# elodin-sys/elodin

Hardware: AMD Instinct MI355X
Metric: entity-steps/s (6DOF RK4) (higher is better)
Workload: dtype f64

## Files before the change

elodin_amd/codegen.py:

```python
from __future__ import annotations

import hashlib
import os
import subprocess
from dataclasses import dataclass, field
from pathlib import Path
from typing import Callable, Optional, Dict, List, NamedTuple, Sequence, Tuple

from . import dsl

PKG = Path(__file__).resolve().parent
CSRC = PKG / "csrc"
JIT_DIR = PKG / "_jit"
HIPCC = os.environ.get("HIPCC", "/opt/rocm/bin/hipcc")

_LEAF_CPP = {
    "qi": "b.q.i", "qj": "b.q.j", "qk": "b.q.k", "qw": "b.q.w", "px": "b.p.x", "py": "b.p.y", "pz": "b.p.z",
    "wx": "b.v.ang.x", "wy": "b.v.ang.y", "wz": "b.v.ang.z", "vx": "b.v.lin.x", "vy": "b.v.lin.y", "vz": "b.v.lin.z",
    "Ix": "b.I.x", "Iy": "b.I.y", "Iz": "b.I.z", "mass": "b.mass",
}
_BIN = {"add": "+", "sub": "-", "mul": "*", "div": "/"}
_FN1 = {"sqrt": "m_sqrt", "abs": "m_abs", "sin": "m_sin", "cos": "m_cos", "tan": "m_tan", "exp": "m_exp",
        "log": "m_log", "acos": "m_acos", "asin": "m_asin", "log1p": "m_log1p", "expm1": "m_expm1", "cbrt": "m_cbrt",
        "floor": "m_floor", "ceil": "m_ceil", "trunc": "m_trunc", "rint": "m_rint", "sinh": "m_sinh", "cosh": "m_cosh",
# ... 1490 lines not shown
    if constexpr (kOnlySmall != 1) {{      // one pack launch (unless p->packed), then fold + integrate per tick
        const hipError_t e = launch_pair_ticks_t<PairCustom, false, kOnlyIntegrator>(*p, integrator, n_ticks, p->packed != 0, s, launches);
        if (e != hipSuccess) return static_cast<int>(e);
    }}
    return static_cast<int>(hipSuccess);
}}
'''


def build_pair(tf: "dsl.TracedFold", integrator: Optional[int] = None, small: Optional[bool] = None) -> Path:
    return _compile(generate_pair_source(tf, integrator, small), "pair")


def generate_graph_fold_source(tf: "dsl.TracedGraphFold") -> str:
    u = _Unit()
    f = tf.fold
    w = tf.widths[f.out]
    _, loads_a, loads_b, body = _fold_front(u, tf.outputs, w, [(f"P.left[{i}]", tf.widths[n]) for i, n in enumerate(f.left)],
                                            [(f"P.right[{i}]", tf.widths[n]) for i, n in enumerate(f.right)], T="double")
    init = ", ".join(repr(v) for v in f.init)
    nl = "\n"
    return f'''// generated by elodin_amd/codegen.py — do not edit.  stand-alone edge_fold system: {f.__name__}
#include <hip/hip_runtime.h>
#include <cstdint>
#include <cmath>
namespace sixdof {{
__device__ __forceinline__ double fast_sqrt(double x) {{ return sqrt(x); }}
__device__ __forceinline__ float fast_sqrt(float x) {{ return sqrtf(x); }}
{_PRELUDE}
{_emit_tables(u)}
struct GraphFoldParams {{
    const double* left[8];
    const double* right[8];
    double* scratch;             // [n_src, {w}]
    double* out;                 // the output component column, dense over the row set
    const uint32_t* row_start;   // [n_src + 1]
    const uint32_t* dst;         // [n_edges] target rows
    const uint32_t* src_rows;    // [n_src] source rows
    uint32_t n_src;
}};

__global__ __launch_bounds__(256) void graph_fold_kernel(const GraphFoldParams P) {{
    using T = double;
    const uint32_t i = blockIdx.x * blockDim.x + threadIdx.x;
    if (i >= P.n_src) return;
    const uint32_t row = P.src_rows[i];
{nl.join(loads_a)}
    double acc[{w}] = {{{init}}};
    for (uint32_t e = P.row_start[i]; e < P.row_start[i + 1]; e++) {{
{nl.join(loads_b("P.dst[e]"))}
{body}
    }}
    for (int k = 0; k < {w}; k++) P.scratch[(size_t)i * {w} + k] = acc[k];
}}

__global__ __launch_bounds__(256) void graph_fold_commit(const GraphFoldParams P) {{
    const uint32_t i = blockIdx.x * blockDim.x + threadIdx.x;
    if (i >= P.n_src) return;
    for (int k = 0; k < {w}; k++) P.out[(size_t)P.src_rows[i] * {w} + k] = P.scratch[(size_t)i * {w} + k];
}}
}}  // namespace sixdof

extern "C" unsigned graph_fold_abi() {{ return static_cast<unsigned>(sizeof(sixdof::GraphFoldParams)); }}
extern "C" int graph_fold_launch(const sixdof::GraphFoldParams* p, unsigned n_ticks, void* stream) {{
    using namespace sixdof;
    if (p->n_src == 0) return 0;
    hipStream_t s = static_cast<hipStream_t>(stream);
    const dim3 grid((p->n_src + 255) / 256);
    for (unsigned t = 0; t < n_ticks; t++) {{
        hipLaunchKernelGGL(graph_fold_kernel, grid, dim3(256), 0, s, *p);
        hipLaunchKernelGGL(graph_fold_commit, grid, dim3(256), 0, s, *p);
    }}
    return static_cast<int>(hipGetLastError());
}}
'''


def build_graph_fold(tf: "dsl.TracedGraphFold") -> Path:
    return _compile(generate_graph_fold_source(tf), "gfold")


def _headers_digest() -> str:
    h = hashlib.sha1()
    for name in ("step_kernel.hpp", "pair_kernel.hpp", "effectors.hpp", "spatial.hpp", "kernels.hpp"):
        h.update((CSRC / name).read_bytes())
    h.update((PKG.parent / "include" / "sixdof_hip.h").read_bytes())
    return h.hexdigest()


def policy_for(n_rows: int, row_elems: int, elem_bytes: int) -> Optional[int]:
    if os.environ.get("SIXDOF_STREAMING") is not None or os.environ.get("SIXDOF_ALL_POLICIES", "") == "1":
        return None
    return 1 if int(n_rows) * int(row_elems) * int(elem_bytes) <= (768 << 20) else 9


def build(tp: dsl.TracedPipe, dtype: str = "float64", integrator: int = 0, fast_math: bool = False, window_soa: bool = False,
          column_soa: bool = False, guard_selects: Optional[bool] = None, policy: Optional[int] = None) -> Path:
    policy = policy if policy in (0, 1, 9) else None
    if getattr(tp, "prebuilt_so", None) is not None:
        if not Path(tp.prebuilt_so).exists():
            raise FileNotFoundError(tp.prebuilt_so)
        return Path(tp.prebuilt_so)
    if getattr(tp, "frozen_source", None) is not None:
        return _compile(tp.frozen_source, "pipe")
    if dtype == "float32" and getattr(tp, "float32_refused", None):
        raise NotImplementedError("this program cannot be built with dtype float32: " + "; ".join(tp.float32_refused[:4]))
    variants = VARIANTS if isinstance(tp, dsl.TracedProgram) else VARIANTS[:2]
    first_src = None
    if isinstance(tp, dsl.TracedProgram) and not tp.fold_stages:
        u = _unit(tp, variants[0], fast_math, window_soa, column_soa, guard_selects, policy, estimate=True)
        first_src = _source(tp, dtype, integrator, fast_math, u)
        est = u.estimate
        regs_per_value = 2 if dtype == "float64" else 1
        held = sum(int(w_) for _, w_ in tp.columns)
        if est and (est.get("program", 0) + held) * regs_per_value > PRESSURE_BUDGET_REGS:
            lean = sorted([v for v in ("program", "demand", "pressure") if v in est], key=lambda v: (est[v], VARIANTS.index(v)))
            variants = tuple(lean) + tuple(v for v in variants if v not in lean)
            first_src = None
        last_estimate.clear()
        last_estimate.update(est)
    for k, variant in enumerate(variants):
        try:
            src_k = first_src if (k == 0 and first_src is not None) else \
                generate_variant(tp, variant, dtype, integrator, fast_math, window_soa, column_soa, guard_selects, policy)
            so = _compile(src_k, "pipe", expect_scratch=variant == "memory")
            last_variant[0] = variant
            return so
        except SpillError:
            if os.environ.get(ALLOW_SPILLS_ENV, "") == "1" or k == len(variants) - 1:
                raise


VARIANTS = ("program", "demand", "pressure", "memory", "out_of_line")
PRESSURE_BUDGET_REGS = 440
last_estimate: Dict[str, int] = {}
last_variant = ["program"]


def generate_variant(tp, variant: str, dtype: str = "float64", integrator: int = 0, fast_math: bool = False, window_soa: bool = False,
                     column_soa: bool = False, guard_selects: Optional[bool] = None, policy: Optional[int] = None) -> str:
    if variant not in VARIANTS:
        raise ValueError(f"variant must be one of {VARIANTS}")
    return _source(tp, dtype, integrator, fast_math, _unit(tp, variant, fast_math, window_soa, column_soa, guard_selects, policy))


_BASE_FLAGS = ["-mllvm", "-disable-machine-licm"]
_RETRY_FLAGS = ["-mllvm", "-sink-insts-to-avoid-spills"]
_ATTEMPTS = (("-O3", _BASE_FLAGS), ("-O3", _BASE_FLAGS + _RETRY_FLAGS), ("-O1", []))
_CACHE_TAG = "rp3"
SPECULATIVE_MIN_SOURCE = 120_000
build_stats: Dict[str, float] = {"hipcc_invocations": 0, "cache_hits": 0}
ALLOW_SPILLS_ENV = "SIXDOF_ALLOW_SPILLS"
last_resources: Dict[str, int] = {}


class SpillError(RuntimeError):
    """No build of a generated program fits a wave's registers."""


_hipcc_id = None


def _hipcc_version() -> str:
    global _hipcc_id
    if _hipcc_id is None:
        try:
            _hipcc_id = subprocess.run([HIPCC, "--version"], capture_output=True, text=True).stdout.strip()
# ... 381 lines not shown
```

elodin_amd/csrc/aql_chain.cpp:

```cpp
#include <dlfcn.h>
#include <elf.h>
#include <hip/hip_runtime.h>
#include <hsa/hsa_ext_amd.h>

#include <algorithm>
#include <atomic>
#include <chrono>
#include <cstring>
#include <fstream>
#include <iterator>
#include <map>
#include <mutex>
#include <string>
#include <vector>

#include "aql_chain.hpp"

namespace sixdof::aql {

namespace {

constexpr uint32_t kRingSlots = 1024;
constexpr char kBundleMagic[] = "__CLANG_OFFLOAD_BUNDLE__";
constexpr char kTarget[] = "hipv4-amdgcn-amd-amdhsa--gfx950";
// ... 117 lines not shown
                uint64_t off, size, tl;
                std::memcpy(&off, sec + e, 8);
                std::memcpy(&size, sec + e + 8, 8);
                std::memcpy(&tl, sec + e + 16, 8);
                e += 24;
                if (e + tl > s.sh_size) break;
                if (std::string(sec + e, tl) == kTarget && b + off + size <= s.sh_size) out.emplace_back(s.sh_offset + b + off, size);
                e += tl;
            }
        }
    }
    return out;
}

bool contains(const char* p, size_t n, const std::string& needle) {
    return std::search(p, p + n, needle.begin(), needle.end()) != p + n;
}

}

Device* acquire(int hip_device, std::string* why) {
    std::lock_guard<std::mutex> lock(g_devices_mutex);
    auto it = g_devices.find(hip_device);
    if (it != g_devices.end()) {
        it->second->refs++;
        return it->second;
    }
    hsa_status_t s = hsa_init();
    if (s != HSA_STATUS_SUCCESS) return *why = hsa_error("hsa_init", s), nullptr;
    auto* d = new Device();
    d->hip_device = hip_device;
    if (!setup(d, why)) {
        destroy(d);
        return nullptr;
    }
    d->refs = 1;
    g_devices[hip_device] = d;
    return d;
}

void release(Device* d) {
    if (!d) return;
    std::lock_guard<std::mutex> lock(g_devices_mutex);
    if (--d->refs > 0) return;
    g_devices.erase(d->hip_device);
    destroy(d);
}

bool kernel_code(Device* d, const void* stub, uint32_t explicit_kernarg_bytes, KernelCode* out, std::string* why) {
    std::lock_guard<std::mutex> lock(d->m);
    if (auto it = d->kernels.find(stub); it != d->kernels.end()) return *out = it->second, true;
    Dl_info info{};
    if (!dladdr(stub, &info) || !info.dli_sname || info.dli_saddr != stub) return *why = "dladdr: the kernel's host handle has no symbol", false;
    const std::string name = std::string(info.dli_sname) + ".kd";
    for (const auto& [off, size] : gfx950_code_objects(d->library)) {
        if (!contains(d->library.data() + off, size, std::string(1, '\0') + name + '\0')) continue;
        auto ex = d->executables.find(off);
        if (ex == d->executables.end()) {
            hsa_code_object_reader_t reader;
            hsa_executable_t exe;
            hsa_status_t s = hsa_code_object_reader_create_from_memory(d->library.data() + off, size, &reader);
            if (s != HSA_STATUS_SUCCESS) return *why = hsa_error("hsa_code_object_reader_create_from_memory", s), false;
            s = hsa_executable_create_alt(HSA_PROFILE_FULL, HSA_DEFAULT_FLOAT_ROUNDING_MODE_DEFAULT, nullptr, &exe);
            if (s == HSA_STATUS_SUCCESS) {
                s = hsa_executable_load_agent_code_object(exe, d->agent, reader, nullptr, nullptr);
                if (s == HSA_STATUS_SUCCESS) s = hsa_executable_freeze(exe, nullptr);
                if (s != HSA_STATUS_SUCCESS) hsa_executable_destroy(exe);
            }
            hsa_code_object_reader_destroy(reader);
            if (s != HSA_STATUS_SUCCESS) return *why = hsa_error("loading the library's gfx950 code object", s), false;
            ex = d->executables.emplace(off, exe).first;
        }
        hsa_executable_symbol_t sym;
        if (hsa_executable_get_symbol_by_name(ex->second, name.c_str(), &d->agent, &sym) != HSA_STATUS_SUCCESS) continue;
        KernelCode k;
        bool dynamic_stack = true;
        hsa_status_t s = hsa_executable_symbol_get_info(sym, HSA_EXECUTABLE_SYMBOL_INFO_KERNEL_OBJECT, &k.object);
        if (s == HSA_STATUS_SUCCESS) s = hsa_executable_symbol_get_info(sym, HSA_EXECUTABLE_SYMBOL_INFO_KERNEL_KERNARG_SEGMENT_SIZE, &k.kernarg_size);
        if (s == HSA_STATUS_SUCCESS) s = hsa_executable_symbol_get_info(sym, HSA_EXECUTABLE_SYMBOL_INFO_KERNEL_KERNARG_SEGMENT_ALIGNMENT, &k.kernarg_align);
        if (s == HSA_STATUS_SUCCESS) s = hsa_executable_symbol_get_info(sym, HSA_EXECUTABLE_SYMBOL_INFO_KERNEL_GROUP_SEGMENT_SIZE, &k.group_size);
        if (s == HSA_STATUS_SUCCESS) s = hsa_executable_symbol_get_info(sym, HSA_EXECUTABLE_SYMBOL_INFO_KERNEL_PRIVATE_SEGMENT_SIZE, &k.private_size);
        if (s == HSA_STATUS_SUCCESS) s = hsa_executable_symbol_get_info(sym, HSA_EXECUTABLE_SYMBOL_INFO_KERNEL_DYNAMIC_CALLSTACK, &dynamic_stack);
        if (s != HSA_STATUS_SUCCESS) return *why = hsa_error("hsa_executable_symbol_get_info", s), false;
        if (k.kernarg_size != explicit_kernarg_bytes)
            return *why = name + ": kernarg segment of " + std::to_string(k.kernarg_size) + " bytes, " +
                          std::to_string(explicit_kernarg_bytes) + " explicit (hidden arguments)", false;
        if (dynamic_stack) return *why = name + ": dynamic call stack", false;
        d->kernels[stub] = k;
        return *out = k, true;
    }
    return *why = name + ": not found in the library's gfx950 code objects", false;
}

namespace {

uint64_t ring_read_index(void* q) { return hsa_queue_load_read_index_scacquire(static_cast<hsa_queue_t*>(q)); }
uint64_t ring_reserve(void* q, uint64_t n) { return hsa_queue_add_write_index_scacq_screl(static_cast<hsa_queue_t*>(q), n); }
void ring_doorbell(void* q, uint64_t index) {
    hsa_signal_store_screlease(static_cast<hsa_queue_t*>(q)->doorbell_signal, static_cast<hsa_signal_value_t>(index));
}

}

bool run_chain(Device* d, const Run* runs, size_t n_runs, double stall_s, double* device_ms, std::string* why) {
    std::lock_guard<std::mutex> lock(d->m);
    if (d->fault.empty() && d->queue_status.load() != HSA_STATUS_SUCCESS)
        d->fault = hsa_error("AQL queue error", static_cast<hsa_status_t>(d->queue_status.load()));
    if (!d->fault.empty()) return *why = d->fault, false;
    uint64_t n = 0;
    for (size_t i = 0; i < n_runs; i++) n += runs[i].count;
    *device_ms = 0.0;
    if (n == 0) return true;
    hsa_signal_store_relaxed(d->first, 1);
    hsa_signal_store_relaxed(d->last, 1);
    const hsa_signal_t first = n == 1 ? d->last : d->first;
    const Ring ring{static_cast<hsa_kernel_dispatch_packet_t*>(d->queue->base_address), d->queue->size, d->queue,
                    ring_read_index, ring_reserve, ring_doorbell};
    if (!write_chain(ring, runs, n_runs, first, d->last, stall_s))
        return *why = d->fault = "AQL chain: the queue read no packet for " + std::to_string(stall_s) + " s", false;
    uint64_t seen = hsa_queue_load_read_index_relaxed(d->queue);
    auto deadline = std::chrono::steady_clock::now() + std::chrono::duration<double>(stall_s);
    while (hsa_signal_load_scacquire(d->last) != 0) {
        if (d->queue_status.load() != HSA_STATUS_SUCCESS)
            return *why = d->fault = hsa_error("AQL queue error", static_cast<hsa_status_t>(d->queue_status.load())), false;
        const auto now = std::chrono::steady_clock::now();
        if (const uint64_t read = hsa_queue_load_read_index_relaxed(d->queue); read != seen) {
            seen = read;
            deadline = now + std::chrono::duration<double>(stall_s);
        } else if (now > deadline) {
            return *why = d->fault = "AQL chain: no progress for " + std::to_string(stall_s) + " s", false;
        }
    }
    hsa_amd_profiling_dispatch_time_t a{}, b{};
    if (hsa_amd_profiling_get_dispatch_time(d->agent, first, &a) == HSA_STATUS_SUCCESS &&
        hsa_amd_profiling_get_dispatch_time(d->agent, d->last, &b) == HSA_STATUS_SUCCESS && b.end > a.start)
        *device_ms = static_cast<double>(b.end - a.start) * 1e-6;
    return true;
}

}
```

elodin_amd/csrc/aql_chain.hpp:

```cpp
#pragma once

#include <hsa/hsa.h>

#include <cstdint>
#include <string>

namespace sixdof::aql {

constexpr uint16_t kWorkgroup = 64;

struct KernelCode {
    uint64_t object = 0;
    uint32_t kernarg_size = 0, kernarg_align = 0, group_size = 0, private_size = 0;
};

struct Run {
    KernelCode code;
    const void* kernarg = nullptr;
    uint32_t blocks = 0;
    uint64_t count = 0;
};

uint32_t header_setup(uint64_t i, uint64_t n);

void fill_body(hsa_kernel_dispatch_packet_t* p, const KernelCode& k, uint32_t blocks, const void* kernarg, hsa_signal_t signal);

struct Ring {
    hsa_kernel_dispatch_packet_t* base = nullptr;
    uint64_t size = 0;
    void* ctx = nullptr;
    uint64_t (*read_index)(void* ctx) = nullptr;
    uint64_t (*reserve)(void* ctx, uint64_t n) = nullptr;
    void (*doorbell)(void* ctx, uint64_t index) = nullptr;
};

bool write_chain(const Ring& r, const Run* runs, size_t n_runs, hsa_signal_t first, hsa_signal_t last, double timeout_s);


struct Device;

Device* acquire(int hip_device, std::string* why);
void release(Device* d);

bool kernel_code(Device* d, const void* stub, uint32_t explicit_kernarg_bytes, KernelCode* out, std::string* why);

bool run_chain(Device* d, const Run* runs, size_t n_runs, double stall_s, double* device_ms, std::string* why);

}
```

elodin_amd/csrc/aql_packets.cpp:

```cpp
#include <chrono>
#include <cstring>

#include "aql_chain.hpp"

namespace sixdof::aql {

uint32_t header_setup(uint64_t i, uint64_t n) {
    const uint32_t acquire = i == 0 ? HSA_FENCE_SCOPE_SYSTEM : HSA_FENCE_SCOPE_AGENT;
    const uint32_t release = i + 1 == n ? HSA_FENCE_SCOPE_SYSTEM : HSA_FENCE_SCOPE_AGENT;
    const uint32_t header = (HSA_PACKET_TYPE_KERNEL_DISPATCH << HSA_PACKET_HEADER_TYPE) | (1u << HSA_PACKET_HEADER_BARRIER) |
                            (acquire << HSA_PACKET_HEADER_SCACQUIRE_FENCE_SCOPE) |
                            (release << HSA_PACKET_HEADER_SCRELEASE_FENCE_SCOPE);
    const uint32_t setup = 1u << HSA_KERNEL_DISPATCH_PACKET_SETUP_DIMENSIONS;
    return header | setup << 16;
}

void fill_body(hsa_kernel_dispatch_packet_t* p, const KernelCode& k, uint32_t blocks, const void* kernarg, hsa_signal_t signal) {
    std::memset(reinterpret_cast<char*>(p) + 4, 0, sizeof(*p) - 4);
    p->workgroup_size_x = kWorkgroup;
    p->workgroup_size_y = 1;
    p->workgroup_size_z = 1;
    p->grid_size_x = static_cast<uint32_t>(kWorkgroup) * blocks;
    p->grid_size_y = 1;
    p->grid_size_z = 1;
    p->private_segment_size = k.private_size;
    p->group_segment_size = k.group_size;
    p->kernel_object = k.object;
    p->kernarg_address = const_cast<void*>(kernarg);
    p->completion_signal = signal;
}

bool write_chain(const Ring& r, const Run* runs, size_t n_runs, hsa_signal_t first, hsa_signal_t last, double timeout_s) {
    uint64_t n = 0;
    for (size_t i = 0; i < n_runs; i++) n += runs[i].count;
    if (n == 0) return true;
    const hsa_signal_t none{0};
    size_t run = 0;
    uint64_t in_run = 0;
    uint64_t done = 0;
    while (done < n) {
        uint64_t room = r.size - (r.reserve(r.ctx, 0) - r.read_index(r.ctx));
        const auto deadline = std::chrono::steady_clock::now() + std::chrono::duration<double>(timeout_s);
        while (room == 0) {
            if (std::chrono::steady_clock::now() > deadline) return false;
            room = r.size - (r.reserve(r.ctx, 0) - r.read_index(r.ctx));
        }
        const uint64_t m = n - done < room ? n - done : room;
        const uint64_t w = r.reserve(r.ctx, m);
        for (uint64_t j = 0; j < m; j++) {
            while (in_run == runs[run].count) run++, in_run = 0;
            const Run& R = runs[run];
            const uint64_t i = done + j;
            const hsa_signal_t sig = i + 1 == n ? last : i == 0 ? first : none;
            fill_body(&r.base[(w + j) & (r.size - 1)], R.code, R.blocks, R.kernarg, sig);
            in_run++;
        }
        for (uint64_t j = 0; j < m; j++)
            __atomic_store_n(reinterpret_cast<uint32_t*>(&r.base[(w + j) & (r.size - 1)]), header_setup(done + j, n), __ATOMIC_RELEASE);
        done += m;
        r.doorbell(r.ctx, w + m - 1);
    }
    return true;
}

}
```

elodin_amd/csrc/hip_fake.cpp:

```cpp
#include <hip/hip_runtime.h>

#include <algorithm>
#include <cstdio>
#include <cstdlib>
#include <cstring>
#include <deque>
#include <functional>
#include <map>
#include <set>
#include <string>
#include <vector>

#include "../../include/sixdof_hip.h"
#include "aql_chain.hpp"
#include "covariance_plan.hpp"
#include "envelope_plan.hpp"
#include "events_plan.hpp"
#include "extremes_plan.hpp"
#include "history_plan.hpp"
#include "kernels.hpp"
#include "quantile_plan.hpp"

namespace hip_fake {

std::map<const char*, size_t> g_allocs;
std::set<void*> g_streams, g_events;
std::map<const char*, size_t> g_pins;
long g_calls = 0, g_fail_at = -1, g_violations = 0;
bool g_fired = false;

enum { kAtOnce = 0, kMinimal = 1, kComputeFirst = 2, kCopyFirst = 3 };
int g_schedule = kAtOnce;
bool g_running = false;
struct Op {
    std::string what;
    std::function<hipError_t()> run;
    std::vector<const void*> dev;
    const char* host = nullptr;
    size_t host_bytes = 0;
    void* wait_stream = nullptr;
    uint64_t wait_pos = 0;
};
struct Queue {
    uint64_t order = 0;
    bool non_blocking = false;
    std::deque<Op> ops;
    uint64_t done = 0;
    uint64_t enqueued() const { return done + ops.size(); }
};
struct Record { void* stream = nullptr; uint64_t pos = 0; };
std::map<void*, Queue> g_queues;
std::map<void*, Record> g_records;
std::vector<void*> g_quarantine;
uint64_t g_order = 0;

void fail_after(long n) { g_fail_at = n < 0 ? -1 : g_calls + n, g_fired = false; }
bool fired() { return g_fired; }
long calls() { return g_calls; }
long violations() { return g_violations; }
size_t live_allocations() { return g_allocs.size(); }
size_t live_streams() { return g_streams.size(); }
size_t live_events() { return g_events.size(); }
size_t live_page_locks() { return g_pins.size(); }
bool lock_intersects(const void* p, size_t bytes) {
    const char* lo = static_cast<const char*>(p);
    for (auto& kv : g_pins)
        if (kv.first < lo + bytes && lo < kv.first + kv.second) return true;
    return false;
}
size_t queued() {
    size_t n = 0;
    for (auto& kv : g_queues) n += kv.second.ops.size();
    return n;
}
const char* schedule_name(int schedule) {
    return schedule == kAtOnce ? "at-once" : schedule == kMinimal ? "minimal" : schedule == kComputeFirst ? "compute-first" : "copy-first";
}

static hipError_t fallible() {
    if (g_calls++ != g_fail_at) return hipSuccess;
    g_fired = true;
    return hipErrorOutOfMemory;
}
static bool live(const void* p, size_t bytes) {
    auto it = g_allocs.upper_bound(static_cast<const char*>(p));
    if (!p || it == g_allocs.begin()) return false;
    --it;
    return static_cast<const char*>(p) + bytes <= it->first + it->second;
}
static bool need(bool ok, const char* what) {
    if (!ok) std::fprintf(stderr, "hip_fake: a launch was handed a table that is not (wholly) a live allocation: %s\n", what), g_violations++;
    return ok;
}
static hipError_t launch(bool ok) {
    if (!g_running)
        if (hipError_t e = fallible(); e != hipSuccess) return e;
    return ok ? hipSuccess : hipErrorInvalidValue;
}

static void flush_quarantine() {
    if (queued()) return;
    for (void* p : g_quarantine) std::free(p);
    g_quarantine.clear();
}
static hipError_t drain(void* s, uint64_t upto) {
    auto it = g_queues.find(s);
    if (it == g_queues.end()) return hipSuccess;
    Queue& q = it->second;
    hipError_t first = hipSuccess;
    while (q.done < upto && !q.ops.empty()) {
        Op& op = q.ops.front();
        if (op.wait_stream)
            if (hipError_t e = drain(op.wait_stream, op.wait_pos); e != hipSuccess) return e;
        if (op.run) {
            if (hipError_t e = fallible(); e != hipSuccess) return e;
            g_running = true;
            const hipError_t e = op.run();
            g_running = false;
            if (e != hipSuccess && first == hipSuccess) first = e;
        }
        q.ops.pop_front();
        q.done++;
    }
    return first;
}
static hipError_t drain_all(bool youngest_first, bool blocking_only = false) {
    std::vector<std::pair<uint64_t, void*>> order;
    for (auto& kv : g_queues)
        if (!blocking_only || !kv.second.non_blocking) order.emplace_back(kv.second.order, kv.first);
    std::sort(order.begin(), order.end());
    if (youngest_first) std::reverse(order.begin(), order.end());
    hipError_t first = hipSuccess;
    for (auto& o : order) {
        auto it = g_queues.find(o.second);
        if (it == g_queues.end()) continue;
        const hipError_t e = drain(o.second, it->second.enqueued());
        if (e == hipErrorOutOfMemory) return e;
        if (e != hipSuccess && first == hipSuccess) first = e;
    }
    return first;
}
static hipError_t force(void* s, uint64_t upto) {
// ... 172 lines not shown
    std::memcpy(dst, src, bytes);
    return hipSuccess;
}
static const char* copy_name(hipMemcpyKind kind) {
    return kind == hipMemcpyDeviceToHost ? "device-to-host copy" : kind == hipMemcpyHostToDevice ? "host-to-device copy" : "device-to-device copy";
}
static void copy_host_side(void* dst, const void* src, size_t bytes, hipMemcpyKind kind) {
    if (kind == hipMemcpyDeviceToHost) host_extent(dst, bytes, copy_name(kind));
    if (kind == hipMemcpyHostToDevice) host_extent(src, bytes, copy_name(kind));
}
hipError_t hipMemcpy(void* dst, const void* src, size_t bytes, hipMemcpyKind kind) {
    copy_host_side(dst, src, bytes, kind);
    if (deferring()) {
        const hipError_t e = g_schedule == kMinimal ? drain_all(false, true) : force(nullptr, 0);
        flush_quarantine();
        if (e != hipSuccess) return e;
    }
    return copy(dst, src, bytes, kind);
}
hipError_t hipMemcpyAsync(void* dst, const void* src, size_t bytes, hipMemcpyKind kind, hipStream_t s) {
    if (!need(g_streams.count(s), "copy on a null or destroyed stream")) return hipErrorInvalidHandle;
    copy_host_side(dst, src, bytes, kind);
    if (!deferring()) return copy(dst, src, bytes, kind);
    std::vector<const void*> dev;
    if (kind != hipMemcpyHostToDevice) dev.push_back(src);
    if (kind != hipMemcpyDeviceToHost) dev.push_back(dst);
    const void* host = kind == hipMemcpyDeviceToHost ? dst : kind == hipMemcpyHostToDevice ? src : nullptr;
    if (kind == hipMemcpyDeviceToHost) std::memset(dst, 0xFF, bytes);
    return defer(s, copy_name(kind), std::move(dev), [=] { return copy(dst, src, bytes, kind); }, host, host ? bytes : 0);
}
hipError_t hipMemsetAsync(void* dst, int v, size_t bytes, hipStream_t s) {
    if (deferring()) return defer(s, "memset", {dst}, [=] { return hipMemsetAsync(dst, v, bytes, s); });
    if (!g_running)
        if (hipError_t e = fallible(); e != hipSuccess) return e;
    if (!need(live(dst, bytes), "memset destination")) return hipErrorInvalidValue;
    std::memset(dst, v, bytes);
    return hipSuccess;
}

namespace sixdof {

static bool body_ok(const void* pos, const void* vel, const void* accel, const void* force, const void* inertia, size_t n, size_t es) {
    return need(live(pos, n * 7 * es), "world_pos") & need(live(vel, n * 6 * es), "world_vel") & need(live(accel, n * 6 * es), "world_accel") &
           need(live(force, n * 6 * es), "force") & need(live(inertia, n * 7 * es), "inertia");
}
static bool ops_ok(const DevOp* ops, uint32_t n_ops, size_t n, size_t es) {
    bool ok = true;
    for (uint32_t k = 0; k < n_ops; k++)
        if (ops[k].aux) ok &= need(live(ops[k].aux, n * (ops[k].aux_width ? ops[k].aux_width : 3) * es), "effector aux column");
    return ok;
}
static bool step_ok(const StepParams& p, int dtype) {
    const size_t n = p.n, es = dtype == 1 ? 4 : 8;
    bool ok = body_ok(p.pos, p.vel, p.accel, p.force, p.inertia, n, es) & ops_ok(p.ops, p.n_ops, n, es);
    if (p.hist_ring) {
        const size_t r = p.hist_ring;
        ok &= need(live(p.hist_pos, r * n * 7 * es), "hist_pos") & need(live(p.hist_vel, r * n * 6 * es), "hist_vel") &
              need(live(p.hist_accel, r * n * 6 * es), "hist_accel") & need(live(p.hist_force, r * n * 6 * es), "hist_force");
    }
    for (int k = 0; k < kMaxModelCols; k++) {
        if (p.model_cols[k]) ok &= need(live(p.model_cols[k], n * es), "program column");
        if (p.model_hist[k]) ok &= need(live(p.model_hist[k], p.hist_ring * n * es), "program column ring");
    }
    return ok;
}
static bool pair_ok(const PairParams& p) {
    const size_t n = p.n, u = sizeof(uint32_t), d = sizeof(double);
    bool ok = body_ok(p.pos, p.vel, p.accel, p.force, p.inertia, n, 8) & ops_ok(p.ops, p.n_ops, n, 8);
    if (n) ok &= need(live(p.pack, n * kPackWidth * d), "pack") & need(live(p.partial, n * p.partial_width * p.splits * d), "partial");
    if (n && p.pack_next) ok &= need(live(p.pack_next, n * kPackWidth * d), "pack_next");
    if (p.pair_kind != SIXDOF_EFF_ALLPAIRS_GRAVITY_SOFTENED) {
        ok &= need(live(p.row_start, (n + 1) * u), "row_start");
        if (ok) ok &= need(p.row_start[n] == p.n_edges, "row_start[n] != n_edges");
    }
    if (p.n_edges) ok &= need(live(p.dst, p.n_edges * u), "dst");
    if (p.n_hubs)
        ok &= need(live(p.hub_rows, p.n_hubs * u), "hub_rows") & need(live(p.hub_chunk_start, (p.n_hubs + 1) * u), "hub_chunk_start") &
              need(live(p.chunk_e0, p.n_hub_chunks * u), "chunk_e0") & need(live(p.chunk_row, p.n_hub_chunks * u), "chunk_row") &
              need(live(p.chunk_partial, size_t(p.n_hub_chunks) * kPartialWidth * d), "chunk_partial");
    return ok;
}

StepKernel select_step(const StepParams&, int, int) { return {}; }
hipError_t launch_step(const StepParams& p, int integrator, int dtype, hipStream_t s) {
    if (deferring()) return defer(s, "launch_step", {p.pos, p.vel, p.accel, p.force, p.hist_pos, p.hist_vel, p.hist_accel, p.hist_force}, [=] { return launch_step(p, integrator, dtype, s); });
    const bool ok = step_ok(p, dtype);
    if (ok && p.hist_ring && p.hist_pos) {
        const size_t es = dtype == 1 ? 4 : 8;
        const void* live_col[4] = {p.pos, p.vel, p.accel, p.force};
        void* rings[4] = {p.hist_pos, p.hist_vel, p.hist_accel, p.hist_force};
        for (uint32_t t = 0; t < p.n_ticks; t++)
            for (int k = 0; k < 4; k++) {
                const size_t block = size_t(p.n) * (k == 0 ? 7 : 6) * es;
                std::memcpy(static_cast<char*>(rings[k]) + (p.hist_slot0 + t) % p.hist_ring * block, live_col[k], block);
            }
    }
    return launch(ok);
}
uint32_t pair_splits_for(uint32_t) { return 1; }
static hipError_t launch_pair(const PairParams& p, hipStream_t s) {
    if (deferring()) return defer(s, "pair launch", {p.pos, p.vel, p.accel, p.force, p.pack, p.partial}, [=] { return launch(pair_ok(p)); });
    return launch(pair_ok(p));
}
hipError_t launch_pair_ticks(const PairParams& p, int, uint32_t n_ticks, hipStream_t s, uint64_t* launches) { return *launches += 1 + 2 * n_ticks, launch_pair(p, s); }
hipError_t launch_pair_small(const PairParams& p, int, uint32_t, hipStream_t s, uint64_t* launches) { return *launches += 1, launch_pair(p, s); }
hipError_t launch_apollo(const ApolloParams&, hipStream_t s) {
    if (deferring()) return defer(s, "launch_apollo", {}, [] { return launch(true); });
    return launch(true);
}

static hipError_t move_rows(char* dst, const char* src, const uint32_t* rows, uint32_t m, size_t row, bool gather) {
    if (!need(live(rows, m * sizeof(uint32_t)), "join rows")) return launch(false);
    for (uint32_t j = 0; j < m; j++) {
        char* to = gather ? dst + j * row : dst + rows[j] * row;
        const char* from = gather ? src + rows[j] * row : src + j * row;
        if (!need(live(to, row) && live(from, row), "joined column")) return launch(false);
        std::memcpy(to, from, row);
    }
    return launch(true);
}
hipError_t launch_gather_rows(void* dst, const void* src, const uint32_t* rows, uint32_t m, uint32_t w, size_t elem, hipStream_t s) {
    if (deferring()) return defer(s, "gather_rows", {dst, src, rows}, [=] { return launch_gather_rows(dst, src, rows, m, w, elem, s); });
    return move_rows(static_cast<char*>(dst), static_cast<const char*>(src), rows, m, w * elem, true);
}
hipError_t launch_scatter_rows(void* dst, const void* src, const uint32_t* rows, uint32_t m, uint32_t w, size_t elem, hipStream_t s) {
    if (deferring()) return defer(s, "scatter_rows", {dst, src, rows}, [=] { return launch_scatter_rows(dst, src, rows, m, w, elem, s); });
    return move_rows(static_cast<char*>(dst), static_cast<const char*>(src), rows, m, w * elem, false);
}
hipError_t launch_history_gather(const HistoryGatherArgs& a, uint32_t n_components, void* out, const uint32_t* rows, uint64_t m, uint64_t n,
                                 uint64_t first_tick, uint64_t n_samples, uint64_t every, uint64_t ring, size_t elem, hipStream_t s) {
    if (deferring()) {
        std::vector<const void*> dev{out, rows};
        for (uint32_t c = 0; c < n_components; c++) dev.push_back(a.c[c].ring);
        return defer(s, "history_gather", std::move(dev), [=] { return launch_history_gather(a, n_components, out, rows, m, n, first_tick, n_samples, every, ring, elem, s); });
    }
    if (!need(live(rows, m * sizeof(uint32_t)), "watch rows")) return launch(false);
    for (uint32_t c = 0; c < n_components; c++) {
        const size_t row = a.c[c].w * elem;
        for (uint64_t e = 0; e < m; e++)
            for (uint64_t j = 0; j < n_samples; j++) {
                const char* from = static_cast<const char*>(a.c[c].ring) + (((first_tick + j * every - 1) % ring) * n + rows[e]) * row;
                char* to = static_cast<char*>(out) + a.c[c].out_offset * elem + (e * n_samples + j) * row;
                if (!need(live(from, row) && live(to, row), "ring or watch staging")) return launch(false);
                std::memcpy(to, from, row);
            }
    }
    return launch(true);
}
template <class Units, class Tick>
static bool ring_bin_walk(const char* who, const RingBinArgs& a, uint32_t n_components, double* out, uint64_t planes, uint64_t stride, uint64_t n,
                          uint32_t period, uint64_t first_tick, uint64_t sample0, uint64_t n_samples, uint64_t every, uint64_t ring, size_t elem,
                          Units units, Tick tick) {
    const std::string scratch = std::string(who) + " scratch of one sample", blocks = std::string("ring or ") + who + " staging";
    for (uint32_t k = 0; k < n_components; k++) {
        const RingBinDesc& d = a.c[k];
        if (!envelope_supported(d.w, period)) return false;
        if (!need(d.scratch_offset + units(d) <= stride, scratch.c_str())) return false;
        const uint64_t total = n * d.w;
        for (uint64_t j = 0; j < n_samples; j++) {
            const char* src = static_cast<const char*>(d.ring) + sample_slot(first_tick, sample0 + j, every, ring) * total * elem;
            double* to = out + d.out_offset + (sample0 + j) * period * planes * d.w;
            if (!need(live(src, total * elem) && live(to, size_t(period) * planes * d.w * sizeof(double)), blocks.c_str())) return false;
            tick(d, j, src, to);
        }
    }
    return true;
}
hipError_t launch_history_envelope(const RingBinArgs& a, uint32_t n_components, double* out, void* partial, uint64_t partial_stride, uint64_t n,
                                   uint32_t period, uint64_t first_tick, uint64_t sample0, uint64_t n_samples, uint64_t every, uint64_t ring,
// ... 322 lines not shown
```

elodin_amd/csrc/kernels.hpp:

```cpp
#pragma once
#include <hip/hip_runtime.h>
#include <stdint.h>

#pragma clang fp contract(on)

namespace sixdof {

constexpr int kMaxOps = 4;
constexpr int kMaxModelCols = 128;
constexpr int kBlock = 256;

struct DevOp {
    int32_t kind;
    int32_t aux_width;
    const void* aux;
    double p[6];
};

struct StepParams {
    void* pos;
    void* vel;
    void* accel;
    void* force;
    const void* inertia;
    uint32_t n;
    uint32_t n_ticks;
    double dt_g;
    double dt;
    uint32_t n_ops;
    uint32_t vel_independent;
    uint32_t streaming;
    uint32_t hist_ring;
    uint64_t hist_slot0;
    void* hist_pos;
    void* hist_vel;
    void* hist_accel;
    void* hist_force;
    uint64_t tick0;
    uint32_t accel_in_check;
    uint32_t state_only;
    DevOp ops[kMaxOps];
    void* model_cols[kMaxModelCols];
    void* model_hist[kMaxModelCols];
};

enum : int { kRk4 = 0, kSemiImplicit = 1, kNone = 2 };

struct StepKernel {
    const void* fn = nullptr;
    dim3 grid;
};

StepKernel select_step(const StepParams& p, int integrator, int dtype);

hipError_t launch_step(const StepParams& p, int integrator, int dtype, hipStream_t stream);

using CustomAbiFn = unsigned (*)();
using CustomLayoutFn = unsigned (*)();
using CustomLaunchFn = int (*)(const StepParams*, int integrator, int dtype, void* stream);

constexpr int kPackWidth = 10;
constexpr int kPartialForce = 9;
constexpr int kPartialWidth = 18;

struct PairParams {
    void* pos;
    void* vel;
    void* accel;
    void* force;
    const void* inertia;
    uint32_t n;
    double dt_g, dt;
    double* pack;
    double* pack_next;
    double* partial;
    uint32_t splits;
    uint32_t partial_width;
    const uint32_t* row_start;
    const uint32_t* dst;
    uint32_t n_edges;
    uint32_t n_hubs, n_hub_chunks;
    const uint32_t* hub_rows;
    const uint32_t* hub_chunk_start;
    const uint32_t* chunk_e0;
    const uint32_t* chunk_row;
    double* chunk_partial;
    int32_t pair_kind;
    double p0, p1;
    uint32_t n_ops;
    DevOp ops[kMaxOps];
    uint32_t packed;
};
uint32_t pair_splits_for(uint32_t n);
hipError_t launch_pair_ticks(const PairParams& p, int integrator, uint32_t n_ticks, hipStream_t stream, uint64_t* launches);
constexpr uint32_t kPairSmallMax = 256;
constexpr uint32_t kHubDegree = 32;
constexpr uint32_t kHubChunk = 256;
hipError_t launch_pair_small(const PairParams& p, int integrator, uint32_t n_ticks, hipStream_t stream,
                             uint64_t* launches);
using CustomPairAbiFn = unsigned (*)();
using CustomPairLaunchFn = int (*)(const PairParams* p, int integrator, uint32_t n_ticks, int small, void* stream,
                                   uint64_t* launches);

hipError_t launch_gather_rows(void* dst, const void* src, const uint32_t* rows, uint32_t m, uint32_t w, size_t elem,
                              hipStream_t s);
hipError_t launch_scatter_rows(void* dst, const void* src, const uint32_t* rows, uint32_t m, uint32_t w, size_t elem,
                               hipStream_t s);

constexpr uint32_t kHistoryGatherMax = 32;
struct HistoryGatherDesc {
    const void* ring;
    uint64_t out_offset;
    uint32_t w;
    uint32_t reserved;
};
struct HistoryGatherArgs { HistoryGatherDesc c[kHistoryGatherMax]; };
hipError_t launch_history_gather(const HistoryGatherArgs& a, uint32_t n_components, void* out, const uint32_t* rows,
                                 uint64_t m, uint64_t n, uint64_t first_tick, uint64_t n_samples, uint64_t every,
                                 uint64_t ring, size_t elem, hipStream_t s);

constexpr uint32_t kRingBinMaxComponents = 32;
struct RingBinDesc {
    const void* ring;
    uint64_t out_offset;
    uint64_t scratch_offset;
    uint32_t w;
    uint32_t reserved;
};
struct RingBinArgs { RingBinDesc c[kRingBinMaxComponents]; };

hipError_t launch_history_envelope(const RingBinArgs& a, uint32_t n_components, double* out, void* partial, uint64_t partial_stride,
                                   uint64_t n, uint32_t period, uint64_t first_tick, uint64_t sample0, uint64_t n_samples,
                                   uint64_t every, uint64_t ring, size_t elem, hipStream_t s);

struct QuantileRanks;
hipError_t launch_history_quantiles(const RingBinArgs& a, uint32_t n_components, const QuantileRanks& ranks, double* out, void* hist,
                                    void* state, uint64_t slot_stride, uint64_t n, uint32_t period, uint64_t first_tick,
                                    uint64_t sample0, uint64_t n_samples, uint64_t every, uint64_t ring, size_t elem, hipStream_t s);
// ... 46 lines not shown
```

elodin_amd/csrc/sixdof_capi.cpp:

```cpp
#include <dlfcn.h>
#include <hip/hip_runtime.h>

#include <algorithm>
#include <chrono>
#include <cmath>
#include <cstdio>
#include <cstdlib>
#include <cstring>
#include <iterator>
#include <map>
#include <string>
#include <unordered_map>
#include <vector>

#include "../../include/sixdof_hip.h"
#include "../../include/sixdof_apollo.h"
#include "kernels.hpp"
#include "abi_guard.hpp"
#include "device_mem.hpp"
#include "aql_chain.hpp"
#include "covariance_plan.hpp"
#include "envelope_plan.hpp"
#include "events_plan.hpp"
#include "extremes_plan.hpp"
#include "quantile_plan.hpp"
#include "history_plan.hpp"
#include "step_plan.hpp"

using namespace sixdof;

namespace {

struct Column {
    uint64_t id = 0;
    int prim = SIXDOF_PRIM_F64;
    uint64_t width = 1;
    uint64_t n_rows = 0;
    size_t elem = 8;
    size_t bytes = 0;
    std::vector<uint64_t> ids;
    void* host = nullptr;
    DeviceBuffer dev;
    std::vector<uint32_t> rows;
    DeviceBuffer d_rows, compact;
    void* live = nullptr;
    bool joined = false;
    DeviceBuffer snap;
    PinnedRange host_pinned;

    void drop_join() {
        d_rows.reset(), compact.reset();
        rows.clear();
        live = nullptr;
        joined = false;
    }
};

thread_local std::string g_create_error;

struct FoldTable {
    const uint32_t* src_rows;
    const uint32_t* row_start;
    const uint32_t* dst;
    uint32_t n_src;
    uint32_t n_lane;
};
constexpr uint32_t kFoldWaveDegree = 64;

struct FoldSlot {
    bool needs_table = false;
    bool wave_ok = false;
    uint32_t count = 1, stride = 0;
    bool set = false;
    DeviceBuffer d_blob;
    FoldTable table{};
};
using SetFoldTableFn = int (*)(unsigned, const FoldTable*);

double now_ms() {
    using namespace std::chrono;
    return duration<double, std::milli>(steady_clock::now().time_since_epoch()).count();
}

uint64_t cid(const char* s) { return sixdof_component_id(s); }

constexpr uint32_t kAqlSlots = 8;
constexpr uint32_t kAqlSpare0 = 3;

struct Replay {
    StepParams key{};
    std::map<uint32_t, hipGraphExec_t> graphs;
    bool state_only_off = false;
    bool aql_off = false;
    aql::Device* aql_dev = nullptr;
    std::string aql_why;
    std::string aql_fault;
    DeviceBuffer aql_args;
    std::map<uint64_t, aql::Run> aql_runs;
    uint64_t aql_slot_key[kAqlSlots] = {};
    uint32_t aql_next_spare = kAqlSpare0;

    void drop() {
        for (auto& kv : graphs) hipGraphExecDestroy(kv.second);
        graphs.clear();
        aql_runs.clear();
        std::fill(std::begin(aql_slot_key), std::end(aql_slot_key), 0);
        aql_next_spare = kAqlSpare0;
    }
    void rekey(StepParams P) {
        P.tick0 = P.hist_slot0 = 0;
        if (std::memcmp(&P, &key, sizeof(P)) != 0) drop(), key = P;
    }
    void release() {
        drop();
        if (!aql_fault.empty()) (void)aql_args.release();
        aql_args.reset();
        aql::release(aql_dev);
    }
};

struct Edges {
    std::vector<uint32_t> src, dst;
    DeviceBuffer d_csr_start, d_csr_dst;
    DeviceBuffer d_hub, d_chunk_partial;
    uint32_t n_hubs = 0, n_hub_chunks = 0;
};

struct History {
    uint32_t ring = 0;
    uint64_t first_tick = 0;
    DeviceBuffer body[4];
    std::vector<DeviceBuffer> model;
    DeviceBuffer env_stage, env_partial;
    DeviceBuffer quant_stage, quant_scratch;
    DeviceBuffer cov_stage, cov_partial;
    struct ScanState {
        bool valid = false;
        std::vector<uint64_t> signature;
        std::vector<const void*> rings;
        std::vector<size_t> widths;
        uint64_t n = 0;
        uint64_t last_tick = 0;
    };
    struct TimeScan {
        DeviceBuffer stage, scratch, rec;
        ScanState acc;
    } extremes, events;
    void reset() { *this = History{}; }
};

struct CopyLane {
    Stream stream;
    Event ev_snap, ev_copied;
    bool pending = false;
    uint64_t stream_lo = 1, stream_hi = 0;
    std::vector<PinnedRange> pinned_user;
    hipError_t hold(hipStream_t compute) { return pending ? hipStreamWaitEvent(compute, ev_copied.get(), 0) : hipSuccess; }
    hipError_t begin(hipStream_t compute) {
        hipError_t e = ensure();
        if (e == hipSuccess) e = hipEventRecord(ev_snap.get(), compute);
        if (e == hipSuccess) e = hipStreamWaitEvent(stream.get(), ev_snap.get(), 0);
        return e;
    }
    hipError_t copy(void* dst, const void* src, size_t bytes, size_t pin_bytes) {
        if (pin_bytes)
            if (hipError_t e = pin(dst, pin_bytes); e != hipSuccess) return e;
        return hipMemcpyAsync(dst, src, bytes, hipMemcpyDeviceToHost, stream.get());
    }
    hipError_t end() {
        hipError_t e = hipEventRecord(ev_copied.get(), stream.get());
        if (e == hipSuccess) pending = true;
        return e;
    }
    hipError_t ensure() {
        if (stream) return hipSuccess;
        Stream s;
// ... 90 lines not shown
    std::vector<uint64_t> watch_ids;
    DeviceBuffer d_watch_rows;
    size_t watch_m = 0;
    DeviceBuffer d_watch_stage;
    int model = 0;
    std::vector<double> ap_time, ap_alt, ap_rate, ap_pitch, ap_hspeed, ap_downrange;
    bool accel_is_host_data = false;
    uint32_t ap_ticks_per_telemetry = 3;
    uint32_t ap_guidance_period = 5;
    uint64_t ap_max_ticks = 0;
    DeviceBuffer d_tick_refs;
    Replay replay;
    std::string path;
    mutable std::string err;

    BodyCol body[5] = {{"world_pos", 7, SIXDOF_COL_WORLD_POS, 0, 0},     {"world_vel", 6, SIXDOF_COL_WORLD_VEL, 1, 0},
                       {"world_accel", 6, SIXDOF_COL_WORLD_ACCEL, 2, 0}, {"force", 6, SIXDOF_COL_FORCE, 3, 0},
                       {"inertia", 7, SIXDOF_COL_INERTIA, -1, 0}};
    uint64_t id_pos, id_vel, id_accel, id_force, id_inertia, id_tick, id_dt;

    int fail(int code, const std::string& msg) const {
        err = msg;
        return code;
    }
    int hip_fail(hipError_t e, const char* what) const {
        err = std::string(what) + ": " + hipGetErrorString(e);
        return SIXDOF_ERR_BACKEND;
    }
    Column* col(uint64_t id) {
        auto it = cols.find(id);
        return it == cols.end() ? nullptr : &it->second;
    }
    const Column* col(uint64_t id) const {
        auto it = cols.find(id);
        return it == cols.end() ? nullptr : &it->second;
    }
    size_t elem_size() const { return desc.dtype == SIXDOF_F32 ? 4 : 8; }
    int state_prim() const { return desc.dtype == SIXDOF_F32 ? SIXDOF_PRIM_F32 : SIXDOF_PRIM_F64; }
    void drop_watch() {
        d_watch_rows.reset();
        watch_ids.clear();
        watch_m = 0;
    }
    bool has_pair_op() const {
        for (auto& o : ops)
            if (SIXDOF_EFF_IS_PAIR(o.kind)) return true;
        return false;
    }
};

std::string* err_of(const sixdof_handle* h) { return h ? &const_cast<sixdof_handle*>(h)->err : &g_create_error; }

#define HIP_TRY(h, call)                                      \
    do {                                                      \
        hipError_t e_ = (call);                               \
        if (e_ != hipSuccess) return (h)->hip_fail(e_, #call); \
    } while (0)

static int resolve_join(sixdof_handle* h, Column* c) {
    if (c->joined) return SIXDOF_OK;
    const size_t m = h->joined_ids.size();
    if (c->ids == h->joined_ids) {
        c->live = c->dev.get();
        c->joined = true;
        return SIXDOF_OK;
    }
    std::vector<uint32_t> rows;
    if (resolve_rows(row_map(c->ids), h->joined_ids.data(), m, &rows) != m)
        return h->fail(SIXDOF_ERR_ENTITY_MISMATCH, "join: a column does not cover the joined Body entity set");
    DeviceBuffer d_rows, compact;
    if (m) {
        HIP_TRY(h, d_rows.alloc(m * sizeof(uint32_t)));
        HIP_TRY(h, hipMemcpy(d_rows.get(), rows.data(), m * sizeof(uint32_t), hipMemcpyHostToDevice));
        HIP_TRY(h, compact.alloc(m * c->width * c->elem));
    }
    c->rows.swap(rows);
    c->d_rows = std::move(d_rows), c->compact = std::move(compact);
    c->live = c->compact.get();
    c->joined = true;
    return SIXDOF_OK;
}

static int gather_joined(sixdof_handle* h, Column* c) {
    if (!c->joined || !c->compact) return SIXDOF_OK;
    hipError_t e = launch_gather_rows(c->compact.get(), c->dev.get(), c->d_rows.get<uint32_t>(), static_cast<uint32_t>(h->joined_ids.size()),
                                      static_cast<uint32_t>(c->width), c->elem, h->stream.get());
    return e == hipSuccess ? SIXDOF_OK : h->hip_fail(e, "gather_rows");
}

static int ensure_joined(sixdof_handle* h, Column* c) {
    if (c->joined) return SIXDOF_OK;
    int rc = resolve_join(h, c);
    return rc != SIXDOF_OK ? rc : gather_joined(h, c);
}

static int upload_one(sixdof_handle* h, Column* c) {
    if (c->bytes) HIP_TRY(h, hipMemcpyAsync(c->dev.get(), c->host, c->bytes, hipMemcpyHostToDevice, h->stream.get()));
    return gather_joined(h, c);
}

extern "C" {

uint32_t sixdof_abi_version(void) { return SIXDOF_ABI_VERSION; }


int sixdof_device_count(void) try {
    int n = 0;
    if (hipGetDeviceCount(&n) != hipSuccess) return 0;
    return n;
} SIXDOF_ABI_CATCH(&g_create_error)

const char* sixdof_last_error(const sixdof_handle* h) { return h ? h->err.c_str() : g_create_error.c_str(); }

void sixdof_destroy(sixdof_handle* h);

int sixdof_create(const sixdof_desc* d, sixdof_handle** out) try {
    if (!d || !out) {
        g_create_error = "sixdof_create: null argument";
        return SIXDOF_ERR_INVALID_ARGUMENT;
    }
    *out = nullptr;
    if (d->struct_size != sizeof(sixdof_desc)) {
        g_create_error = "sixdof_create: struct_size mismatch (ABI version skew)";
        return SIXDOF_ERR_INVALID_ARGUMENT;
    }
    if (d->integrator != SIXDOF_INTEGRATOR_RK4 && d->integrator != SIXDOF_INTEGRATOR_SEMI_IMPLICIT &&
        d->integrator != SIXDOF_INTEGRATOR_NONE) {
        g_create_error = "sixdof_create: unknown integrator";
        return SIXDOF_ERR_INVALID_ARGUMENT;
    }
    if (d->dtype != SIXDOF_F64 && d->dtype != SIXDOF_F32) {
        g_create_error = "sixdof_create: unknown dtype";
        return SIXDOF_ERR_INVALID_ARGUMENT;
    }
    if (d->n_entities > 0xFFFFFFF0ull) {
        g_create_error = "sixdof_create: n_entities exceeds u32 row index range";
        return SIXDOF_ERR_INVALID_ARGUMENT;
    }
    int n_dev = 0;
    hipError_t e = hipGetDeviceCount(&n_dev);
    if (e != hipSuccess || n_dev == 0) {
        g_create_error = std::string("sixdof_create: no HIP device (") + hipGetErrorString(e) +
                         "); this backend has no CPU fallback";
        return SIXDOF_ERR_NO_DEVICE;
    }
    if (d->device_ordinal < 0 || d->device_ordinal >= n_dev) {
        g_create_error = "sixdof_create: device_ordinal out of range";
        return SIXDOF_ERR_INVALID_ARGUMENT;
    }
    auto* h = new sixdof_handle();
    h->desc = *d;
    if (h->desc.ticks_per_launch == 0) h->desc.ticks_per_launch = 1;
    const char* aql_env = std::getenv("SIXDOF_AQL");
    h->replay.aql_off = aql_env && aql_env[0] == '0';
    const char* so_env = std::getenv("SIXDOF_STATE_ONLY");
    h->replay.state_only_off = so_env && so_env[0] == '0';
    h->device = d->device_ordinal;
    for (BodyCol& b : h->body) b.id = cid(b.name);
    h->id_pos = h->body[0].id, h->id_vel = h->body[1].id, h->id_accel = h->body[2].id, h->id_force = h->body[3].id;
    h->id_inertia = h->body[4].id;
    h->id_tick = cid("tick");
    h->id_dt = cid("simulation_time_step");
    if ((e = hipSetDevice(h->device)) != hipSuccess || (e = hipStreamCreate(h->stream.out())) != hipSuccess ||
        (e = hipEventCreate(h->ev0.out())) != hipSuccess || (e = hipEventCreate(h->ev1.out())) != hipSuccess ||
        (e = hipEventCreate(h->evp0.out())) != hipSuccess || (e = hipEventCreate(h->evp1.out())) != hipSuccess) {
        g_create_error = std::string("sixdof_create: ") + hipGetErrorString(e);
        sixdof_destroy(h);
        return SIXDOF_ERR_BACKEND;
    }
    *out = h;
    return SIXDOF_OK;
} SIXDOF_ABI_CATCH(&g_create_error)

void sixdof_destroy(sixdof_handle* h) try {
    if (!h) return;
    hipSetDevice(h->device);
    if (h->stream) hipStreamSynchronize(h->stream.get());
    if (h->copy.stream) hipStreamSynchronize(h->copy.stream.get());
    h->replay.release();
    delete h;
} SIXDOF_ABI_CATCH_VALUE(err_of(h), )

int sixdof_bind_columns(sixdof_handle* h, const sixdof_column* cols, size_t n_cols) try {
    if (!h || (!cols && n_cols)) return SIXDOF_ERR_INVALID_ARGUMENT;
    h->bound = h->resident = false;
    h->hist.extremes.acc.valid = h->hist.events.acc.valid = false;
    HIP_TRY(h, hipSetDevice(h->device));
    h->replay.drop();
    if (h->d_watch_rows) {
        HIP_TRY(h, hipStreamSynchronize(h->stream.get()));
        h->drop_watch();
    }
    for (size_t i = 0; i < n_cols; i++) {
        const sixdof_column& c = cols[i];
        if (c.ndim > 1) return h->fail(SIXDOF_ERR_UNSUPPORTED, "bind_columns: only scalar / 1-D components");
        if (!c.host_ptr && c.n_rows) return h->fail(SIXDOF_ERR_INVALID_ARGUMENT, "bind_columns: null host_ptr");
        Column col;
        col.id = c.component_id;
        col.prim = c.prim_type;
        col.width = c.ndim == 0 ? 1 : c.dims[0];
        col.n_rows = c.n_rows;
        col.elem = c.prim_type == SIXDOF_PRIM_F32 ? 4 : 8;
        col.bytes = static_cast<size_t>(col.width * col.n_rows) * col.elem;
        col.host = c.host_ptr;
        if (c.entity_ids) col.ids.assign(c.entity_ids, c.entity_ids + c.n_rows);
        if (Column* old = h->col(c.component_id)) {
            if (old->bytes == col.bytes) col.dev = std::move(old->dev);
            if (h->copy.stream) HIP_TRY(h, hipStreamSynchronize(h->copy.stream.get()));
        }
        if (!col.dev && col.bytes) HIP_TRY(h, col.dev.alloc(col.bytes));
        h->cols[c.component_id] = std::move(col);
    }
    const Column* first = nullptr;
    bool identical = true;
    for (auto& b : h->body) {
        const Column* c = h->col(b.id);
        if (!c) return h->fail(SIXDOF_ERR_COMPONENT_NOT_FOUND, std::string("bind_columns: missing Body column ") + b.name);
        if (c->prim != h->state_prim())
            return h->fail(SIXDOF_ERR_VALUE_SIZE_MISMATCH, std::string("bind_columns: dtype mismatch on ") + b.name);
        if (c->width != b.width)
            return h->fail(SIXDOF_ERR_VALUE_SIZE_MISMATCH, std::string("bind_columns: shape mismatch on ") + b.name);
        if (c->ids.size() != c->n_rows)
            return h->fail(SIXDOF_ERR_INVALID_ARGUMENT, std::string("bind_columns: entity_ids missing on ") + b.name);
        if (!first) first = c;
        else if (c->ids != first->ids) identical = false;
    }
    if (identical) {
        h->joined_ids = first->ids;
    } else {
        std::vector<uint64_t> acc(first->ids);
        std::sort(acc.begin(), acc.end());
        for (auto& b : h->body) {
            std::vector<uint64_t> ids(h->col(b.id)->ids), out;
            std::sort(ids.begin(), ids.end());
            std::set_intersection(acc.begin(), acc.end(), ids.begin(), ids.end(), std::back_inserter(out));
            acc.swap(out);
        }
        h->joined_ids.swap(acc);
    }
    h->identity_join = identical;
    if (h->desc.n_entities == 0) h->desc.n_entities = h->joined_ids.size();
    if (h->custom_rows_multiple > 1 && h->desc.n_entities % h->custom_rows_multiple != 0)
        return h->fail(SIXDOF_ERR_INVALID_ARGUMENT, "bind_columns: the installed program lays a world out as " + std::to_string(h->custom_rows_multiple) +
                       " consecutive rows; the joined " + std::to_string(h->desc.n_entities) + " rows are not a whole number of worlds");
    if (h->joined_ids.size() != h->desc.n_entities)
        return h->fail(SIXDOF_ERR_VALUE_SIZE_MISMATCH, "bind_columns: n_entities does not match the joined Body entity set");
    for (auto& kv : h->cols) kv.second.drop_join();
    for (auto& b : h->body) {
        int rc = resolve_join(h, h->col(b.id));
        if (rc != SIXDOF_OK) return rc;
    }
    h->bound = true;
    return SIXDOF_OK;
} SIXDOF_ABI_CATCH(err_of(h))

int sixdof_bind_world(sixdof_handle* h, sixdof_world* w) try {
    if (!h || !w) return SIXDOF_ERR_INVALID_ARGUMENT;
    std::vector<uint64_t> ids(sixdof_world_components(w, nullptr, 0));
    sixdof_world_components(w, ids.data(), ids.size());
    std::vector<sixdof_column> cols;
    for (uint64_t id : ids) {
        sixdof_column c{};
        if (sixdof_world_column(w, id, &c) != SIXDOF_OK) continue;
        if (id == h->id_tick || id == h->id_dt) continue;
        if (c.prim_type != h->state_prim() || c.ndim > 1) continue;
        cols.push_back(c);
    }
    h->desc.simulation_time_step = sixdof_world_time_step(w);
    h->tick = sixdof_world_tick(w);
    return sixdof_bind_columns(h, cols.data(), cols.size());
} SIXDOF_ABI_CATCH(err_of(h))

int sixdof_set_effectors(sixdof_handle* h, const sixdof_effector_op* ops, size_t n_ops) try {
    if (!h || (!ops && n_ops)) return SIXDOF_ERR_INVALID_ARGUMENT;
    size_t n_entity_ops = 0, n_pair = 0;
    for (size_t i = 0; i < n_ops; i++) {
        const int k = ops[i].kind;
        if (k < SIXDOF_EFF_CONST_WRENCH || k > SIXDOF_EFF_WORLD_FORCE || k == SIXDOF_EFF_EDGE_CUSTOM)
            return h->fail(SIXDOF_ERR_INVALID_ARGUMENT, "set_effectors: unknown effector kind");
        if (SIXDOF_EFF_IS_PAIR(k)) {
            n_pair++;
            if (i + 1 != n_ops)
                return h->fail(SIXDOF_ERR_UNSUPPORTED, "set_effectors: a pair (edge_fold) op must be last in the pipe");
        } else {
            n_entity_ops++;
        }
    }
    if (n_entity_ops > static_cast<size_t>(kMaxOps))
        return h->fail(SIXDOF_ERR_UNSUPPORTED, "set_effectors: at most 4 per-entity ops");
    if (n_pair > 1) return h->fail(SIXDOF_ERR_UNSUPPORTED, "set_effectors: at most one pair op");
    h->ops.assign(ops, ops + n_ops);
    h->replay.drop();
    return SIXDOF_OK;
} SIXDOF_ABI_CATCH(err_of(h))

int sixdof_set_edges(sixdof_handle* h, const uint64_t* from_ids, const uint64_t* to_ids, size_t n_edges) try {
    if (!h || ((!from_ids || !to_ids) && n_edges)) return SIXDOF_ERR_INVALID_ARGUMENT;
    if (!h->bound) return h->fail(SIXDOF_ERR_COMPONENT_NOT_FOUND, "set_edges: bind Body columns first");
    HIP_TRY(h, hipSetDevice(h->device));
    Edges ne;
    std::vector<uint32_t>&src = ne.src, &dst = ne.dst;
    const RowMap row_of = row_map(h->joined_ids);
    if (resolve_rows(row_of, from_ids, n_edges, &src) != n_edges || resolve_rows(row_of, to_ids, n_edges, &dst) != n_edges)
        return h->fail(SIXDOF_ERR_COMPONENT_NOT_FOUND, "set_edges: edge endpoint is not a Body entity");
    const uint32_t n = static_cast<uint32_t>(h->desc.n_entities);
    std::vector<uint32_t> start(n + 1, 0), cdst(n_edges);
    for (size_t e = 0; e < n_edges; e++) start[src[e] + 1]++;
    for (uint32_t i = 0; i < n; i++) start[i + 1] += start[i];
    std::vector<uint32_t> cursor(start.begin(), start.end() - 1);
    for (size_t e = 0; e < n_edges; e++) cdst[cursor[src[e]]++] = dst[e];
    HIP_TRY(h, ne.d_csr_start.alloc((n + 1) * sizeof(uint32_t)));
    HIP_TRY(h, hipMemcpy(ne.d_csr_start.get(), start.data(), (n + 1) * sizeof(uint32_t), hipMemcpyHostToDevice));
    if (n_edges) {
        HIP_TRY(h, ne.d_csr_dst.alloc(n_edges * sizeof(uint32_t)));
        HIP_TRY(h, hipMemcpy(ne.d_csr_dst.get(), cdst.data(), n_edges * sizeof(uint32_t), hipMemcpyHostToDevice));
    }
    std::vector<uint32_t> hub_rows, hub_chunk_start{0}, chunk_e0, chunk_row;
    const char* no_hubs = std::getenv("SIXDOF_NO_HUBS");
    for (uint32_t i = 0; i < n && !(no_hubs && no_hubs[0] == '1'); i++) {
        const uint32_t deg = start[i + 1] - start[i];
        if (deg < kHubDegree) continue;
        hub_rows.push_back(i);
        for (uint32_t e = start[i]; e < start[i + 1]; e += kHubChunk) {
            chunk_e0.push_back(e);
            chunk_row.push_back(i);
        }
        hub_chunk_start.push_back(static_cast<uint32_t>(chunk_e0.size()));
    }
    ne.n_hubs = static_cast<uint32_t>(hub_rows.size());
    ne.n_hub_chunks = static_cast<uint32_t>(chunk_e0.size());
    if (ne.n_hubs) {
        std::vector<uint32_t> blob;
        blob.insert(blob.end(), hub_rows.begin(), hub_rows.end());
        blob.insert(blob.end(), hub_chunk_start.begin(), hub_chunk_start.end());
        blob.insert(blob.end(), chunk_e0.begin(), chunk_e0.end());
// ... 69 lines not shown
    }
    HIP_TRY(h, hipStreamSynchronize(h->stream.get()));
    h->last.d2h_download_ms = now_ms() - t_dn;
    return SIXDOF_OK;
} SIXDOF_ABI_CATCH(err_of(h))

int sixdof_download_async(sixdof_handle* h, uint32_t mask) try {
    if (!h) return SIXDOF_ERR_INVALID_ARGUMENT;
    if (!h->bound) return h->fail(SIXDOF_ERR_COMPONENT_NOT_FOUND, "download_async: no columns bound");
    HIP_TRY(h, hipSetDevice(h->device));
    CopyLane& lane = h->copy;
    HIP_TRY(h, lane.hold(h->stream.get()));
    Column* picked[5];
    int n_picked = 0;
    for (auto& b : h->body) {
        if (!(mask & b.bit)) continue;
        Column* c = h->col(b.id);
        if (!c || !c->bytes) continue;
        int rc = scatter_back(h, c);
        if (rc != SIXDOF_OK) return rc;
        if (!c->snap) HIP_TRY(h, c->snap.alloc(c->bytes));
        HIP_TRY(h, hipMemcpyAsync(c->snap.get(), c->dev.get(), c->bytes, hipMemcpyDeviceToDevice, h->stream.get()));
        if (!c->host_pinned) c->host_pinned.lock(c->host, c->bytes);
        picked[n_picked++] = c;
    }
    HIP_TRY(h, lane.begin(h->stream.get()));
    for (int k = 0; k < n_picked; k++) HIP_TRY(h, lane.copy(picked[k]->host, picked[k]->snap.get(), picked[k]->bytes, 0));
    HIP_TRY(h, lane.end());
    return SIXDOF_OK;
} SIXDOF_ABI_CATCH(err_of(h))

int sixdof_download_wait(sixdof_handle* h) try {
    if (!h) return SIXDOF_ERR_INVALID_ARGUMENT;
    if (!h->copy.pending) return SIXDOF_OK;
    HIP_TRY(h, hipSetDevice(h->device));
    const double t0 = now_ms();
    HIP_TRY(h, hipEventSynchronize(h->copy.ev_copied.get()));
    h->copy.stream_lo = 1, h->copy.stream_hi = 0;
    h->last.d2h_download_ms = now_ms() - t0;
    return SIXDOF_OK;
} SIXDOF_ABI_CATCH(err_of(h))

int sixdof_sync(sixdof_handle* h) try {
    if (!h) return SIXDOF_ERR_INVALID_ARGUMENT;
    HIP_TRY(h, hipSetDevice(h->device));
    HIP_TRY(h, hipStreamSynchronize(h->stream.get()));
    if (h->copy.stream) HIP_TRY(h, hipStreamSynchronize(h->copy.stream.get()));
    float ms0 = 0.f;
    if (h->step_pending && hipEventElapsedTime(&ms0, h->ev0.get(), h->ev1.get()) == hipSuccess) h->last.kernel_device_ms = ms0;
    h->step_pending = h->prev_pending = false;
    h->copy.pending = false;
    h->copy.stream_lo = 1, h->copy.stream_hi = 0;
    h->copy.pinned_user.clear();
    return SIXDOF_OK;
} SIXDOF_ABI_CATCH(err_of(h))

int sixdof_get_tick(const sixdof_handle* h, uint64_t* tick) try {
    if (!h || !tick) return SIXDOF_ERR_INVALID_ARGUMENT;
    *tick = h->tick;
    return SIXDOF_OK;
} SIXDOF_ABI_CATCH(err_of(h))
int sixdof_set_tick(sixdof_handle* h, uint64_t tick) try {
    if (!h) return SIXDOF_ERR_INVALID_ARGUMENT;
    h->tick = tick;
    h->hist.first_tick = tick + 1;
    return SIXDOF_OK;
} SIXDOF_ABI_CATCH(err_of(h))
int sixdof_set_ticks_per_launch(sixdof_handle* h, uint32_t k) try {
    if (!h || k == 0) return SIXDOF_ERR_INVALID_ARGUMENT;
    h->desc.ticks_per_launch = k;
    h->replay.drop();
    return h->resident ? prepare_graph(h) : SIXDOF_OK;
} SIXDOF_ABI_CATCH(err_of(h))

int sixdof_set_flags(sixdof_handle* h, uint32_t flags) try {
    if (!h) return SIXDOF_ERR_INVALID_ARGUMENT;
    h->desc.flags = flags;
    return SIXDOF_OK;
} SIXDOF_ABI_CATCH(err_of(h))

void* sixdof_device_column(sixdof_handle* h, uint64_t component_id) try {
    if (!h) return nullptr;
    Column* c = h->col(component_id);
    return c ? (c->live ? c->live : c->dev.get()) : nullptr;
} SIXDOF_ABI_CATCH_VALUE(err_of(h), nullptr)
void* sixdof_stream(sixdof_handle* h) { return h ? static_cast<void*>(h->stream.get()) : nullptr; }

}


namespace {

int build_dev_ops(sixdof_handle* h, DevOp* out, uint32_t* n_out, uint32_t* vel_independent) {
    uint32_t n = 0;
    *vel_independent = 1;
    if (h->custom_launch) {
        for (size_t k = 0; k < h->custom_folds.size(); k++)
            if (h->custom_folds[k].needs_table && !h->custom_folds[k].set)
                return h->fail(SIXDOF_ERR_UNSUPPORTED, "step: fold stage " + std::to_string(k) + " of the installed program reads its edges from "
                               "device memory and has no table yet (sixdof_set_fold_edges)");
        for (uint64_t id : h->custom_aux) {
            Column* c = h->col(id);
            if (!c) return h->fail(SIXDOF_ERR_COMPONENT_NOT_FOUND, "step: column read by the generated pipe is not bound");
            if (c->width < 1 || c->width > 3 || c->prim != h->state_prim())
                return h->fail(SIXDOF_ERR_VALUE_SIZE_MISMATCH, "step: generated-pipe columns must be [n,1..3] of the state dtype");
            if (int rc = ensure_joined(h, c); rc != SIXDOF_OK) return rc;
            DevOp d{};
            d.aux = c->live;
            d.aux_width = static_cast<int32_t>(c->width);
            out[n++] = d;
        }
        *n_out = n;
        return SIXDOF_OK;
    }
    for (auto& o : h->ops) {
        if (SIXDOF_EFF_IS_PAIR(o.kind)) continue;
        DevOp d{};
        d.kind = o.kind;
        std::memcpy(d.p, o.p, sizeof(d.p));
        if (o.kind == SIXDOF_EFF_BODY_TORQUE || o.kind == SIXDOF_EFF_BODY_FORCE || o.kind == SIXDOF_EFF_BALL_DRAG ||
            o.kind == SIXDOF_EFF_WORLD_TORQUE || o.kind == SIXDOF_EFF_WORLD_FORCE) {
            Column* c = h->col(o.aux_component_id);
            if (!c) return h->fail(SIXDOF_ERR_COMPONENT_NOT_FOUND, "step: effector aux column not bound");
            if (c->width != 3 || c->prim != h->state_prim())
                return h->fail(SIXDOF_ERR_VALUE_SIZE_MISMATCH, "step: effector aux column must be [n,3] of the state dtype");
            if (int rc = ensure_joined(h, c); rc != SIXDOF_OK) return rc;
            d.aux = c->live;
        }
        if (o.kind == SIXDOF_EFF_BALL_DRAG) *vel_independent = 0;
        out[n++] = d;
    }
    *n_out = n;
    return SIXDOF_OK;
}

int fill_step_params(sixdof_handle* h, StepParams* P) {
    std::memset(P, 0, sizeof(*P));
    P->pos = h->col(h->id_pos)->live;
    P->vel = h->col(h->id_vel)->live;
    P->accel = h->col(h->id_accel)->live;
    P->force = h->col(h->id_force)->live;
    P->inertia = h->col(h->id_inertia)->live;
    P->n = static_cast<uint32_t>(h->desc.n_entities);
    P->dt_g = h->desc.simulation_time_step;
    P->dt = h->desc.has_time_step ? h->desc.time_step : h->desc.simulation_time_step;
    const char* force_nt = std::getenv("SIXDOF_STREAMING");
    size_t row_elems = 32;
    for (size_t k = 0; k < h->custom_model.size(); k++)
        if (const Column* c = h->col(h->custom_model[k])) row_elems += c->width;
    const size_t state_bytes = static_cast<size_t>(h->desc.n_entities) * row_elems * h->elem_size();
    uint32_t policy = 9u;
    if (state_bytes <= (768ull << 20)) policy = 1u;
    if (force_nt) {
        const uint32_t code = static_cast<uint32_t>(std::atoi(force_nt));
#ifdef SIXDOF_AB_BUILD
        policy = code;
#else
        const uint32_t pol = code & 255u;
        if ((code & ~0x1ffu) == 0 && (pol == 0u || pol == 1u || pol == 9u)) policy = code;
#endif
    }
    P->streaming = policy;
    P->hist_ring = h->hist.ring;
    if (h->hist.ring) {
        P->hist_pos = h->hist.body[0].get();
        P->hist_vel = h->hist.body[1].get();
        P->hist_accel = h->hist.body[2].get();
        P->hist_force = h->hist.body[3].get();
    }
    for (size_t k = 0; k < h->custom_model.size(); k++) {
        Column* c = h->col(h->custom_model[k]);
        if (!c) return h->fail(SIXDOF_ERR_COMPONENT_NOT_FOUND, "step: component column of the generated program is not bound");
        const unsigned expect = k < h->custom_model_width.size() ? h->custom_model_width[k] : 0u;
        const bool window = (expect >> 31) != 0;
        const size_t want = expect & 0x1fffffffu;
        if (c->prim != h->state_prim() || c->width < 1 || (!window && c->width > 64) || (want && c->width != want))
            return h->fail(SIXDOF_ERR_VALUE_SIZE_MISMATCH,
                           "step: program columns must be of the state dtype and as wide as the generated code expects "
                           "([n,1..64]; a window column [n, rows*width])");
        if (!c->joined) {
            int rc = resolve_join(h, c);
            if (rc != SIXDOF_OK) return rc;
            if (c->compact && ((expect >> 29) & 1u))
                return h->fail(SIXDOF_ERR_UNSUPPORTED, "step: a program built for element-major columns needs every column on "
                                                       "the executor's own entity set (no entity-set join)");
            if (rc = gather_joined(h, c); rc != SIXDOF_OK) return rc;
        }
        P->model_cols[k] = c->live;
        P->model_hist[k] = (h->hist.ring && k < h->hist.model.size()) ? h->hist.model[k].get() : nullptr;
    }
    P->tick0 = h->tick;
    return build_dev_ops(h, P->ops, &P->n_ops, &P->vel_independent);
}

size_t align_up(size_t x, size_t a) { return (x + a - 1) / a * a; }

hipError_t launch_any(sixdof_handle* h, const StepParams& P) {
    if (h->desc.integrator == SIXDOF_INTEGRATOR_NONE && !h->custom_launch) return hipErrorInvalidValue;
    if (h->custom_launch) {
        for (size_t k = 0; k < h->custom_folds.size(); k++)
            if (h->custom_folds[k].needs_table) h->custom_set_fold_table(static_cast<unsigned>(k), h->custom_folds[k].set ? &h->custom_folds[k].table : nullptr);
        return static_cast<hipError_t>(h->custom_launch(&P, h->desc.integrator, h->desc.dtype, h->stream.get()));
    }
    return launch_step(P, h->desc.integrator, h->desc.dtype, h->stream.get());
}

int fill_pair_params(sixdof_handle* h, PairParams* P) {
    std::memset(P, 0, sizeof(*P));
    const size_t n = h->desc.n_entities;
    const size_t es = h->elem_size();
    const sixdof_effector_op& pop = h->ops.back();
    const uint32_t splits = pop.kind == SIXDOF_EFF_ALLPAIRS_GRAVITY_SOFTENED ? pair_splits_for(static_cast<uint32_t>(n)) : 1;
    (void)es;
    const bool allpairs = pop.kind == SIXDOF_EFF_ALLPAIRS_GRAVITY_SOFTENED;
    const size_t pwidth = allpairs ? kPartialForce : kPartialWidth;
    const size_t pack_bytes = align_up(sizeof(double) * kPackWidth * n, 256);
    const size_t partial_bytes = align_up(sizeof(double) * pwidth * n * splits, 256);
    const size_t total = pack_bytes + partial_bytes + (allpairs ? 0 : pack_bytes);
    if (total > h->d_scratch.bytes()) HIP_TRY(h, h->d_scratch.alloc(total));
    char* base = h->d_scratch.get<char>();
    P->pos = h->col(h->id_pos)->live;
    P->vel = h->col(h->id_vel)->live;
    P->accel = h->col(h->id_accel)->live;
    P->force = h->col(h->id_force)->live;
    P->inertia = h->col(h->id_inertia)->live;
    P->n = static_cast<uint32_t>(n);
    P->dt_g = h->desc.simulation_time_step;
    P->dt = h->desc.has_time_step ? h->desc.time_step : h->desc.simulation_time_step;
    P->pack = reinterpret_cast<double*>(base);
    P->partial = reinterpret_cast<double*>(base + pack_bytes);
    P->pack_next = allpairs ? nullptr : reinterpret_cast<double*>(base + pack_bytes + partial_bytes);
    P->splits = splits;
    P->partial_width = static_cast<uint32_t>(pwidth);
    P->pair_kind = pop.kind;
    P->p0 = pop.p[0];
    P->p1 = pop.p[1];
    if (pop.kind != SIXDOF_EFF_ALLPAIRS_GRAVITY_SOFTENED) {
        const Edges& ed = h->edges;
        if (!ed.d_csr_start) return h->fail(SIXDOF_ERR_COMPONENT_NOT_FOUND, "step: edge effector without sixdof_set_edges");
        P->row_start = ed.d_csr_start.get<uint32_t>();
        P->dst = ed.d_csr_dst.get<uint32_t>();
        P->n_edges = static_cast<uint32_t>(ed.src.size());
        P->n_hubs = ed.n_hubs;
        P->n_hub_chunks = ed.n_hub_chunks;
        if (ed.n_hubs) {
            P->hub_rows = ed.d_hub.get<uint32_t>();
            P->hub_chunk_start = P->hub_rows + ed.n_hubs;
            P->chunk_e0 = P->hub_chunk_start + (ed.n_hubs + 1);
            P->chunk_row = P->chunk_e0 + ed.n_hub_chunks;
            P->chunk_partial = ed.d_chunk_partial.get<double>();
        }
    }
    uint32_t vi = 0;
    return build_dev_ops(h, P->ops, &P->n_ops, &vi);
}

double ref_interp(double t, const std::vector<double>& xs, const std::vector<double>& ys) {
    const size_t n = xs.size();
    if (t <= xs[0]) return ys[0];
    if (t >= xs[n - 1]) return ys[n - 1];
    size_t lo = 0, hi = n;
    while (lo < hi) {
        const size_t mid = (lo + hi) / 2;
        if (t < xs[mid]) hi = mid; else lo = mid + 1;
    }
    const size_t a = lo - 1, b = lo;
    const double span = xs[b] - xs[a];
    if (span <= 0.0) return ys[a];
    const double frac = (t - xs[a]) / span;
    return ys[a] + (ys[b] - ys[a]) * frac;
}

int snapshot_tick_to_ring(sixdof_handle* h, uint64_t ticks_done) {
    if (!h->hist.ring) return SIXDOF_OK;
    const size_t n = h->desc.n_entities, es = h->elem_size();
    const size_t slot = static_cast<size_t>(history_slot(ticks_done, h->hist.ring));
    for (int k = 0; k < 4; k++) {
        const size_t block = n * h->body[k].width * es;
        if (!block) continue;
        HIP_TRY(h, hipMemcpyAsync(h->hist.body[k].get<char>() + slot * block, h->col(h->body[k].id)->live, block,
                                  hipMemcpyDeviceToDevice, h->stream.get()));
    }
    return SIXDOF_OK;
}

int step_apollo(sixdof_handle* h, uint64_t n_ticks, uint64_t* launches) {
    const char* names[5] = {"apollo_state", "apollo_params", "apollo_guidance", "apollo_score", "apollo_result"};
    const uint64_t widths[5] = {APOLLO_N_STATE, APOLLO_N_PARAMS, APOLLO_N_GUIDANCE, APOLLO_N_SCORE, APOLLO_N_RESULT};
    Column* c[5];
    for (int k = 0; k < 5; k++) {
        c[k] = h->col(cid(names[k]));
        if (!c[k]) return h->fail(SIXDOF_ERR_COMPONENT_NOT_FOUND, std::string("step: Apollo model column not bound: ") + names[k]);
        if (c[k]->width != widths[k] || c[k]->prim != SIXDOF_PRIM_F64)
            return h->fail(SIXDOF_ERR_VALUE_SIZE_MISMATCH, std::string("step: bad shape for ") + names[k]);
        if (int rc = ensure_joined(h, c[k]); rc != SIXDOF_OK) return rc;
    }
    ApolloParams P{};
    P.pos = static_cast<double*>(h->col(h->id_pos)->live);
    P.vel = static_cast<double*>(h->col(h->id_vel)->live);
    P.accel = static_cast<double*>(h->col(h->id_accel)->live);
    P.force = static_cast<double*>(h->col(h->id_force)->live);
    P.inertia = static_cast<double*>(h->col(h->id_inertia)->live);
    P.state = static_cast<double*>(c[0]->live);
    P.params = static_cast<const double*>(c[1]->live);
    P.guidance = static_cast<double*>(c[2]->live);
    P.score = static_cast<double*>(c[3]->live);
    P.result = static_cast<double*>(c[4]->live);
    P.n = static_cast<uint32_t>(h->desc.n_entities);
    P.max_ticks = h->ap_max_ticks;
    P.guidance_period = h->ap_guidance_period;
    P.ticks_per_telemetry = h->ap_ticks_per_telemetry;
    P.dt = h->desc.simulation_time_step;
    const uint32_t K = h->hist.ring ? 1u : h->desc.ticks_per_launch;
    if (const size_t need = static_cast<size_t>(K) * 8 * sizeof(double); need > h->d_tick_refs.bytes())
        HIP_TRY(h, h->d_tick_refs.alloc(need));
    std::vector<double> refs(static_cast<size_t>(K) * 8);
    uint64_t done = 0;
    while (done < n_ticks) {
        const uint32_t k = static_cast<uint32_t>(std::min<uint64_t>(K, n_ticks - done));
        for (uint32_t j = 0; j < k; j++) {
            const double t_s = static_cast<double>(h->tick + done + j) * (1.0 / 120.0);
            double* r = &refs[static_cast<size_t>(j) * 8];
            r[0] = ref_interp(t_s, h->ap_time, h->ap_alt);
            r[1] = ref_interp(t_s, h->ap_time, h->ap_rate);
            r[2] = std::fabs(ref_interp(t_s, h->ap_time, h->ap_pitch));
            r[3] = ref_interp(t_s, h->ap_time, h->ap_hspeed);
            r[4] = ref_interp(t_s, h->ap_time, h->ap_downrange);
            r[5] = r[3] - ref_interp(t_s + 1.0, h->ap_time, h->ap_hspeed);
            r[6] = r[7] = 0.0;
        }
        HIP_TRY(h, hipMemcpyAsync(h->d_tick_refs.get(), refs.data(), static_cast<size_t>(k) * 8 * sizeof(double),
                                  hipMemcpyHostToDevice, h->stream.get()));
        HIP_TRY(h, hipStreamSynchronize(h->stream.get()));
        P.tick_refs = h->d_tick_refs.get<double>();
        P.n_ticks = k;
        P.tick0 = h->tick + done;
        hipError_t e = launch_apollo(P, h->stream.get());
        if (e != hipSuccess) return h->hip_fail(e, "launch_apollo");
        (*launches)++;
        done += k;
        if (h->hist.ring) {
            int rc = snapshot_tick_to_ring(h, h->tick + done);
            if (rc != SIXDOF_OK) return rc;
        }
    }
    return SIXDOF_OK;
}

}

extern "C" {

int sixdof_set_model_apollo(sixdof_handle* h, const sixdof_apollo_tables* t) try {
    if (!h || !t || t->n < 2 || !t->time_s || !t->altitude_m || !t->descent_rate_mps || !t->pitch_deg ||
        !t->horizontal_speed_mps || !t->downrange_m)
        return SIXDOF_ERR_INVALID_ARGUMENT;
    if (h->desc.integrator != SIXDOF_INTEGRATOR_SEMI_IMPLICIT || h->desc.dtype != SIXDOF_F64)
        return h->fail(SIXDOF_ERR_UNSUPPORTED, "set_model_apollo: the example uses el.Integrator.SemiImplicit in f64 (sim.py:523)");
    h->ap_time.assign(t->time_s, t->time_s + t->n);
    h->ap_alt.assign(t->altitude_m, t->altitude_m + t->n);
    h->ap_rate.assign(t->descent_rate_mps, t->descent_rate_mps + t->n);
    h->ap_pitch.assign(t->pitch_deg, t->pitch_deg + t->n);
    h->ap_hspeed.assign(t->horizontal_speed_mps, t->horizontal_speed_mps + t->n);
    h->ap_downrange.assign(t->downrange_m, t->downrange_m + t->n);
    h->ap_guidance_period = t->guidance_period_ticks ? t->guidance_period_ticks : 5;
    h->ap_ticks_per_telemetry = t->ticks_per_telemetry ? t->ticks_per_telemetry : 3;
    h->ap_max_ticks = t->max_ticks;
    h->model = 1;
    return SIXDOF_OK;
} SIXDOF_ABI_CATCH(err_of(h))

int sixdof_last_timings(const sixdof_handle* h, sixdof_timings* out) try {
    if (!h || !out) return SIXDOF_ERR_INVALID_ARGUMENT;
    *out = h->last;
    return SIXDOF_OK;
} SIXDOF_ABI_CATCH(err_of(h))

int sixdof_count_nonfinite(sixdof_handle* h, uint64_t* count, uint8_t* row_flags) try {
    if (!h || !count) return SIXDOF_ERR_INVALID_ARGUMENT;
    if (!h->bound) return h->fail(SIXDOF_ERR_COMPONENT_NOT_FOUND, "count_nonfinite: no columns bound");
    HIP_TRY(h, hipSetDevice(h->device));
    const uint32_t n = static_cast<uint32_t>(h->desc.n_entities);
    DeviceBuffer d_count, d_flags;
    HIP_TRY(h, d_count.alloc(sizeof(unsigned long long)));
    hipError_t e = hipMemsetAsync(d_count.get(), 0, sizeof(unsigned long long), h->stream.get());
    if (e == hipSuccess && row_flags && n) e = d_flags.alloc(n);
    if (e == hipSuccess)
        e = launch_nonfinite(h->col(h->id_pos)->live, h->col(h->id_vel)->live, n, h->elem_size(), d_flags.get<uint8_t>(),
                             d_count.get<unsigned long long>(), h->stream.get());
    unsigned long long host_count = 0;
    if (e == hipSuccess) e = hipMemcpyAsync(&host_count, d_count.get(), sizeof(host_count), hipMemcpyDeviceToHost, h->stream.get());
    if (e == hipSuccess && d_flags) e = hipMemcpyAsync(row_flags, d_flags.get(), n, hipMemcpyDeviceToHost, h->stream.get());
    if (e == hipSuccess) e = hipStreamSynchronize(h->stream.get());
    if (e != hipSuccess) {
        (void)hipStreamSynchronize(h->stream.get());
        return h->hip_fail(e, "count_nonfinite");
    }
    *count = host_count;
    return SIXDOF_OK;
} SIXDOF_ABI_CATCH(err_of(h))

int sixdof_set_custom_pipe(sixdof_handle* h, const char* so_path, const uint64_t* aux_ids, size_t n_aux) try {
    if (!h || !so_path || (!aux_ids && n_aux)) return SIXDOF_ERR_INVALID_ARGUMENT;
    DlHandle owned;
    void* dl = *owned.out() = dlopen(so_path, RTLD_NOW | RTLD_LOCAL);
    if (!dl) return h->fail(SIXDOF_ERR_BACKEND, std::string("set_custom_pipe: dlopen failed: ") + dlerror());
    auto abi = reinterpret_cast<CustomAbiFn>(dlsym(dl, "sixdof_custom_abi"));
    auto layout = reinterpret_cast<CustomLayoutFn>(dlsym(dl, "sixdof_custom_layout"));
    auto launch = reinterpret_cast<CustomLaunchFn>(dlsym(dl, "sixdof_custom_launch"));
    if (!abi || !layout || !launch || abi() != sizeof(StepParams))
        return h->fail(SIXDOF_ERR_BACKEND, "set_custom_pipe: not a generated pipe for this library build (StepParams layout differs)");
    auto col_widths = reinterpret_cast<void (*)(unsigned*)>(dlsym(dl, "sixdof_custom_column_widths"));
    auto rows_multiple = reinterpret_cast<unsigned (*)()>(dlsym(dl, "sixdof_custom_rows_multiple"));
    if (rows_multiple && rows_multiple() > 1 && h->desc.n_entities % rows_multiple() != 0)
        return h->fail(SIXDOF_ERR_INVALID_ARGUMENT, "set_custom_pipe: the program lays a world out as " + std::to_string(rows_multiple()) +
                       " consecutive rows; " + std::to_string(h->desc.n_entities) + " rows are not a whole number of worlds");
    const unsigned lay = layout();
    const size_t k_aux = lay & 0xff, k_model = (lay >> 8) & 0xff;
    if (k_aux > static_cast<size_t>(kMaxOps) || k_model > static_cast<size_t>(kMaxModelCols) || k_aux + k_model != n_aux)
        return h->fail(SIXDOF_ERR_VALUE_SIZE_MISMATCH, "set_custom_pipe: column list does not match the generated code's layout");
    auto fold_count = reinterpret_cast<unsigned (*)()>(dlsym(dl, "sixdof_custom_fold_count"));
    auto fold_info = reinterpret_cast<int (*)(unsigned, unsigned*)>(dlsym(dl, "sixdof_custom_fold_info"));
    auto set_fold_table = reinterpret_cast<SetFoldTableFn>(dlsym(dl, "sixdof_custom_set_fold_table"));
    std::vector<FoldSlot> folds;
    if (fold_count && fold_info && set_fold_table) {
        folds.resize(fold_count());
        for (size_t k = 0; k < folds.size(); k++) {
            unsigned info[4] = {0, 0, 0, 0};
            if (fold_info(static_cast<unsigned>(k), info) != 0 || info[3] != sizeof(FoldTable))
                return h->fail(SIXDOF_ERR_BACKEND, "set_custom_pipe: the object's fold tables are not this library build's (FoldTable layout differs)");
            folds[k].needs_table = (info[0] & 1u) != 0;
            folds[k].wave_ok = (info[0] & 2u) != 0;
            folds[k].count = info[1];
            folds[k].stride = info[2];
        }
    }
    HIP_TRY(h, hipStreamSynchronize(h->stream.get()));
    h->custom_set_fold_table = folds.empty() ? nullptr : set_fold_table;
    h->custom_folds = std::move(folds);
    h->custom_dl = std::move(owned);
    h->custom_launch = launch;
    h->custom_rows_multiple = rows_multiple ? rows_multiple() : 1;
    h->custom_aux.assign(aux_ids, aux_ids + k_aux);
    h->custom_model.assign(aux_ids + k_aux, aux_ids + k_aux + k_model);
    h->custom_tick_free = ((lay >> 17) & 1u) != 0;
    h->custom_model_width.assign(k_model, 0u);
    if (col_widths && k_model) col_widths(h->custom_model_width.data());
    h->ops.clear();
    h->replay.drop();
    return SIXDOF_OK;
} SIXDOF_ABI_CATCH(err_of(h))

int sixdof_set_fold_edges(sixdof_handle* h, uint32_t fold_index, const uint64_t* from_ids, const uint64_t* to_ids, size_t n_edges) try {
    if (!h || ((!from_ids || !to_ids) && n_edges)) return SIXDOF_ERR_INVALID_ARGUMENT;
    if (!h->custom_launch) return h->fail(SIXDOF_ERR_UNSUPPORTED, "set_fold_edges: no generated program is installed (sixdof_set_custom_pipe)");
    if (!h->custom_set_fold_table)
        return h->fail(SIXDOF_ERR_UNSUPPORTED, "set_fold_edges: the installed program bakes its folds' edges into its code; build it with device fold tables");
    if (fold_index >= h->custom_folds.size())
        return h->fail(SIXDOF_ERR_INVALID_ARGUMENT, "set_fold_edges: fold_index " + std::to_string(fold_index) + " out of range (the program has " +
                       std::to_string(h->custom_folds.size()) + " fold stages)");
    FoldSlot& f = h->custom_folds[fold_index];
    if (!f.needs_table) return h->fail(SIXDOF_ERR_INVALID_ARGUMENT, "set_fold_edges: this fold stage folds the complete graph of a world: it has no edge table");
    if (!h->bound) return h->fail(SIXDOF_ERR_COMPONENT_NOT_FOUND, "set_fold_edges: bind Body columns first");
    if (n_edges > 0xFFFFFFFFull) return h->fail(SIXDOF_ERR_INVALID_ARGUMENT, "set_fold_edges: more than 2^32 - 1 edges");
    const uint64_t n = h->desc.n_entities;
    const bool replicated = f.count > 1 || f.stride > 0;
    if (replicated && static_cast<uint64_t>(f.count) * f.stride != n)
        return h->fail(SIXDOF_ERR_INVALID_ARGUMENT, "set_fold_edges: the program was generated for " + std::to_string(f.count) + " replicas of " +
                       std::to_string(f.stride) + " rows; the handle has " + std::to_string(n) + " rows");
    const uint32_t row_limit = replicated ? f.stride : static_cast<uint32_t>(std::min<uint64_t>(n, 0xFFFFFFFFull));
    std::vector<uint32_t> src, dst;
    const RowMap row_of = row_map(h->joined_ids);
    if (resolve_rows(row_of, from_ids, n_edges, &src) != n_edges || resolve_rows(row_of, to_ids, n_edges, &dst) != n_edges)
        return h->fail(SIXDOF_ERR_COMPONENT_NOT_FOUND, "set_fold_edges: edge endpoint is not an entity of this handle");
    std::vector<uint32_t> o_src(n_edges), o_start(n_edges + 1), o_dst(n_edges);
    uint32_t n_src = 0, n_lane = 0;
    const int brc = sixdof_build_fold_table(src.data(), dst.data(), n_edges, row_limit, f.wave_ok ? kFoldWaveDegree : 0u, o_src.data(),
                                            o_start.data(), o_dst.data(), &n_src, &n_lane);
    if (brc == SIXDOF_ERR_INVALID_ARGUMENT)
        return h->fail(brc, replicated ? "set_fold_edges: with replicas the edges name entities of replica 0 only" : "set_fold_edges: an edge row lies outside the handle's rows");
    if (brc != SIXDOF_OK) return h->fail(brc, "set_fold_edges: the table could not be built (out of memory)");
    std::vector<uint32_t> blob;
    blob.reserve(static_cast<size_t>(n_src) * 2 + 1 + n_edges);
    blob.insert(blob.end(), o_src.begin(), o_src.begin() + n_src);
    blob.insert(blob.end(), o_start.begin(), o_start.begin() + n_src + 1);
    blob.insert(blob.end(), o_dst.begin(), o_dst.end());
    HIP_TRY(h, hipSetDevice(h->device));
    DeviceBuffer fresh;
    HIP_TRY(h, fresh.alloc(blob.size() * sizeof(uint32_t)));
    hipError_t e = hipMemcpyAsync(fresh.get(), blob.data(), blob.size() * sizeof(uint32_t), hipMemcpyHostToDevice, h->stream.get());
    if (e == hipSuccess) e = hipStreamSynchronize(h->stream.get());
    if (e != hipSuccess) {
        (void)hipStreamSynchronize(h->stream.get());
        return h->hip_fail(e, "set_fold_edges: upload");
    }
    f.d_blob = std::move(fresh);
    const uint32_t* d_new = f.d_blob.get<uint32_t>();
    f.table.src_rows = d_new;
    f.table.row_start = d_new + n_src;
    f.table.dst = d_new + static_cast<size_t>(n_src) * 2 + 1;
    f.table.n_src = n_src;
    f.table.n_lane = n_lane;
    f.set = true;
    h->replay.drop();
    return SIXDOF_OK;
} SIXDOF_ABI_CATCH(err_of(h))

int sixdof_set_custom_pair(sixdof_handle* h, const char* so_path) try {
    if (!h || !so_path) return SIXDOF_ERR_INVALID_ARGUMENT;
    if (h->custom_launch) return h->fail(SIXDOF_ERR_UNSUPPORTED, "set_custom_pair: a generated per-entity pipe is installed; pair folds combine with built-in ops only");
    DlHandle owned;
    void* dl = *owned.out() = dlopen(so_path, RTLD_NOW | RTLD_LOCAL);
    if (!dl) return h->fail(SIXDOF_ERR_BACKEND, std::string("set_custom_pair: dlopen failed: ") + dlerror());
    auto abi = reinterpret_cast<CustomPairAbiFn>(dlsym(dl, "sixdof_custom_pair_abi"));
    auto launch = reinterpret_cast<CustomPairLaunchFn>(dlsym(dl, "sixdof_custom_pair_launch"));
    if (!abi || !launch || abi() != sizeof(PairParams))
        return h->fail(SIXDOF_ERR_BACKEND, "set_custom_pair: not a generated pair fold for this library build (PairParams layout differs)");
    h->pair_dl = std::move(owned);
    h->pair_launch = launch;
    auto only_small = reinterpret_cast<int (*)()>(dlsym(dl, "sixdof_custom_pair_only_small"));
    h->pair_only_small = only_small ? only_small() : -1;
    while (!h->ops.empty() && SIXDOF_EFF_IS_PAIR(h->ops.back().kind)) h->ops.pop_back();
    sixdof_effector_op op{};
    op.kind = SIXDOF_EFF_EDGE_CUSTOM;
// ... 583 lines not shown
            return SIXDOF_OK;
        },
        [&](const StagedRead& rd, size_t, uint64_t units, uint32_t segments, bool merge_into) -> int {
            if (events_record_bytes(units) > sc.rec.bytes()) {
                HIP_TRY(h, hipStreamSynchronize(h->stream.get()));
                HIP_TRY(h, sc.rec.alloc(static_cast<size_t>(events_record_bytes(units))));
            }
            hipError_t e = launch_history_events(a, nt, sc.rec.get(), sc.stage.get<double>(), sc.scratch.get(), segments, merge_into, n, period, first_tick, n_samples,
                                                 every, hs.ring, h->elem_size(), h->stream.get());
            if (e != hipSuccess) return h->hip_fail(e, "history_events");
            for (size_t k0 = 0; k0 < n_captures; k0 += kRingBinMaxComponents) {
                const uint32_t cnt = static_cast<uint32_t>(std::min<size_t>(kRingBinMaxComponents, n_captures - k0));
                RingBinArgs c{};
                for (uint32_t k = 0; k < cnt; k++) {
                    const StagedRead::Part& p = rd.parts[1 + k0 + k];
                    c.c[k].ring = p.ring, c.c[k].out_offset = p.offset / sizeof(double), c.c[k].w = static_cast<uint32_t>(p.w);
                }
                e = launch_events_capture(a, nt, c, cnt, sc.rec.get(), sc.stage.get<double>(), merge_into, n, period, first_tick, n_samples, every, hs.ring,
                                          h->elem_size(), h->stream.get());
                if (e != hipSuccess) return h->hip_fail(e, "history_events capture");
            }
            return SIXDOF_OK;
        });
} SIXDOF_ABI_CATCH(err_of(h))

int sixdof_download_column(sixdof_handle* h, uint64_t component_id) try {
    if (!h) return SIXDOF_ERR_INVALID_ARGUMENT;
    Column* c = h->col(component_id);
    if (!c) return h->fail(SIXDOF_ERR_COMPONENT_NOT_FOUND, "download_column: unknown component");
    HIP_TRY(h, hipSetDevice(h->device));
    int rc = scatter_back(h, c);
    if (rc != SIXDOF_OK) return rc;
    if (c->bytes) HIP_TRY(h, hipMemcpyAsync(c->host, c->dev.get(), c->bytes, hipMemcpyDeviceToHost, h->stream.get()));
    HIP_TRY(h, hipStreamSynchronize(h->stream.get()));
    return SIXDOF_OK;
} SIXDOF_ABI_CATCH(err_of(h))

int sixdof_upload_column(sixdof_handle* h, uint64_t component_id) try {
    if (!h) return SIXDOF_ERR_INVALID_ARGUMENT;
    Column* c = h->col(component_id);
    if (!c) return h->fail(SIXDOF_ERR_COMPONENT_NOT_FOUND, "upload_column: unknown component");
    if (!h->resident) return h->fail(SIXDOF_ERR_INVALID_ARGUMENT, "upload_column: nothing is resident yet (sixdof_upload first)");
    HIP_TRY(h, hipSetDevice(h->device));
    if (int rc = upload_one(h, c); rc != SIXDOF_OK) return rc;
    HIP_TRY(h, hipStreamSynchronize(h->stream.get()));
    if (component_id == h->id_accel) h->accel_is_host_data = true;
    return SIXDOF_OK;
} SIXDOF_ABI_CATCH(err_of(h))

bool graph_eligible(const sixdof_handle* h) {
    return (h->desc.flags & SIXDOF_FLAG_USE_GRAPH) && !(h->desc.flags & SIXDOF_FLAG_TIME_EACH_LAUNCH) && !h->hist.ring &&
           (h->custom_model.empty() || h->custom_tick_free) && h->model == 0 && !h->has_pair_op();
}

static bool opens_with_check(const sixdof_handle* h, uint64_t n_ticks) {
    return h->accel_is_host_data && h->desc.integrator == SIXDOF_INTEGRATOR_RK4 && n_ticks > 0;
}

static bool state_only_eligible(const sixdof_handle* h) {
    return !h->replay.state_only_off && !h->custom_launch && !h->hist.ring && h->model == 0 && !h->has_pair_op();
}

constexpr size_t kGraphCacheMax = 8;

enum class Chain : uint32_t { kAll = 0, kStateOnly = 1, kClosing = 2 };
static uint32_t graph_key(uint32_t len, Chain v) { return len << 2 | static_cast<uint32_t>(v); }

int ensure_graph(sixdof_handle* h, const StepParams& P, uint32_t len, Chain variant, hipGraphExec_t* out) {
    std::map<uint32_t, hipGraphExec_t>& graphs = h->replay.graphs;
    if (auto it = graphs.find(graph_key(len, variant)); it != graphs.end()) {
        *out = it->second;
        return SIXDOF_OK;
    }
    if (graphs.size() >= kGraphCacheMax) {
        for (auto g = graphs.begin(); g != graphs.end();) {
            if (g->first >> 2 == kGraphLen || g->first >> 2 == kGraphLong) { ++g; continue; }
            hipGraphExecDestroy(g->second);
            g = graphs.erase(g);
        }
    }
    StepParams Q = P;
    Q.state_only = variant == Chain::kAll ? 0u : 1u;
    hipGraph_t g = nullptr;
    HIP_TRY(h, hipStreamBeginCapture(h->stream.get(), hipStreamCaptureModeThreadLocal));
    hipError_t le = hipSuccess;
    for (uint32_t i = 0; i < len && le == hipSuccess; i++) {
        if (i + 1 == len && variant == Chain::kClosing) Q.state_only = 0;
        le = launch_any(h, Q);
    }
    hipError_t ce = hipStreamEndCapture(h->stream.get(), &g);
    if (le != hipSuccess) return h->hip_fail(le, "launch_step (capture)");
    if (ce != hipSuccess) return h->hip_fail(ce, "hipStreamEndCapture");
    hipGraphExec_t exec = nullptr;
    hipError_t ie = hipGraphInstantiate(&exec, g, nullptr, nullptr, 0);
    hipGraphDestroy(g);
    if (ie != hipSuccess) return h->hip_fail(ie, "hipGraphInstantiate");
    (void)hipGraphUpload(exec, h->stream.get());
    graphs[graph_key(len, variant)] = exec;
    *out = exec;
    return SIXDOF_OK;
}

struct ChainReplay {
    uint32_t len = 0;
    Chain variant = Chain::kAll;
    uint64_t times = 0;
    hipGraphExec_t graph = nullptr;
};

static int ensure_plan_graphs(sixdof_handle* h, const StepParams& P, const BatchPlan& b, ChainReplay r[5]) {
    const ChainPlan& c = b.chains;
    const Chain v = state_only_eligible(h) ? Chain::kStateOnly : Chain::kAll;
    r[0] = {kGraphLen, v, c.open ? 1u : 0u};
    r[1] = {kGraphLong, v, c.n_long};
    r[2] = {kGraphLen, v, c.n_short};
    r[3] = {c.tail, v, c.tail ? 1u : 0u};
    r[4] = {};
    if (v == Chain::kStateOnly && c.launches() && c.launches() == b.full && !b.rem) {
        int last = 3;
        while (!r[last].times) last--;
        r[last].times--;
        r[4] = {r[last].len, Chain::kClosing, 1};
    }
    for (bool tail : {false, true})
        for (int i = 0; i < 5; i++) {
            if (!r[i].times || (r[i].len != kGraphLen && r[i].len != kGraphLong) != tail) continue;
            if (int rc = ensure_graph(h, P, r[i].len, r[i].variant, &r[i].graph); rc != SIXDOF_OK) return rc;
        }
    return SIXDOF_OK;
}


constexpr size_t kAqlSlotBytes = (sizeof(StepParams) + 255) / 256 * 256;
constexpr double kAqlStallS = 60.0;

static bool aql_run(sixdof_handle* h, const StepParams& P, uint32_t check, uint32_t state_only, uint32_t ticks, aql::Run* out) {
    Replay& rp = h->replay;
    const uint64_t key = uint64_t(state_only) << 33 | uint64_t(check) << 32 | ticks;
    if (auto it = rp.aql_runs.find(key); it != rp.aql_runs.end()) return *out = it->second, true;
    uint32_t slot_index = state_only ? 2 : check;
    if (ticks != h->desc.ticks_per_launch) {
        slot_index = rp.aql_next_spare;
        rp.aql_next_spare = slot_index + 1 == kAqlSlots ? kAqlSpare0 : slot_index + 1;
        rp.aql_runs.erase(rp.aql_slot_key[slot_index]);
        rp.aql_slot_key[slot_index] = 0;
    }
    StepParams Q = P;
    Q.accel_in_check = check;
    Q.state_only = state_only;
    Q.n_ticks = ticks;
    Q.tick0 = Q.hist_slot0 = 0;
    const StepKernel k = select_step(Q, h->desc.integrator, h->desc.dtype);
    if (!k.fn) return rp.aql_why = "no built-in kernel for this launch", false;
    aql::Run r;
    if (!aql::kernel_code(rp.aql_dev, k.fn, sizeof(StepParams), &r.code, &rp.aql_why)) return false;
    if (r.code.kernarg_align > 256) return rp.aql_why = "kernarg alignment above 256 bytes", false;
    char* slot = rp.aql_args.get<char>() + slot_index * kAqlSlotBytes;
    hipError_t e = hipMemcpy(slot, &Q, sizeof(Q), hipMemcpyHostToDevice);
    if (e != hipSuccess) return rp.aql_why = std::string("hipMemcpy (argument block): ") + hipGetErrorString(e), false;
    r.kernarg = slot;
    r.blocks = k.grid.x;
    rp.aql_runs[key] = r;
    if (slot_index >= kAqlSpare0) rp.aql_slot_key[slot_index] = key;
    return *out = r, true;
}

constexpr size_t kAqlRuns = 4;

static bool aql_batch(sixdof_handle* h, const StepParams& P, const BatchPlan& b, aql::Run runs[kAqlRuns]) {
    const uint32_t K = h->desc.ticks_per_launch;
    const uint64_t closing = state_only_eligible(h) ? (b.full && !b.rem ? 1 : 0) : b.full;
    const uint64_t state_only = b.full - closing;
    if ((b.check_ticks && !aql_run(h, P, 1, 0, b.check_ticks, &runs[0])) || (state_only && !aql_run(h, P, 0, 1, K, &runs[1])) ||
        (closing && !aql_run(h, P, 0, 0, K, &runs[2])) || (b.rem && !aql_run(h, P, 0, 0, b.rem, &runs[3])))
        return false;
    runs[0].count = b.check_ticks ? 1 : 0;
    runs[1].count = state_only;
    runs[2].count = closing;
    runs[3].count = b.rem ? 1 : 0;
    return true;
}

enum class Path { kApollo, kPair, kAql, kRigid };

struct Route {
    Path path;
    const char* why = nullptr;
    int rc = SIXDOF_OK;
    BatchPlan plan{};
};

static Route choose_path(sixdof_handle* h, uint64_t n_ticks, StepParams* P, aql::Run runs[kAqlRuns]) {
    if (h->model == 1) return {Path::kApollo};
    if (h->has_pair_op()) return {Path::kPair};
    Replay& rp = h->replay;
    const bool replay = graph_eligible(h);
    const char* why = nullptr;
    if (rp.aql_off) why = "SIXDOF_AQL=0";
    else if (!replay) why = "not graph-eligible";
    else if (h->custom_launch) why = "generated pipe";
    else if (h->desc.flags & SIXDOF_FLAG_ASYNC_STEP) why = "ASYNC_STEP";
    else if (h->desc.n_entities == 0) why = "no rows";
    else if (!rp.aql_why.empty()) why = rp.aql_why.c_str();
    else if (!rp.aql_fault.empty()) return {Path::kAql};
    else if (!h->resident) why = "columns not uploaded yet";
    if (!h->bound) return {Path::kRigid, why, SIXDOF_ERR_COMPONENT_NOT_FOUND};
    if (int rc = fill_step_params(h, P); rc != SIXDOF_OK) return {Path::kRigid, why ? why : h->err.c_str(), rc};
    const uint32_t K = h->desc.ticks_per_launch;
    P->n_ticks = K;
    if (replay) rp.rekey(*P);
    const BatchPlan plan = plan_batch(n_ticks, K, opens_with_check(h, n_ticks), replay);
    if (!why && !rp.aql_dev && (rp.aql_dev = aql::acquire(h->device, &rp.aql_why))) {
        if (hipError_t e = rp.aql_args.alloc(kAqlSlots * kAqlSlotBytes); e != hipSuccess)
            rp.aql_why = std::string("hipMalloc: ") + hipGetErrorString(e);
    }
    if (!why && (!rp.aql_why.empty() || !aql_batch(h, *P, plan, runs))) why = rp.aql_why.c_str();
    return {why ? Path::kRigid : Path::kAql, why, SIXDOF_OK, plan};
}

static int prepare_batch(sixdof_handle* h, const Route& r, const StepParams& P, uint64_t n_ticks) {
    if (r.path == Path::kAql && !h->replay.aql_fault.empty()) return SIXDOF_OK;
    aql::Run runs[kAqlRuns];
    ChainReplay unused[5];
    for (bool check : {false, opens_with_check(h, n_ticks)}) {
        const BatchPlan b = plan_batch(n_ticks, h->desc.ticks_per_launch, check, true);
        if (r.path == Path::kAql) (void)aql_batch(h, P, b, runs);
        else if (int rc = ensure_plan_graphs(h, P, b, unused); rc != SIXDOF_OK) return rc;
    }
    if (r.path != Path::kAql) HIP_TRY(h, hipStreamSynchronize(h->stream.get()));
    return SIXDOF_OK;
}

int prepare_graph(sixdof_handle* h) {
    if (!h->bound || !graph_eligible(h)) return SIXDOF_OK;
    StepParams P;
    aql::Run runs[kAqlRuns];
    const Route r = choose_path(h, h->desc.ticks_per_launch, &P, runs);
    if (r.rc != SIXDOF_OK) return SIXDOF_OK;
    if (r.path == Path::kAql) return prepare_batch(h, r, P, 2 * uint64_t(h->desc.ticks_per_launch));
    hipGraphExec_t unused = nullptr;
    int rc = ensure_graph(h, P, kGraphLen, state_only_eligible(h) ? Chain::kStateOnly : Chain::kAll, &unused);
    if (rc == SIXDOF_OK) (void)hipStreamSynchronize(h->stream.get());
    return rc;
}

int sixdof_prepare_step(sixdof_handle* h, uint64_t n_ticks) try {
    if (!h) return SIXDOF_ERR_INVALID_ARGUMENT;
    if (!h->bound || !h->resident) return h->fail(SIXDOF_ERR_COMPONENT_NOT_FOUND, "prepare_step: upload the columns first");
    if (!graph_eligible(h)) return SIXDOF_OK;
    HIP_TRY(h, hipSetDevice(h->device));
    StepParams P;
    aql::Run runs[kAqlRuns];
    const Route r = choose_path(h, n_ticks, &P, runs);
    return r.rc != SIXDOF_OK ? r.rc : prepare_batch(h, r, P, n_ticks);
} SIXDOF_ABI_CATCH(err_of(h))

const char* sixdof_step_path(sixdof_handle* h) try {
    if (!h) return "invalid handle";
    (void)hipSetDevice(h->device);
    StepParams P;
    aql::Run runs[kAqlRuns];
    const Route r = choose_path(h, h->desc.ticks_per_launch, &P, runs);
    if (r.path == Path::kApollo) h->path = "apollo";
    else if (r.path == Path::kPair) h->path = "pair";
    else if (r.path == Path::kAql) h->path = h->replay.aql_fault.empty() ? "aql" : "aql (failed: " + h->replay.aql_fault + ")";
    else h->path = std::string(graph_eligible(h) ? "hipgraph: " : "eager: ") + r.why;
    return h->path.c_str();
} SIXDOF_ABI_CATCH_VALUE(err_of(h), nullptr)

static int step_pair(sixdof_handle* h, uint64_t n_ticks, uint64_t* launches) {
    if (h->desc.dtype != SIXDOF_F64) return h->fail(SIXDOF_ERR_UNSUPPORTED, "step: pair effectors are f64 only");
    PairParams P;
    int rc = fill_pair_params(h, &P);
    if (rc != SIXDOF_OK) return rc;
    const char* no_small = std::getenv("SIXDOF_PAIR_SMALL");
    const bool custom = P.pair_kind == SIXDOF_EFF_EDGE_CUSTOM;
    bool small = P.n <= kPairSmallMax && !(no_small && no_small[0] == '0');
    if (custom) {
        if (!h->pair_launch) return h->fail(SIXDOF_ERR_BACKEND, "step: custom pair op without sixdof_set_custom_pair");
        if (h->pair_only_small >= 0) small = h->pair_only_small == 1;
        if (small && P.n > kPairSmallMax)
            return h->fail(SIXDOF_ERR_INVALID_ARGUMENT, "step: the pair object was generated for the one-launch small-graph kernel (<= " +
                           std::to_string(kPairSmallMax) + " rows) but the joined graph has " + std::to_string(P.n) + " rows");
    }
    const uint32_t K = h->hist.ring ? 1u : (small ? h->desc.ticks_per_launch : 1u << 20);
    const bool sets_packed = custom || !small;
    for (uint64_t done = 0; done < n_ticks;) {
        const uint32_t k = static_cast<uint32_t>(std::min<uint64_t>(K, n_ticks - done));
        if (custom) {
            hipError_t e = static_cast<hipError_t>(h->pair_launch(&P, h->desc.integrator, k, small ? 1 : 0, h->stream.get(), launches));
            if (e != hipSuccess) return h->hip_fail(e, "custom pair launch");
        } else if (small) {
            hipError_t e = launch_pair_small(P, h->desc.integrator, k, h->stream.get(), launches);
            if (e != hipSuccess) return h->hip_fail(e, "launch_pair_small");
        } else {
            hipError_t e = launch_pair_ticks(P, h->desc.integrator, k, h->stream.get(), launches);
            if (e != hipSuccess) return h->hip_fail(e, "launch_pair_ticks");
        }
        done += k;
        if (sets_packed) P.packed = 1;
        if (int src = snapshot_tick_to_ring(h, h->tick + done); src != SIXDOF_OK) return src;
    }
    return SIXDOF_OK;
}

static int step_rigid(sixdof_handle* h, const StepParams& P, const BatchPlan& b, uint64_t n_ticks, uint64_t* launches) {
    const uint32_t K = h->desc.ticks_per_launch;
    const bool time_each = (h->desc.flags & SIXDOF_FLAG_TIME_EACH_LAUNCH) != 0;
    if (time_each) {
        const uint64_t need = 2 * b.launches();
        if (need > 8192) return h->fail(SIXDOF_ERR_INVALID_ARGUMENT, "step: TIME_EACH_LAUNCH supports <= 4096 launches per call");
        while (h->launch_events.size() < need) {
            Event e;
            HIP_TRY(h, hipEventCreate(e.out()));
            h->launch_events.push_back(std::move(e));
        }
    }
    const bool may_skip = state_only_eligible(h);
    auto eager = [&](StepParams Q, uint32_t ticks) -> int {
        Q.n_ticks = ticks;
        Q.state_only = may_skip && !Q.accel_in_check && *launches + 1 < b.launches();
        Q.tick0 = Q.hist_slot0 = h->tick + *launches * K;
        if (time_each) HIP_TRY(h, hipEventRecord(h->launch_events[2 * *launches].get(), h->stream.get()));
        hipError_t e = launch_any(h, Q);
        if (e != hipSuccess) return h->hip_fail(e, "launch_step");
        if (time_each) HIP_TRY(h, hipEventRecord(h->launch_events[2 * *launches + 1].get(), h->stream.get()));
        ++*launches;
        return SIXDOF_OK;
    };
    if (n_ticks > 0) h->accel_is_host_data = false;
    if (b.check_ticks) {
        StepParams P1 = P;
        P1.accel_in_check = 1;
        if (int rc = eager(P1, b.check_ticks); rc != SIXDOF_OK) return rc;
    }
    if (const ChainPlan& c = b.chains; c.launches()) {
        ChainReplay replays[5];
        if (int rc = ensure_plan_graphs(h, P, b, replays); rc != SIXDOF_OK) return rc;
        HIP_TRY(h, hipEventRecord(h->ev0.get(), h->stream.get()));
        for (const ChainReplay& r : replays)
            for (uint64_t i = 0; i < r.times; i++) HIP_TRY(h, hipGraphLaunch(r.graph, h->stream.get()));
        *launches += c.launches();
    }
    h->last.graph_launches = b.chains.launches();
    for (uint64_t i = b.chains.launches(); i < b.full; i++)
        if (int rc = eager(P, K); rc != SIXDOF_OK) return rc;
    return b.rem ? eager(P, b.rem) : SIXDOF_OK;
}

static int step_aql(sixdof_handle* h, const BatchPlan& b, const aql::Run runs[kAqlRuns], uint64_t n_ticks, uint64_t* launches) {
    Replay& rp = h->replay;
    if (!rp.aql_fault.empty()) return h->fail(SIXDOF_ERR_BACKEND, rp.aql_fault);
    for (hipStream_t s : {h->stream.get(), static_cast<hipStream_t>(nullptr)}) {
        const hipError_t q = hipStreamQuery(s);
        if (q == hipErrorNotReady) HIP_TRY(h, hipStreamSynchronize(s));
        else if (q != hipSuccess) return h->hip_fail(q, "hipStreamQuery");
    }
    double device_ms = 0.0;
    if (!aql::run_chain(rp.aql_dev, runs, kAqlRuns, kAqlStallS, &device_ms, &rp.aql_fault))
        return h->fail(SIXDOF_ERR_BACKEND, rp.aql_fault);
    if (n_ticks > 0) h->accel_is_host_data = false;
    *launches = b.launches();
    h->last.graph_launches = b.chains.launches();
    h->last.kernel_device_ms = device_ms;
    return SIXDOF_OK;
}

int sixdof_step(sixdof_handle* h, uint64_t n_ticks, sixdof_timings* tm) try {
    if (!h) return SIXDOF_ERR_INVALID_ARGUMENT;
    if (!h->bound) return h->fail(SIXDOF_ERR_COMPONENT_NOT_FOUND, "step: no columns bound");
    HIP_TRY(h, hipSetDevice(h->device));
    const double t0 = now_ms();
    const bool async_step = (h->desc.flags & SIXDOF_FLAG_ASYNC_STEP) != 0;
    if (h->step_pending || h->prev_pending) {
        std::swap(h->ev0, h->evp0);
        std::swap(h->ev1, h->evp1);
        std::swap(h->step_pending, h->prev_pending);
        if (h->step_pending) {
            float ms_prev = 0.f;
            HIP_TRY(h, hipEventSynchronize(h->ev1.get()));
            if (hipEventElapsedTime(&ms_prev, h->ev0.get(), h->ev1.get()) == hipSuccess) h->last.kernel_device_ms = ms_prev;
            h->step_pending = false;
        }
    }
    if (h->hist.ring && h->copy.pending && h->copy.stream_hi >= h->copy.stream_lo && n_ticks) {
        const uint64_t ring = h->hist.ring, in_flight = h->copy.stream_hi - h->copy.stream_lo + 1;
        const uint64_t a = history_slot(h->tick + 1, ring), b = history_slot(h->copy.stream_lo, ring);
        const uint64_t gap_ab = (b + ring - a) % ring, gap_ba = (a + ring - b) % ring;
        const bool overlap = n_ticks + in_flight > ring || gap_ab < std::min<uint64_t>(n_ticks, ring) || gap_ba < in_flight;
        if (overlap) HIP_TRY(h, hipStreamWaitEvent(h->stream.get(), h->copy.ev_copied.get(), 0));
    }
    if (h->desc.integrator == SIXDOF_INTEGRATOR_NONE && (!h->custom_launch || h->model != 0 || h->has_pair_op()))
        return h->fail(SIXDOF_ERR_UNSUPPORTED, "step: SIXDOF_INTEGRATOR_NONE runs generated system programs only (sixdof_set_custom_pipe)");
    uint64_t launches = 0;
    StepParams P;
    aql::Run runs[kAqlRuns];
    const Route r = choose_path(h, n_ticks, &P, runs);
    if (r.rc != SIXDOF_OK) return r.rc;
    const bool aql = r.path == Path::kAql;
    if (!aql) HIP_TRY(h, hipEventRecord(h->ev0.get(), h->stream.get()));
    const int rc = aql                       ? step_aql(h, r.plan, runs, n_ticks, &launches)
                   : r.path == Path::kApollo ? step_apollo(h, n_ticks, &launches)
                   : r.path == Path::kPair   ? step_pair(h, n_ticks, &launches)
                                             : step_rigid(h, P, r.plan, n_ticks, &launches);
    if (rc != SIXDOF_OK) return rc;
    if (!aql) HIP_TRY(h, hipEventRecord(h->ev1.get(), h->stream.get()));
    if (!async_step && !aql) {
        const double spin_until = now_ms() + 0.25;
        hipError_t q = hipEventQuery(h->ev1.get());
        while (q == hipErrorNotReady && now_ms() < spin_until) q = hipEventQuery(h->ev1.get());
        if (q != hipSuccess) {
            (void)hipGetLastError();
            HIP_TRY(h, hipStreamSynchronize(h->stream.get()));
        }
        float ms0 = 0.f;
        hipEventElapsedTime(&ms0, h->ev0.get(), h->ev1.get());
        h->last.kernel_device_ms = ms0;
    }
    h->tick += n_ticks;
    h->step_pending = async_step;
    h->last.kernel_invoke_ms = now_ms() - t0;
    h->last.launches = launches;
    h->last.ticks = n_ticks;
    h->last.kernel_sum_ms = 0.0;
    if ((h->desc.flags & SIXDOF_FLAG_TIME_EACH_LAUNCH) && !h->has_pair_op()) {
        for (uint64_t i = 0; i < launches && 2 * i + 1 < h->launch_events.size(); i++) {
            float one = 0.f;
            if (hipEventElapsedTime(&one, h->launch_events[2 * i].get(), h->launch_events[2 * i + 1].get()) == hipSuccess) h->last.kernel_sum_ms += one;
        }
    }
    if (tm) *tm = h->last;
    return SIXDOF_OK;
} SIXDOF_ABI_CATCH(err_of(h))


static thread_local sixdof_handle* g_tick_handle = nullptr;

int sixdof_tick_bind(sixdof_handle* h) try {
    g_tick_handle = h;
    return SIXDOF_OK;
} SIXDOF_ABI_CATCH(err_of(h))

static void tick_slot_ids(const sixdof_handle* h, std::vector<uint64_t>* in, std::vector<uint64_t>* out) {
    *in = {h->id_tick, h->id_force, h->id_inertia, h->id_pos, h->id_dt, h->id_vel, h->id_accel};
    for (auto& o : h->ops)
        if (o.aux_component_id) in->push_back(o.aux_component_id);
    std::map<uint64_t, int> ordered;
    for (uint64_t id : *in) ordered[id] = 1;
    out->clear();
    for (auto& kv : ordered) out->push_back(kv.first);
}

static uint64_t slot_bytes(const sixdof_handle* h, uint64_t id) {
    if (id == h->id_tick || id == h->id_dt) return 8;
    const Column* c = h->col(id);
    return c ? c->bytes : 0;
}

int sixdof_tick_slots(const sixdof_handle* h, sixdof_slot* inputs, size_t in_cap, size_t* n_in, sixdof_slot* outputs,
                      size_t out_cap, size_t* n_out) try {
    if (!h || !n_in || !n_out) return SIXDOF_ERR_INVALID_ARGUMENT;
    std::vector<uint64_t> in, out;
    tick_slot_ids(h, &in, &out);
    *n_in = in.size();
    *n_out = out.size();
    if (in_cap < in.size() || out_cap < out.size())
        return h->fail(SIXDOF_ERR_VALUE_SIZE_MISMATCH, "tick_slots: buffer too small");
    for (size_t i = 0; inputs && i < in.size(); i++) inputs[i] = {in[i], slot_bytes(h, in[i])};
    for (size_t i = 0; outputs && i < out.size(); i++) outputs[i] = {out[i], slot_bytes(h, out[i])};
    return SIXDOF_OK;
} SIXDOF_ABI_CATCH(err_of(h))

void sixdof_tick(const uint8_t* const* inputs, uint8_t* const* outputs) try {
    sixdof_handle* h = g_tick_handle;
    if (!h || !h->bound || !inputs || !outputs) return;
    if (hipSetDevice(h->device) != hipSuccess) return;
    std::vector<uint64_t> in, out;
    tick_slot_ids(h, &in, &out);
    uint64_t tick = 0;
    for (size_t i = 0; i < in.size(); i++) {
        if (in[i] == h->id_tick) std::memcpy(&tick, inputs[i], 8);
        else if (in[i] == h->id_dt) std::memcpy(&h->desc.simulation_time_step, inputs[i], 8);
// ... 24 lines not shown
```

elodin_amd/csrc/sixdof_kernels.hip:

```cpp
#include "step_kernel.hpp"

namespace sixdof {


namespace {

using PipeNone = PipeStatic<>;
using PipeGravity = PipeStatic<SIXDOF_EFF_UNIFORM_GRAVITY>;
using PipeGravityTorque = PipeStatic<SIXDOF_EFF_UNIFORM_GRAVITY, SIXDOF_EFF_BODY_TORQUE>;
using PipeGravityDrag = PipeStatic<SIXDOF_EFF_UNIFORM_GRAVITY, SIXDOF_EFF_BALL_DRAG>;
using PipeGravityThrustTorque = PipeStatic<SIXDOF_EFF_UNIFORM_GRAVITY, SIXDOF_EFF_BODY_FORCE, SIXDOF_EFF_BODY_TORQUE>;

bool kinds_are(const StepParams& p, std::initializer_list<int> kinds) {
    if (p.n_ops != kinds.size()) return false;
    uint32_t k = 0;
    for (int kind : kinds)
        if (p.ops[k++].kind != kind) return false;
    return true;
}

}

StepKernel select_step(const StepParams& p, int integrator, int dtype) {
    const dim3 grid((p.n + kWave - 1) / kWave);
    if (kinds_are(p, {})) return select_p<PipeNone>(p, integrator, dtype, grid);
    if (kinds_are(p, {SIXDOF_EFF_UNIFORM_GRAVITY})) return select_p<PipeGravity>(p, integrator, dtype, grid);
    if (kinds_are(p, {SIXDOF_EFF_UNIFORM_GRAVITY, SIXDOF_EFF_BODY_TORQUE}))
        return select_p<PipeGravityTorque, true>(p, integrator, dtype, grid);
    if (kinds_are(p, {SIXDOF_EFF_UNIFORM_GRAVITY, SIXDOF_EFF_BALL_DRAG}))
        return select_p<PipeGravityDrag>(p, integrator, dtype, grid);
    if (kinds_are(p, {SIXDOF_EFF_UNIFORM_GRAVITY, SIXDOF_EFF_BODY_FORCE, SIXDOF_EFF_BODY_TORQUE}))
        return select_p<PipeGravityThrustTorque>(p, integrator, dtype, grid);
    return select_p<PipeGeneric>(p, integrator, dtype, grid);
}

hipError_t launch_step(const StepParams& p, int integrator, int dtype, hipStream_t stream) {
    if (p.n == 0) return hipSuccess;
    const StepKernel k = select_step(p, integrator, dtype);
    if (!k.fn) return hipSuccess;
    void* args[] = {const_cast<StepParams*>(&p)};
    return hipLaunchKernel(k.fn, k.grid, dim3(kWave), args, 0, stream);
}

}
```

elodin_amd/csrc/step_kernel.hpp:

```cpp
#pragma once
#include <type_traits>

#include "effectors.hpp"
#include "kernels.hpp"
#include "spatial.hpp"

namespace sixdof {

constexpr int kWave = 64;

typedef __attribute__((address_space(1))) const void* global_cptr;
typedef __attribute__((address_space(3))) void* lds_ptr;


constexpr int kPolPlain = 0, kPolNtStores = 1, kPolSc1Stores = 2, kPolNt = 9;
constexpr int pol_ld(int pol) { return pol / 8; }
constexpr int pol_st(int pol) { return pol % 8; }

template <int BYTES, int POL>
__device__ __forceinline__ void slab_dma_in(const char* __restrict__ g, char* l, uint32_t lane) {
    constexpr int kFull = BYTES / 1024, kRem = (BYTES % 1024) / 16;
    constexpr int kAux = pol_ld(POL) == 1 ? 2 : 0;
#pragma unroll
    for (int i = 0; i < kFull; i++)
        __builtin_amdgcn_global_load_lds((global_cptr)(g + i * 1024 + lane * 16), (lds_ptr)(l + i * 1024), 16, 0,
                                         kAux);
    if (kRem && lane < (uint32_t)kRem)
        __builtin_amdgcn_global_load_lds((global_cptr)(g + kFull * 1024 + lane * 16), (lds_ptr)(l + kFull * 1024), 16,
                                         0, kAux);
}

typedef float vfloat4 __attribute__((ext_vector_type(4)));
template <int POL>
__device__ __forceinline__ void store16(char* g, vfloat4 v) {
    constexpr int ST = pol_st(POL);
    if constexpr (ST == 1) __builtin_nontemporal_store(v, reinterpret_cast<vfloat4*>(g));
    else if constexpr (ST == 2) asm volatile("global_store_dwordx4 %0, %1, off sc1" ::"v"(g), "v"(v) : "memory");
    else if constexpr (ST == 3) asm volatile("global_store_dwordx4 %0, %1, off sc0 sc1" ::"v"(g), "v"(v) : "memory");
    else if constexpr (ST == 4) asm volatile("global_store_dwordx4 %0, %1, off sc1 nt" ::"v"(g), "v"(v) : "memory");
    else *reinterpret_cast<vfloat4*>(g) = v;
}
template <int BYTES, int NT>
__device__ __forceinline__ void slab_out(const char* l, char* __restrict__ g, uint32_t lane) {
    constexpr int kFull = BYTES / 1024, kRem = (BYTES % 1024) / 16;
    vfloat4 tmp[kFull + 1];
#pragma unroll
    for (int i = 0; i < kFull; i++) tmp[i] = *reinterpret_cast<const vfloat4*>(l + i * 1024 + lane * 16);
    if (kRem && lane < (uint32_t)kRem) tmp[kFull] = *reinterpret_cast<const vfloat4*>(l + kFull * 1024 + lane * 16);
#pragma unroll
    for (int i = 0; i < kFull; i++) store16<NT>(g + i * 1024 + lane * 16, tmp[i]);
    if (kRem && lane < (uint32_t)kRem) store16<NT>(g + kFull * 1024 + lane * 16, tmp[kFull]);
}

template <class T>
__device__ __forceinline__ void slab_in_tail(const T* __restrict__ g, T* l, uint32_t count, uint32_t lane) {
    for (uint32_t e = lane; e < count; e += kWave) l[e] = g[e];
}
template <class T>
__device__ __forceinline__ void slab_out_tail(const T* l, T* __restrict__ g, uint32_t count, uint32_t lane) {
    for (uint32_t e = lane; e < count; e += kWave) g[e] = l[e];
}

template <int POL, class T>
__device__ __forceinline__ T col_ld(const T* p) {
    if constexpr (pol_ld(POL) == 1) return __builtin_nontemporal_load(p);
    else return *p;
}
template <int POL, class T>
__device__ __forceinline__ void col_st(T* p, T v) {
    if constexpr (pol_st(POL) == 1) __builtin_nontemporal_store(v, p);
    else *p = v;
}



template <class PIPE, int K, bool WIDTH>
struct OpArgs {
    int32_t kind, aux_width;
    const void* aux;
    double p[6];
};
template <class PIPE, int K, bool WIDTH>
__device__ __forceinline__ OpArgs<PIPE, K, WIDTH> op_args(const StepParams& P) {
    OpArgs<PIPE, K, WIDTH> o{};
    if constexpr (!PIPE::kStatic) o.kind = P.ops[K].kind;
    if constexpr (WIDTH) o.aux_width = P.ops[K].aux_width;
    if constexpr (PIPE::template uses_aux<K>()) o.aux = P.ops[K].aux;
#pragma unroll
    for (int j = 0; j < PIPE::template n_params<K>(); j++) o.p[j] = P.ops[K].p[j];
    return o;
}
struct NotRead {};
template <bool READ, class V>
__device__ __forceinline__ auto arg_if(const V& v) {
    if constexpr (READ) return v;
    else return NotRead{};
}
template <class V>
__device__ __forceinline__ void hold_in_sgpr(V v) {
    asm volatile("" ::"s"(v));
}
__device__ __forceinline__ void hold_in_sgpr(NotRead) {}
template <class PIPE, int K, bool WIDTH>
__device__ __forceinline__ void hold_in_sgpr(OpArgs<PIPE, K, WIDTH> o) {
    if constexpr (!PIPE::kStatic) hold_in_sgpr(o.kind);
    if constexpr (WIDTH) hold_in_sgpr(o.aux_width);
    if constexpr (PIPE::template uses_aux<K>()) hold_in_sgpr(o.aux);
#pragma unroll
    for (int j = 0; j < PIPE::template n_params<K>(); j++) hold_in_sgpr(o.p[j]);
}
template <class... V>
__device__ __forceinline__ void hold_in_sgprs(V... v) {
    (hold_in_sgpr(v), ...);
}
template <class PIPE, bool CHECK, bool WIDTH>
__device__ __forceinline__ void read_entry_args(const StepParams& P) {
    hold_in_sgprs(P.n_ticks, P.n_ops, P.streaming, P.state_only, P.dt_g, P.dt, arg_if<!PIPE::kStatic>(P.vel_independent),
                  arg_if<CHECK>(P.accel_in_check),
                  P.hist_pos, P.hist_ring, P.hist_slot0, P.hist_vel, P.hist_accel, P.hist_force,
                  op_args<PIPE, 0, WIDTH>(P), op_args<PIPE, 1, WIDTH>(P), op_args<PIPE, 2, WIDTH>(P), op_args<PIPE, 3, WIDTH>(P));
}


template <class T, int INTEGRATOR, class PIPE, int POL, bool CHECK = false, int ROWS = kWave>
__global__ __launch_bounds__(kWave) void sixdof_step_kernel(const StepParams P) {
    __shared__ __attribute__((aligned(16))) T lds[ROWS * 25];
    T* const l_pos = lds;
    T* const l_vel = lds + ROWS * 7;
    T* const l_c = lds + ROWS * 13;
    T* const l_force = lds + ROWS * 19;

    const uint32_t row0 = blockIdx.x * ROWS;
    const uint32_t rows = min((uint32_t)ROWS, P.n - row0);
    const uint32_t t = threadIdx.x;
    const bool full = rows == ROWS;

    T* const g_pos = static_cast<T*>(P.pos) + (size_t)row0 * 7;
    T* const g_vel = static_cast<T*>(P.vel) + (size_t)row0 * 6;
    T* const g_accel = static_cast<T*>(P.accel) + (size_t)row0 * 6;
    T* const g_force = static_cast<T*>(P.force) + (size_t)row0 * 6;
    const T* const g_inertia = static_cast<const T*>(P.inertia) + (size_t)row0 * 7;

    constexpr bool kEntryArgs = PIPE::kBuiltIn && (PIPE::kStatic || INTEGRATOR == kRk4);
    constexpr bool kAuxRows3 = kEntryArgs && (PIPE::kStatic || sizeof(T) == 8);
    if constexpr (kEntryArgs) read_entry_args<PIPE, CHECK, !kAuxRows3>(P);

    constexpr bool kDead = INTEGRATOR == kNone && PIPE::kBodyDead;
    if constexpr (!kDead) {
        if (full) {
            slab_dma_in<ROWS * 7 * sizeof(T), POL>(reinterpret_cast<const char*>(g_pos), reinterpret_cast<char*>(l_pos), t);
            slab_dma_in<ROWS * 6 * sizeof(T), POL>(reinterpret_cast<const char*>(g_vel), reinterpret_cast<char*>(l_vel), t);
            slab_dma_in<ROWS * 7 * sizeof(T), POL>(reinterpret_cast<const char*>(g_inertia), reinterpret_cast<char*>(l_c), t);
        } else {
            slab_in_tail(g_pos, l_pos, rows * 7, t);
            slab_in_tail(g_vel, l_vel, rows * 6, t);
            slab_in_tail(g_inertia, l_c, rows * 7, t);
        }
    }

    const bool active = t < rows;
    Vec3<T> aux[kMaxOps];
#pragma unroll
    for (int k = 0; k < kMaxOps; k++) aux[k] = Vec3<T>{T(0), T(0), T(0)};
    auto load_aux = [&](auto kc) {
        constexpr int k = decltype(kc)::value;
        if constexpr (PIPE::template uses_aux<k>()) {
            if (k < (int)P.n_ops && P.ops[k].aux != nullptr && active) {
                if constexpr (!kAuxRows3) {
                    const int w = P.ops[k].aux_width ? P.ops[k].aux_width : 3;
                    const T* a = static_cast<const T*>(P.ops[k].aux) + (size_t)(row0 + t) * w;
                    aux[k] = Vec3<T>{a[0], w > 1 ? a[1] : T(0), w > 2 ? a[2] : T(0)};
                } else {
                    const T* a = static_cast<const T*>(P.ops[k].aux) + (size_t)(row0 + t) * 3;
                    aux[k] = Vec3<T>{a[0], a[1], a[2]};
                }
            }
        }
    };
    load_aux(std::integral_constant<int, 0>{});
    load_aux(std::integral_constant<int, 1>{});
    load_aux(std::integral_constant<int, 2>{});
    load_aux(std::integral_constant<int, 3>{});

    typename PIPE::template Regs<T> regs;
    if constexpr (PIPE::kHasModel) PIPE::template load<T, POL>(P, row0 + t, active, regs);

    asm volatile("s_waitcnt vmcnt(0)" ::: "memory");
    __syncthreads();

    const Spatial<T> zero6 = {{T(0), T(0), T(0)}, {T(0), T(0), T(0)}};
    Quat<T> q0 = {T(0), T(0), T(0), T(1)};
    Vec3<T> p0 = {T(0), T(0), T(0)}, inv_I = {T(1), T(1), T(1)}, I_diag = {T(1), T(1), T(1)};
    Spatial<T> v0 = zero6, A_out = zero6, F_out = zero6;
    T mass = T(1), inv_m = T(1);
    if (active && !kDead) {
        const T* r = l_pos + t * 7;
        q0 = Quat<T>{r[0], r[1], r[2], r[3]};
        p0 = Vec3<T>{r[4], r[5], r[6]};
        const T* s = l_vel + t * 6;
        v0.ang = Vec3<T>{s[0], s[1], s[2]};
        v0.lin = Vec3<T>{s[3], s[4], s[5]};
        const T* m = l_c + t * 7;
        I_diag = Vec3<T>{m[0], m[1], m[2]};
        inv_I = Vec3<T>{recip(m[0]), recip(m[1]), recip(m[2])};
        mass = m[6];
        inv_m = recip(mass);
        if constexpr (INTEGRATOR == kNone || PIPE::kPreReadsAccel) {
            const T* a = g_accel + (size_t)t * 6;
            A_out = Spatial<T>{{a[0], a[1], a[2]}, {a[3], a[4], a[5]}};
        }
        if constexpr (INTEGRATOR == kNone) {
            const T* f = g_force + (size_t)t * 6;
            F_out = Spatial<T>{{f[0], f[1], f[2]}, {f[3], f[4], f[5]}};
        }
    }
    if (P.n_ticks == 0) return;
    __syncthreads();

    auto stage_pos = [&](const Quat<T>& q, const Vec3<T>& p) {
        if (active) {
            T* r = l_pos + t * 7;
            r[0] = q.i; r[1] = q.j; r[2] = q.k; r[3] = q.w; r[4] = p.x; r[5] = p.y; r[6] = p.z;
        }
    };
    auto stage6 = [&](T* l, const Spatial<T>& m) {
        if (active) {
            T* s = l + t * 6;
            s[0] = m.ang.x; s[1] = m.ang.y; s[2] = m.ang.z; s[3] = m.lin.x; s[4] = m.lin.y; s[5] = m.lin.z;
        }
    };
    auto flush7 = [&](const T* l, T* o, auto pol) {
        if (full) slab_out<ROWS * 7 * sizeof(T), decltype(pol)::value>(reinterpret_cast<const char*>(l), reinterpret_cast<char*>(o), t);
        else slab_out_tail(l, o, rows * 7, t);
    };
    auto flush6 = [&](const T* l, T* o, auto pol) {
        if (full) slab_out<ROWS * 6 * sizeof(T), decltype(pol)::value>(reinterpret_cast<const char*>(l), reinterpret_cast<char*>(o), t);
        else slab_out_tail(l, o, rows * 6, t);
    };
    constexpr std::integral_constant<int, POL> kLive{};
    constexpr std::integral_constant<int, 1> kRing{};

    const bool record = P.hist_pos != nullptr && P.hist_ring != 0;
    const bool early_ok = !PIPE::kHasModel && !record && !(P.streaming & 256u);
    const bool state_only = !PIPE::kHasModel && P.state_only != 0;
    const T dt_g = T(P.dt_g), dt = T(P.dt);
    Body<T> b;
    b.mass = mass;
    b.I = I_diag;
    Wrench<T> F = zero_wrench<T>();
    bool flushed = false;
#ifdef SIXDOF_TICK_OUT_OF_LINE
    auto one_tick = [&](auto early_tag, auto check_tag, uint32_t tick) __attribute__((noinline)) {
#else
    auto one_tick = [&](auto early_tag, auto check_tag, uint32_t tick) {
#endif
        constexpr bool early = decltype(early_tag)::value;
        const bool check = decltype(check_tag)::value || (PIPE::kHasModel && P.accel_in_check && tick == 0);
        if constexpr (PIPE::kHasModel) {
            PIPE::pre(P, P.tick0 + tick + 1, regs, q0, p0, v0, I_diag, mass, A_out);
            if constexpr (PIPE::kWritesInertia) {
                inv_I = Vec3<T>{recip(I_diag.x), recip(I_diag.y), recip(I_diag.z)};
                inv_m = recip(mass);
                b.mass = mass;
                b.I = I_diag;
            }
        }
        if constexpr (INTEGRATOR == kRk4) {
            const T h1 = dt_g * T(0.5), h3 = dt_g;
            Spatial<T> A, sv, sa;
            b.q = normalized(q0);
            b.p = p0;
            b.v = v0;
            if (check && active) {
                const T* a = g_accel + (size_t)t * 6;
                b.v.ang = b.v.ang + T(0) * Vec3<T>{a[0], a[1], a[2]};
                b.v.lin = b.v.lin + T(0) * Vec3<T>{a[3], a[4], a[5]};
            }
            F = zero_wrench<T>();
            PIPE::apply(P, aux, regs, b, F);
            A = calc_accel<PIPE>(b.q, F, inv_I, inv_m, T(0));
            sv = b.v;
            sa = A;
            b.q = integrate_world(q0, h1 * v0.ang);
            b.p = axpy(h1, v0.lin, p0);
            b.v = axpy(h1, A, v0);
            sv = axpy(T(2), b.v, sv);
            F = zero_wrench<T>();
            PIPE::apply(P, aux, regs, b, F);
            A = calc_accel<PIPE>(b.q, F, inv_I, inv_m, T(0));
            sa = axpy(T(2), A, sa);
            b.v = axpy(h1, A, v0);
            sv = axpy(T(2), b.v, sv);
            if (!PIPE::vel_independent(P)) {
                F = zero_wrench<T>();
                PIPE::apply(P, aux, regs, b, F);
                A = calc_accel<PIPE>(b.q, F, inv_I, inv_m, T(0));
            }
            sa = axpy(T(2), A, sa);
            T n3;
            b.q = integrate_world(q0, h3 * v0.ang, &n3);
            const T taint = accel_taint(n3);
            b.p = axpy(h3, v0.lin, p0);
            b.v = axpy(PIPE::vel_independent(P) ? h3 : h3 + taint, A, v0);
            sv = sv + b.v;
            const T g = dt * T(1.0 / 6.0);
            const Quat<T> q_new = integrate_world(q0, g * sv.ang);
            const Vec3<T> p_new = axpy(g + taint, sv.lin, p0);
            if constexpr (early) {
                stage_pos(q_new, p_new);
                __syncthreads();
                flush7(l_pos, g_pos, kLive);
            }
            F = zero_wrench<T>();
            PIPE::apply(P, aux, regs, b, F);
            if constexpr (early) {
                if (!state_only) {
                    stage6(l_force, world_wrench<PIPE>(b.q, F));
                    __syncthreads();
                    flush6(l_force, g_force, kLive);
                }
            }
            A = calc_accel<PIPE>(b.q, F, inv_I, inv_m + taint, taint);
            if constexpr (early) {
                if (!state_only) {
                    stage6(l_c, A);
                    __syncthreads();
                    flush6(l_c, g_accel, kLive);
                }
            }
            sa = sa + A;
            v0 = axpy(g, sa, v0);
            q0 = q_new;
            p0 = p_new;
            A_out = A;
            if constexpr (early) {
                stage6(l_vel, v0);
                __syncthreads();
                flush6(l_vel, g_vel, kLive);
                flushed = true;
            }
        } else if constexpr (INTEGRATOR == kNone) {
        } else {
            T n0;
            b.q = normalized(q0, &n0);
            const T taint = accel_taint(n0);
            b.p = p0;
            b.v = v0;
            F = zero_wrench<T>();
            PIPE::apply(P, aux, regs, b, F);
            if constexpr (early) {
                if (!state_only) {
                    stage6(l_force, world_wrench<PIPE>(b.q, F));
                    __syncthreads();
                    flush6(l_force, g_force, kLive);
                }
            }
            const Spatial<T> A = calc_accel<PIPE>(b.q, F, inv_I, inv_m + taint, taint);
            if constexpr (early) {
                if (!state_only) {
                    stage6(l_c, A);
                    __syncthreads();
                    flush6(l_c, g_accel, kLive);
                }
            }
            v0 = axpy(dt, A, v0);
            if constexpr (early) {
                stage6(l_vel, v0);
                __syncthreads();
                flush6(l_vel, g_vel, kLive);
            }
            q0 = integrate_world(q0, dt * v0.ang);
            p0 = axpy(dt, v0.lin, p0);
            A_out = A;
            if constexpr (early) {
                stage_pos(q0, p0);
                __syncthreads();
                flush7(l_pos, g_pos, kLive);
                flushed = true;
            }
        }
        if constexpr (PIPE::kHasModel) PIPE::post(P, P.tick0 + tick + 1, regs, q0, p0, v0, I_diag, mass, A_out);
        if (record) {
            if constexpr (INTEGRATOR != kNone) F_out = world_wrench<PIPE>(b.q, F);
            const size_t slot = (size_t)((P.hist_slot0 + tick) % P.hist_ring);
            if constexpr (!kDead) {
                stage_pos(q0, p0);
                stage6(l_vel, v0);
                stage6(l_c, A_out);
                stage6(l_force, F_out);
                __syncthreads();
                const size_t r7 = (slot * P.n + row0) * 7, r6 = (slot * P.n + row0) * 6;
                flush7(l_pos, static_cast<T*>(P.hist_pos) + r7, kRing);
                flush6(l_vel, static_cast<T*>(P.hist_vel) + r6, kRing);
                flush6(l_c, static_cast<T*>(P.hist_accel) + r6, kRing);
                flush6(l_force, static_cast<T*>(P.hist_force) + r6, kRing);
            }
            if constexpr (PIPE::kHasModel)
                if (active) PIPE::record(P, slot, row0 + t, regs);
            __syncthreads();
        }
    };
    {
        constexpr std::false_type no{};
        constexpr std::true_type yes{};
        uint32_t tick = 0;
        if constexpr (PIPE::kHasModel) {
            for (; tick < P.n_ticks; tick++) one_tick(no, no, tick);
        } else {
            if constexpr (INTEGRATOR == kRk4 && CHECK)
                if (P.accel_in_check && P.n_ticks) one_tick(no, yes, tick++);
            for (; tick + 1 < P.n_ticks; tick++) one_tick(no, no, tick);
            if (tick < P.n_ticks) {
                if (early_ok) one_tick(yes, no, tick);
                else one_tick(no, no, tick);
            }
        }
    }
    if constexpr (PIPE::kHasModel) {
        if (active) {
            PIPE::template store<T, POL>(P, row0 + t, regs);
            if constexpr (PIPE::kWritesInertia) {
                T* gi = static_cast<T*>(const_cast<void*>(P.inertia)) + (size_t)(row0 + t) * 7;
                gi[0] = I_diag.x; gi[1] = I_diag.y; gi[2] = I_diag.z; gi[6] = mass;
            }
        }
    }
    if (flushed || kDead) return;
    stage_pos(q0, p0);
    stage6(l_vel, v0);
    if (!state_only) {
        if constexpr (INTEGRATOR != kNone) F_out = world_wrench<PIPE>(b.q, F);
        stage6(l_c, A_out);
        stage6(l_force, F_out);
    }
    __syncthreads();
    flush7(l_pos, g_pos, kLive);
    flush6(l_vel, g_vel, kLive);
    if (state_only) return;
    flush6(l_c, g_accel, kLive);
    flush6(l_force, g_force, kLive);
}


template <class T, class PIPE, int POL>
inline StepKernel select_i(const StepParams& p, int integrator, dim3 grid) {
#ifdef SIXDOF_AB_BUILD
    if constexpr (!PIPE::kHasModel) {
        if ((p.streaming & 512u) && integrator == kRk4 && !p.accel_in_check)
            return {reinterpret_cast<const void*>(&sixdof_step_kernel<T, kRk4, PIPE, POL, false, 32>), dim3((p.n + 31) / 32)};
    }
#endif
    if (integrator == kRk4) {
        if constexpr (!PIPE::kHasModel) {
            if (p.accel_in_check)
                return {reinterpret_cast<const void*>(&sixdof_step_kernel<T, kRk4, PIPE, kPolPlain, true>), grid};
        }
        return {reinterpret_cast<const void*>(&sixdof_step_kernel<T, kRk4, PIPE, POL>), grid};
    }
    if (integrator == kNone) {
        if constexpr (PIPE::kHasModel) return {reinterpret_cast<const void*>(&sixdof_step_kernel<T, kNone, PIPE, POL>), grid};
        return {};
    }
    return {reinterpret_cast<const void*>(&sixdof_step_kernel<T, kSemiImplicit, PIPE, POL>), grid};
}

template <class T, class PIPE, bool SWEEP>
inline StepKernel select_t(const StepParams& p, int integrator, dim3 grid) {
    const uint32_t pol = p.streaming & 255u;
    switch (pol) {
    case kPolNt: return select_i<T, PIPE, kPolNt>(p, integrator, grid);
    case kPolNtStores: return select_i<T, PIPE, kPolNtStores>(p, integrator, grid);
    default: break;
    }
#ifdef SIXDOF_AB_BUILD
    if (pol == kPolSc1Stores) return select_i<T, PIPE, kPolSc1Stores>(p, integrator, grid);
    if constexpr (SWEEP) {
        switch (pol) {
        case 3: return select_i<T, PIPE, 3>(p, integrator, grid);
        case 4: return select_i<T, PIPE, 4>(p, integrator, grid);
        case 8: return select_i<T, PIPE, 8>(p, integrator, grid);
        case 10: return select_i<T, PIPE, 10>(p, integrator, grid);
        case 11: return select_i<T, PIPE, 11>(p, integrator, grid);
        case 12: return select_i<T, PIPE, 12>(p, integrator, grid);
        default: break;
        }
    }
#endif
    return select_i<T, PIPE, kPolPlain>(p, integrator, grid);
}

template <class PIPE, bool SWEEP = false>
inline StepKernel select_p(const StepParams& p, int integrator, int dtype, dim3 grid) {
    if (dtype == SIXDOF_F64) return select_t<double, PIPE, SWEEP>(p, integrator, grid);
    return select_t<float, PIPE, false>(p, integrator, grid);
}

}
```

profiles/summarize.py:

```python
#!/usr/bin/env python3
import csv
import glob
import json
import sys
from collections import defaultdict

out, tag = sys.argv[1], sys.argv[2]


def rows(pattern):
    for f in glob.glob(pattern, recursive=True):
        with open(f, newline="") as fh:
            yield from csv.DictReader(fh)


stats = defaultdict(list)
for r in rows(f"{out}/trace/**/*kernel_trace.csv"):
    grid = int(r.get("Grid_Size_X") or r.get("Grid_Size") or 0)
    dur = int(r["End_Timestamp"]) - int(r["Start_Timestamp"])
    stats[(r["Kernel_Name"], grid)].append(dur)

lines = [f"# rocprofv3 --kernel-trace --stats summary ({tag})", "",
         "Command: `python bench.py --steps 2048 --warmup 128 --no-cpu-baseline --extras --skip-legs telemetry_commit,history_stream,monte_carlo_example,world_module,build` (profiles/collect.sh).",
         "Durations in microseconds; `grid` = total work-items (= entities for the step kernel). The 65536-entity",
         "step kernel appears with ticks_per_launch = 1 (timed region + warmup), = 64 (`fused`) and = 64 with the",
         "telemetry ring (`recording`): rows are split by duration.  PipeStatic<2, 3> = gravity | body_torque;",
         "the trailing int is the cache-policy code of the instantiation (load * 8 + store: 1 = plain loads + nt stores,",
         "2 = plain loads + sc1 stores, 9 = nt both ways; csrc/step_kernel.hpp); PipeCustom = a generated pipe / program",
         "(`<float, 1, PipeCustom, 1>` at grid 32768 = the Falcon 9 ascent campaign, 1000 ticks per launch).", "",
         "| kernel | grid | launches | avg us | min us | max us | total ms |", "|---|---|---|---|---|---|---|"]
for (name, grid), d in sorted(stats.items(), key=lambda kv: -sum(kv[1])):
    groups = [("", d)]
    if "sixdof_step_kernel" in name and grid == 65536:
        groups = [(" [1 tick/launch]", [x for x in d if x < 15000]),
                  (" [8 ticks/launch, `telemetry_commit` leg]", [x for x in d if 15000 <= x < 30000]),
                  (" [64 ticks/launch]", [x for x in d if 30000 <= x < 80000]),
                  (" [64 ticks/launch + telemetry ring]", [x for x in d if x >= 80000])]
    for label, g in groups:
        if g:
            lines.append(f"| `{name}`{label} | {grid} | {len(g)} | {sum(g)/len(g)/1e3:.3f} | {min(g)/1e3:.3f} | "
                         f"{max(g)/1e3:.3f} | {sum(g)/1e6:.3f} |")

pmc = defaultdict(lambda: defaultdict(list))
for which in ("fetch", "write"):
    for r in rows(f"{out}/pmc_{which}_*/**/*counter_collection.csv"):
        if "sixdof_step_kernel" not in r["Kernel_Name"]:
            continue
        grid = int(r.get("Grid_Size") or 0)
        pmc[grid][r["Counter_Name"]].append(float(r["Counter_Value"]))
traffic = {}
lines += ["", "## HBM traffic per launch (separate --pmc passes)", "",
          "| entities | FETCH_SIZE KiB (raw) | read bytes (x2, gfx950) | WRITE_SIZE KiB | write bytes | total bytes | algorithmic (384 B/entity) |",
          "|---|---|---|---|---|---|---|"]
for grid, c in sorted(pmc.items()):
    if "FETCH_SIZE" in c and "WRITE_SIZE" in c:
        f = sum(c["FETCH_SIZE"]) / len(c["FETCH_SIZE"])
        w = sum(c["WRITE_SIZE"]) / len(c["WRITE_SIZE"])
        rd, wr = 2 * f * 1024, w * 1024
        traffic[str(grid)] = {"fetch_size_kib_raw": f, "write_size_kib": w, "read_bytes": rd, "write_bytes": wr,
                              "hbm_bytes_per_launch": rd + wr, "correction": "FETCH_SIZE x2 (gfx950), KiB units"}
        lines.append(f"| {grid} | {f:.1f} | {rd:.0f} | {w:.1f} | {wr:.0f} | {rd+wr:.0f} | {384*grid} |")
import hashlib
import os
from pathlib import Path
root = Path(__file__).resolve().parent.parent
h = hashlib.sha256()
for name in ("step_kernel.hpp", "effectors.hpp", "spatial.hpp", "kernels.hpp", "sixdof_kernels.hip"):
    h.update((root / "elodin_amd" / "csrc" / name).read_bytes())
traffic["_stamp"] = {"step_kernel_hash": h.hexdigest()[:16], "tag": tag, "commit": os.environ.get("SIXDOF_COMMIT", "unknown (no .git on the GPU box)")}
open(f"{out}/summary_{tag}.md", "w").write("\n".join(lines) + "\n")
json.dump(traffic, open(f"{out}/pmc_traffic.json", "w"), indent=1)
print("\n".join(lines))
```

Before: 16.02 billion.

## Add specialized one-tick kernel with preloaded kernarg block and cached inverse inertia

Adds a dedicated sixdof_tick_kernel for single-tick RK4 launches with static pipes. It takes a compact TickBlock argument layout so the leading fields can be preloaded, instead of the full StepParams struct. It also adds an optional cached buffer of inverse inertia rows, filled by a small kernel whenever inertia is marked dirty. The aim is to cut kernarg load cost and per-entity divisions in one-tick dispatches, at the price of more kernel instantiations, dirty-flag bookkeeping and a fallback path. The inverse cache is off unless SIXDOF_TICK_INVERSE=1.

```diff
diff --git a/elodin_amd/codegen.py b/elodin_amd/codegen.py
--- a/elodin_amd/codegen.py
+++ b/elodin_amd/codegen.py
@@ -1596,7 +1596,7 @@
 
 def _headers_digest() -> str:
     h = hashlib.sha1()
-    for name in ("step_kernel.hpp", "pair_kernel.hpp", "effectors.hpp", "spatial.hpp", "kernels.hpp"):
+    for name in ("step_kernel.hpp", "step_body.hpp", "pair_kernel.hpp", "effectors.hpp", "spatial.hpp", "kernels.hpp"):
         h.update((CSRC / name).read_bytes())
     h.update((PKG.parent / "include" / "sixdof_hip.h").read_bytes())
     return h.hexdigest()
diff --git a/elodin_amd/csrc/aql_chain.cpp b/elodin_amd/csrc/aql_chain.cpp
--- a/elodin_amd/csrc/aql_chain.cpp
+++ b/elodin_amd/csrc/aql_chain.cpp
@@ -223,9 +223,7 @@
         if (s == HSA_STATUS_SUCCESS) s = hsa_executable_symbol_get_info(sym, HSA_EXECUTABLE_SYMBOL_INFO_KERNEL_PRIVATE_SEGMENT_SIZE, &k.private_size);
         if (s == HSA_STATUS_SUCCESS) s = hsa_executable_symbol_get_info(sym, HSA_EXECUTABLE_SYMBOL_INFO_KERNEL_DYNAMIC_CALLSTACK, &dynamic_stack);
         if (s != HSA_STATUS_SUCCESS) return *why = hsa_error("hsa_executable_symbol_get_info", s), false;
-        if (k.kernarg_size != explicit_kernarg_bytes)
-            return *why = name + ": kernarg segment of " + std::to_string(k.kernarg_size) + " bytes, " +
-                          std::to_string(explicit_kernarg_bytes) + " explicit (hidden arguments)", false;
+        if (!explicit_arguments_only(name, k.kernarg_size, explicit_kernarg_bytes, why)) return false;
         if (dynamic_stack) return *why = name + ": dynamic call stack", false;
         d->kernels[stub] = k;
         return *out = k, true;
diff --git a/elodin_amd/csrc/aql_chain.hpp b/elodin_amd/csrc/aql_chain.hpp
--- a/elodin_amd/csrc/aql_chain.hpp
+++ b/elodin_amd/csrc/aql_chain.hpp
@@ -25,6 +25,8 @@
 
 void fill_body(hsa_kernel_dispatch_packet_t* p, const KernelCode& k, uint32_t blocks, const void* kernarg, hsa_signal_t signal);
 
+bool explicit_arguments_only(const std::string& kernel, uint32_t segment_bytes, uint32_t explicit_bytes, std::string* why);
+
 struct Ring {
     hsa_kernel_dispatch_packet_t* base = nullptr;
     uint64_t size = 0;
diff --git a/elodin_amd/csrc/aql_packets.cpp b/elodin_amd/csrc/aql_packets.cpp
--- a/elodin_amd/csrc/aql_packets.cpp
+++ b/elodin_amd/csrc/aql_packets.cpp
@@ -63,4 +63,11 @@
     return true;
 }
 
+bool explicit_arguments_only(const std::string& kernel, uint32_t segment_bytes, uint32_t explicit_bytes, std::string* why) {
+    if (segment_bytes == explicit_bytes) return true;
+    *why = kernel + ": kernarg segment of " + std::to_string(segment_bytes) + " bytes, " + std::to_string(explicit_bytes) +
+           (segment_bytes > explicit_bytes ? " explicit (hidden arguments)" : " in the host's argument block");
+    return false;
 }
+
+}
diff --git a/elodin_amd/csrc/hip_fake.cpp b/elodin_amd/csrc/hip_fake.cpp
--- a/elodin_amd/csrc/hip_fake.cpp
+++ b/elodin_amd/csrc/hip_fake.cpp
@@ -58,6 +58,8 @@
 bool fired() { return g_fired; }
 long calls() { return g_calls; }
 long violations() { return g_violations; }
+static long g_fills = 0;
+long fills() { return g_fills; }
 size_t live_allocations() { return g_allocs.size(); }
 size_t live_streams() { return g_streams.size(); }
 size_t live_events() { return g_events.size(); }
@@ -396,9 +398,39 @@
 }
 
 StepKernel select_step(const StepParams&, int, int) { return {}; }
-hipError_t launch_step(const StepParams& p, int integrator, int dtype, hipStream_t s) {
-    if (deferring()) return defer(s, "launch_step", {p.pos, p.vel, p.accel, p.force, p.hist_pos, p.hist_vel, p.hist_accel, p.hist_force}, [=] { return launch_step(p, integrator, dtype, s); });
-    const bool ok = step_ok(p, dtype);
+template <class T>
+static bool inverse_is(const void* inertia, const void* inv, size_t n) {
+    const T* m = static_cast<const T*>(inertia);
+    const T* o = static_cast<const T*>(inv);
+    for (size_t i = 0; i < n; i++) {
+        const T want[4] = {T(1) / m[i * 7], T(1) / m[i * 7 + 1], T(1) / m[i * 7 + 2], T(1) / m[i * 7 + 6]};
+        if (std::memcmp(want, o + i * 4, sizeof(want)) != 0) return false;
+    }
+    return true;
+}
+hipError_t launch_fill_inverse(const void* inertia, void* inv, uint32_t n, int dtype, hipStream_t s) {
+    if (deferring()) return defer(s, "launch_fill_inverse", {inertia, inv}, [=] { return launch_fill_inverse(inertia, inv, n, dtype, s); });
+    const size_t es = dtype == 1 ? 4 : 8;
+    const bool ok = need(live(inertia, size_t(n) * 7 * es), "inertia (fill)") & need(live(inv, size_t(n) * 4 * es), "inverse rows (fill)");
+    if (ok) {
+        hip_fake::g_fills++;
+        for (size_t i = 0; i < n; i++)
+            for (int j = 0; j < 4; j++) {
+                const size_t src = i * 7 + (j < 3 ? j : 6);
+                if (dtype == 1) static_cast<float*>(inv)[i * 4 + j] = 1.0f / static_cast<const float*>(inertia)[src];
+                else static_cast<double*>(inv)[i * 4 + j] = 1.0 / static_cast<const double*>(inertia)[src];
+            }
+    }
+    return launch(ok);
+}
+hipError_t launch_step(const StepParams& p, int integrator, int dtype, hipStream_t s, const void* inv) {
+    if (deferring()) return defer(s, "launch_step", {p.pos, p.vel, p.accel, p.force, p.hist_pos, p.hist_vel, p.hist_accel, p.hist_force, inv}, [=] { return launch_step(p, integrator, dtype, s, inv); });
+    bool ok = step_ok(p, dtype);
+    if (ok && inv) {
+        const size_t es = dtype == 1 ? 4 : 8;
+        ok = need(live(inv, size_t(p.n) * 4 * es), "inverse rows") &&
+             need(dtype == 1 ? inverse_is<float>(p.inertia, inv, p.n) : inverse_is<double>(p.inertia, inv, p.n), "inverse rows are stale: a write of the inertia column did not set the dirty flag");
+    }
     if (ok && p.hist_ring && p.hist_pos) {
         const size_t es = dtype == 1 ? 4 : 8;
         const void* live_col[4] = {p.pos, p.vel, p.accel, p.force};
diff --git a/elodin_amd/csrc/kernels.hpp b/elodin_amd/csrc/kernels.hpp
--- a/elodin_amd/csrc/kernels.hpp
+++ b/elodin_amd/csrc/kernels.hpp
@@ -1,5 +1,6 @@
 #pragma once
 #include <hip/hip_runtime.h>
+#include <stddef.h>
 #include <stdint.h>
 
 #pragma clang fp contract(on)
@@ -46,14 +47,58 @@
 
 enum : int { kRk4 = 0, kSemiImplicit = 1, kNone = 2 };
 
+constexpr uint32_t kStreamingKeepStepKernel = 1024u;
+
+constexpr int kTickAux = 2;
+struct TickTail {
+    void* accel;
+    void* force;
+    double dt_g, dt;
+    uint32_t streaming;
+    uint32_t reserved;
+    double p[kMaxOps][6];
+};
+struct TickBlock {
+    void* pos;
+    void* vel;
+    const void* inertia;
+    const void* inv;
+    const void* aux[kTickAux];
+    uint32_t n;
+    uint32_t state_only;
+    TickTail tail;
+};
+static_assert(offsetof(TickBlock, pos) == 0 && offsetof(TickBlock, vel) == 8 && offsetof(TickBlock, inertia) == 16, "TickBlock layout");
+static_assert(offsetof(TickBlock, inv) == 24 && offsetof(TickBlock, aux) == 32 && offsetof(TickBlock, n) == 48 && offsetof(TickBlock, state_only) == 52, "TickBlock layout");
+static_assert(offsetof(TickBlock, tail) == 56 && sizeof(TickBlock) == 56 + sizeof(TickTail), "TickBlock layout");
+static_assert(offsetof(TickTail, accel) == 0 && offsetof(TickTail, force) == 8 && offsetof(TickTail, dt_g) == 16 && offsetof(TickTail, dt) == 24, "TickTail layout");
+static_assert(offsetof(TickTail, streaming) == 32 && offsetof(TickTail, p) == 40 && sizeof(TickTail) == 40 + kMaxOps * 48, "TickTail layout");
+constexpr uint32_t kTickPreloadDwords = offsetof(TickBlock, tail) / 4;
+
 struct StepKernel {
     const void* fn = nullptr;
     dim3 grid;
-};
+    bool tick = false;
+    int tick_aux[kTickAux] = {-1, -1};
+};
+
+inline TickBlock tick_block(const StepParams& p, const StepKernel& k, const void* inv) {
+    TickBlock b{};
+    b.pos = p.pos, b.vel = p.vel, b.inertia = p.inertia, b.inv = inv;
+    for (int j = 0; j < kTickAux; j++)
+        if (k.tick_aux[j] >= 0) b.aux[j] = p.ops[k.tick_aux[j]].aux;
+    b.n = p.n, b.state_only = p.state_only;
+    b.tail.accel = p.accel, b.tail.force = p.force, b.tail.dt_g = p.dt_g, b.tail.dt = p.dt, b.tail.streaming = p.streaming;
+    for (int o = 0; o < kMaxOps; o++)
+        for (int j = 0; j < 6; j++) b.tail.p[o][j] = p.ops[o].p[j];
+    return b;
+}
 
 StepKernel select_step(const StepParams& p, int integrator, int dtype);
-
-hipError_t launch_step(const StepParams& p, int integrator, int dtype, hipStream_t stream);
+StepKernel select_tick(const StepParams& p, int integrator, int dtype);
+
+hipError_t launch_step(const StepParams& p, int integrator, int dtype, hipStream_t stream, const void* inv);
+hipError_t launch_fill_inverse(const void* inertia, void* inv, uint32_t n, int dtype, hipStream_t stream);
 
 using CustomAbiFn = unsigned (*)();
 using CustomLayoutFn = unsigned (*)();
diff --git a/elodin_amd/csrc/sixdof_capi.cpp b/elodin_amd/csrc/sixdof_capi.cpp
--- a/elodin_amd/csrc/sixdof_capi.cpp
+++ b/elodin_amd/csrc/sixdof_capi.cpp
@@ -92,6 +92,10 @@
     std::map<uint32_t, hipGraphExec_t> graphs;
     bool state_only_off = false;
     bool aql_off = false;
+    std::string tick_off;
+    DeviceBuffer inv_rows;
+    bool inv_dirty = true, inv_exposed = false;
+    bool inv_off = true;
     aql::Device* aql_dev = nullptr;
     std::string aql_why;
     std::string aql_fault;
@@ -348,6 +352,7 @@
 }
 
 static int gather_joined(sixdof_handle* h, Column* c) {
+    h->replay.inv_dirty = true;
     if (!c->joined || !c->compact) return SIXDOF_OK;
     hipError_t e = launch_gather_rows(c->compact.get(), c->dev.get(), c->d_rows.get<uint32_t>(), static_cast<uint32_t>(h->joined_ids.size()),
                                       static_cast<uint32_t>(c->width), c->elem, h->stream.get());
@@ -361,6 +366,7 @@
 }
 
 static int upload_one(sixdof_handle* h, Column* c) {
+    h->replay.inv_dirty = true;
     if (c->bytes) HIP_TRY(h, hipMemcpyAsync(c->dev.get(), c->host, c->bytes, hipMemcpyHostToDevice, h->stream.get()));
     return gather_joined(h, c);
 }
@@ -421,6 +427,10 @@
     h->replay.aql_off = aql_env && aql_env[0] == '0';
     const char* so_env = std::getenv("SIXDOF_STATE_ONLY");
     h->replay.state_only_off = so_env && so_env[0] == '0';
+    const char* tick_env = std::getenv("SIXDOF_TICK_KERNEL");
+    if (tick_env && tick_env[0] == '0') h->replay.tick_off = "SIXDOF_TICK_KERNEL=0";
+    const char* inv_env = std::getenv("SIXDOF_TICK_INVERSE");
+    h->replay.inv_off = !(inv_env && inv_env[0] == '1');
     h->device = d->device_ordinal;
     for (BodyCol& b : h->body) b.id = cid(b.name);
     h->id_pos = h->body[0].id, h->id_vel = h->body[1].id, h->id_accel = h->body[2].id, h->id_force = h->body[3].id;
@@ -517,6 +527,7 @@
         if (rc != SIXDOF_OK) return rc;
     }
     h->bound = true;
+    h->replay.inv_dirty = true;
     return SIXDOF_OK;
 } SIXDOF_ABI_CATCH(err_of(h))
 
@@ -752,6 +763,7 @@
 void* sixdof_device_column(sixdof_handle* h, uint64_t component_id) try {
     if (!h) return nullptr;
     Column* c = h->col(component_id);
+    if (c && component_id == h->id_inertia) h->replay.inv_exposed = true;
     return c ? (c->live ? c->live : c->dev.get()) : nullptr;
 } SIXDOF_ABI_CATCH_VALUE(err_of(h), nullptr)
 void* sixdof_stream(sixdof_handle* h) { return h ? static_cast<void*>(h->stream.get()) : nullptr; }
@@ -830,6 +842,7 @@
         if ((code & ~0x1ffu) == 0 && (pol == 0u || pol == 1u || pol == 9u)) policy = code;
 #endif
     }
+    if (!h->replay.tick_off.empty()) policy |= kStreamingKeepStepKernel;
     P->streaming = policy;
     P->hist_ring = h->hist.ring;
     if (h->hist.ring) {
@@ -865,6 +878,28 @@
 
 size_t align_up(size_t x, size_t a) { return (x + a - 1) / a * a; }
 
+const void* inverse_rows(sixdof_handle* h) {
+    Replay& rp = h->replay;
+    if (rp.inv_off || h->custom_launch || h->hist.ring || h->model != 0 || h->has_pair_op() || h->desc.integrator != SIXDOF_INTEGRATOR_RK4 ||
+        h->desc.n_entities == 0)
+        return nullptr;
+    if (!rp.inv_rows) {
+        if (rp.inv_rows.alloc(static_cast<size_t>(h->desc.n_entities) * 4 * h->elem_size()) != hipSuccess) return rp.inv_off = true, nullptr;
+        rp.inv_dirty = true;
+    }
+    return rp.inv_rows.get();
+}
+
+int ensure_inverse(sixdof_handle* h, const StepParams& P) {
+    Replay& rp = h->replay;
+    void* inv = const_cast<void*>(inverse_rows(h));
+    if (!inv || !(rp.inv_dirty || rp.inv_exposed)) return SIXDOF_OK;
+    hipError_t e = launch_fill_inverse(P.inertia, inv, P.n, h->desc.dtype, h->stream.get());
+    if (e != hipSuccess) return h->hip_fail(e, "launch_fill_inverse");
+    rp.inv_dirty = false;
+    return SIXDOF_OK;
+}
+
 hipError_t launch_any(sixdof_handle* h, const StepParams& P) {
     if (h->desc.integrator == SIXDOF_INTEGRATOR_NONE && !h->custom_launch) return hipErrorInvalidValue;
     if (h->custom_launch) {
@@ -872,7 +907,7 @@
             if (h->custom_folds[k].needs_table) h->custom_set_fold_table(static_cast<unsigned>(k), h->custom_folds[k].set ? &h->custom_folds[k].table : nullptr);
         return static_cast<hipError_t>(h->custom_launch(&P, h->desc.integrator, h->desc.dtype, h->stream.get()));
     }
-    return launch_step(P, h->desc.integrator, h->desc.dtype, h->stream.get());
+    return launch_step(P, h->desc.integrator, h->desc.dtype, h->stream.get(), inverse_rows(h));
 }
 
 int fill_pair_params(sixdof_handle* h, PairParams* P) {
@@ -1037,6 +1072,7 @@
     h->ap_ticks_per_telemetry = t->ticks_per_telemetry ? t->ticks_per_telemetry : 3;
     h->ap_max_ticks = t->max_ticks;
     h->model = 1;
+    h->replay.inv_dirty = true;
     return SIXDOF_OK;
 } SIXDOF_ABI_CATCH(err_of(h))
 
@@ -1110,6 +1146,7 @@
     h->custom_folds = std::move(folds);
     h->custom_dl = std::move(owned);
     h->custom_launch = launch;
+    h->replay.inv_dirty = true;
     h->custom_rows_multiple = rows_multiple ? rows_multiple() : 1;
     h->custom_aux.assign(aux_ids, aux_ids + k_aux);
     h->custom_model.assign(aux_ids + k_aux, aux_ids + k_aux + k_model);
@@ -1859,6 +1896,7 @@
     StepParams Q = P;
     Q.state_only = variant == Chain::kAll ? 0u : 1u;
     hipGraph_t g = nullptr;
+    (void)inverse_rows(h);
     HIP_TRY(h, hipStreamBeginCapture(h->stream.get(), hipStreamCaptureModeThreadLocal));
     hipError_t le = hipSuccess;
     for (uint32_t i = 0; i < len && le == hipSuccess; i++) {
@@ -1909,6 +1947,7 @@
 
 
 constexpr size_t kAqlSlotBytes = (sizeof(StepParams) + 255) / 256 * 256;
+static_assert(sizeof(TickBlock) <= kAqlSlotBytes, "a slot holds either argument block");
 constexpr double kAqlStallS = 60.0;
 
 static bool aql_run(sixdof_handle* h, const StepParams& P, uint32_t check, uint32_t state_only, uint32_t ticks, aql::Run* out) {
@@ -1927,13 +1966,19 @@
     Q.state_only = state_only;
     Q.n_ticks = ticks;
     Q.tick0 = Q.hist_slot0 = 0;
-    const StepKernel k = select_step(Q, h->desc.integrator, h->desc.dtype);
+    if (!rp.tick_off.empty()) Q.streaming |= kStreamingKeepStepKernel;
+    StepKernel k = select_step(Q, h->desc.integrator, h->desc.dtype);
     if (!k.fn) return rp.aql_why = "no built-in kernel for this launch", false;
     aql::Run r;
-    if (!aql::kernel_code(rp.aql_dev, k.fn, sizeof(StepParams), &r.code, &rp.aql_why)) return false;
+    if (k.tick && !aql::kernel_code(rp.aql_dev, k.fn, sizeof(TickBlock), &r.code, &rp.tick_off)) {
+        Q.streaming |= kStreamingKeepStepKernel;
+        k = select_step(Q, h->desc.integrator, h->desc.dtype);
+    }
+    if (!k.tick && !aql::kernel_code(rp.aql_dev, k.fn, sizeof(StepParams), &r.code, &rp.aql_why)) return false;
     if (r.code.kernarg_align > 256) return rp.aql_why = "kernarg alignment above 256 bytes", false;
     char* slot = rp.aql_args.get<char>() + slot_index * kAqlSlotBytes;
-    hipError_t e = hipMemcpy(slot, &Q, sizeof(Q), hipMemcpyHostToDevice);
+    const TickBlock block = k.tick ? tick_block(Q, k, inverse_rows(h)) : TickBlock{};
+    hipError_t e = k.tick ? hipMemcpy(slot, &block, sizeof(block), hipMemcpyHostToDevice) : hipMemcpy(slot, &Q, sizeof(Q), hipMemcpyHostToDevice);
     if (e != hipSuccess) return rp.aql_why = std::string("hipMemcpy (argument block): ") + hipGetErrorString(e), false;
     r.kernarg = slot;
     r.blocks = k.grid.x;
@@ -2042,6 +2087,7 @@
     else if (r.path == Path::kPair) h->path = "pair";
     else if (r.path == Path::kAql) h->path = h->replay.aql_fault.empty() ? "aql" : "aql (failed: " + h->replay.aql_fault + ")";
     else h->path = std::string(graph_eligible(h) ? "hipgraph: " : "eager: ") + r.why;
+    if ((r.path == Path::kAql || r.path == Path::kRigid) && !h->replay.tick_off.empty()) h->path += "; one-tick launches: sixdof_step_kernel (" + h->replay.tick_off + ")";
     return h->path.c_str();
 } SIXDOF_ABI_CATCH_VALUE(err_of(h), nullptr)
 
@@ -2175,6 +2221,12 @@
     const Route r = choose_path(h, n_ticks, &P, runs);
     if (r.rc != SIXDOF_OK) return r.rc;
     const bool aql = r.path == Path::kAql;
+    if (aql || r.path == Path::kRigid) {
+        if (int irc = ensure_inverse(h, P); irc != SIXDOF_OK) return irc;
+    } else if (r.path == Path::kApollo) {
+        h->replay.inv_dirty = true;
+    }
+    if (h->custom_launch) h->replay.inv_dirty = true;
     if (!aql) HIP_TRY(h, hipEventRecord(h->ev0.get(), h->stream.get()));
     const int rc = aql                       ? step_aql(h, r.plan, runs, n_ticks, &launches)
                    : r.path == Path::kApollo ? step_apollo(h, n_ticks, &launches)
diff --git a/elodin_amd/csrc/sixdof_kernels.hip b/elodin_amd/csrc/sixdof_kernels.hip
--- a/elodin_amd/csrc/sixdof_kernels.hip
+++ b/elodin_amd/csrc/sixdof_kernels.hip
@@ -3,25 +3,8 @@
 namespace sixdof {
 
 
-namespace {
-
-using PipeNone = PipeStatic<>;
-using PipeGravity = PipeStatic<SIXDOF_EFF_UNIFORM_GRAVITY>;
-using PipeGravityTorque = PipeStatic<SIXDOF_EFF_UNIFORM_GRAVITY, SIXDOF_EFF_BODY_TORQUE>;
-using PipeGravityDrag = PipeStatic<SIXDOF_EFF_UNIFORM_GRAVITY, SIXDOF_EFF_BALL_DRAG>;
-using PipeGravityThrustTorque = PipeStatic<SIXDOF_EFF_UNIFORM_GRAVITY, SIXDOF_EFF_BODY_FORCE, SIXDOF_EFF_BODY_TORQUE>;
-
-bool kinds_are(const StepParams& p, std::initializer_list<int> kinds) {
-    if (p.n_ops != kinds.size()) return false;
-    uint32_t k = 0;
-    for (int kind : kinds)
-        if (p.ops[k++].kind != kind) return false;
-    return true;
-}
-
-}
-
 StepKernel select_step(const StepParams& p, int integrator, int dtype) {
+    if (const StepKernel k = select_tick(p, integrator, dtype); k.fn) return k;
     const dim3 grid((p.n + kWave - 1) / kWave);
     if (kinds_are(p, {})) return select_p<PipeNone>(p, integrator, dtype, grid);
     if (kinds_are(p, {SIXDOF_EFF_UNIFORM_GRAVITY})) return select_p<PipeGravity>(p, integrator, dtype, grid);
@@ -34,10 +17,15 @@
     return select_p<PipeGeneric>(p, integrator, dtype, grid);
 }
 
-hipError_t launch_step(const StepParams& p, int integrator, int dtype, hipStream_t stream) {
+hipError_t launch_step(const StepParams& p, int integrator, int dtype, hipStream_t stream, const void* inv) {
     if (p.n == 0) return hipSuccess;
     const StepKernel k = select_step(p, integrator, dtype);
     if (!k.fn) return hipSuccess;
+    if (k.tick) {
+        TickBlock b = tick_block(p, k, inv);
+        void* args[] = {&b.pos, &b.vel, &b.inertia, &b.inv, &b.aux[0], &b.aux[1], &b.n, &b.state_only, &b.tail};
+        return hipLaunchKernel(k.fn, k.grid, dim3(kWave), args, 0, stream);
+    }
     void* args[] = {const_cast<StepParams*>(&p)};
     return hipLaunchKernel(k.fn, k.grid, dim3(kWave), args, 0, stream);
 }
diff --git a/elodin_amd/csrc/step_body.hpp b/elodin_amd/csrc/step_body.hpp
--- /dev/null
+++ b/elodin_amd/csrc/step_body.hpp
@@ -0,0 +1,358 @@
+    __shared__ __attribute__((aligned(16))) T lds[ROWS * 25];
+    T* const l_pos = lds;
+    T* const l_vel = lds + ROWS * 7;
+    T* const l_c = lds + ROWS * 13;
+    T* const l_force = lds + ROWS * 19;
+
+    const uint32_t row0 = blockIdx.x * ROWS;
+    const uint32_t rows = min((uint32_t)ROWS, P.n - row0);
+    const uint32_t t = threadIdx.x;
+    const bool full = rows == ROWS;
+
+    T* const g_pos = static_cast<T*>(P.pos) + (size_t)row0 * 7;
+    T* const g_vel = static_cast<T*>(P.vel) + (size_t)row0 * 6;
+    T* const g_accel = static_cast<T*>(P.accel) + (size_t)row0 * 6;
+    T* const g_force = static_cast<T*>(P.force) + (size_t)row0 * 6;
+    const T* const g_inertia = static_cast<const T*>(P.inertia) + (size_t)row0 * 7;
+
+    constexpr bool kEntryArgs = PIPE::kBuiltIn && (PIPE::kStatic || INTEGRATOR == kRk4);
+    constexpr bool kAuxRows3 = kEntryArgs && (PIPE::kStatic || sizeof(T) == 8);
+#ifndef SIXDOF_TICK_ENTRY
+    if constexpr (kEntryArgs) read_entry_args<PIPE, CHECK, !kAuxRows3>(P);
+#endif
+
+    constexpr bool kDead = INTEGRATOR == kNone && PIPE::kBodyDead;
+    if constexpr (!kDead) {
+        if (full) {
+            slab_dma_in<ROWS * 7 * sizeof(T), POL>(reinterpret_cast<const char*>(g_pos), reinterpret_cast<char*>(l_pos), t);
+            slab_dma_in<ROWS * 6 * sizeof(T), POL>(reinterpret_cast<const char*>(g_vel), reinterpret_cast<char*>(l_vel), t);
+            slab_dma_in<ROWS * 7 * sizeof(T), POL>(reinterpret_cast<const char*>(g_inertia), reinterpret_cast<char*>(l_c), t);
+        } else {
+            slab_in_tail(g_pos, l_pos, rows * 7, t);
+            slab_in_tail(g_vel, l_vel, rows * 6, t);
+            slab_in_tail(g_inertia, l_c, rows * 7, t);
+        }
+    }
+
+    const bool active = t < rows;
+    Vec3<T> aux[kMaxOps];
+#pragma unroll
+    for (int k = 0; k < kMaxOps; k++) aux[k] = Vec3<T>{T(0), T(0), T(0)};
+    auto load_aux = [&](auto kc) {
+        constexpr int k = decltype(kc)::value;
+#ifdef SIXDOF_TICK_ENTRY
+        if constexpr (PIPE::template uses_aux<k>()) {
+            const uint32_t row = min(row0 + t, P.n - 1);
+            const T* a = P.ops[k].aux != nullptr ? static_cast<const T*>(P.ops[k].aux) + (size_t)row * 3 : static_cast<const T*>(P.pos) + (size_t)row * 7;
+            aux[k] = Vec3<T>{a[0], a[1], a[2]};
+        }
+#else
+        if constexpr (PIPE::template uses_aux<k>()) {
+            if (k < (int)P.n_ops && P.ops[k].aux != nullptr && active) {
+                if constexpr (!kAuxRows3) {
+                    const int w = P.ops[k].aux_width ? P.ops[k].aux_width : 3;
+                    const T* a = static_cast<const T*>(P.ops[k].aux) + (size_t)(row0 + t) * w;
+                    aux[k] = Vec3<T>{a[0], w > 1 ? a[1] : T(0), w > 2 ? a[2] : T(0)};
+                } else {
+                    const T* a = static_cast<const T*>(P.ops[k].aux) + (size_t)(row0 + t) * 3;
+                    aux[k] = Vec3<T>{a[0], a[1], a[2]};
+                }
+            }
+        }
+#endif
+    };
+    load_aux(std::integral_constant<int, 0>{});
+    load_aux(std::integral_constant<int, 1>{});
+    load_aux(std::integral_constant<int, 2>{});
+    load_aux(std::integral_constant<int, 3>{});
+
+    typename PIPE::template Regs<T> regs;
+    if constexpr (PIPE::kHasModel) PIPE::template load<T, POL>(P, row0 + t, active, regs);
+
+#ifdef SIXDOF_TICK_ENTRY
+    T inv_row[4];
+    {
+        const uint32_t row = min(row0 + t, P.n - 1);
+        const T* a = inv_rows != nullptr ? static_cast<const T*>(inv_rows) + (size_t)row * 4 : static_cast<const T*>(P.pos) + (size_t)row * 7;
+        inv_row[0] = a[0], inv_row[1] = a[1], inv_row[2] = a[2], inv_row[3] = a[3];
+    }
+#endif
+
+    asm volatile("s_waitcnt vmcnt(0)" ::: "memory");
+    __syncthreads();
+#ifdef SIXDOF_TICK_ENTRY
+    {
+        auto aux_absent = [&](auto kc) {
+            constexpr int k = decltype(kc)::value;
+            if constexpr (PIPE::template uses_aux<k>())
+                if (P.ops[k].aux == nullptr || !active) aux[k] = Vec3<T>{T(0), T(0), T(0)};
+        };
+        aux_absent(std::integral_constant<int, 0>{});
+        aux_absent(std::integral_constant<int, 1>{});
+        aux_absent(std::integral_constant<int, 2>{});
+        aux_absent(std::integral_constant<int, 3>{});
+    }
+#endif
+
+    const Spatial<T> zero6 = {{T(0), T(0), T(0)}, {T(0), T(0), T(0)}};
+    Quat<T> q0 = {T(0), T(0), T(0), T(1)};
+    Vec3<T> p0 = {T(0), T(0), T(0)}, inv_I = {T(1), T(1), T(1)}, I_diag = {T(1), T(1), T(1)};
+    Spatial<T> v0 = zero6, A_out = zero6, F_out = zero6;
+    T mass = T(1), inv_m = T(1);
+    if (active && !kDead) {
+        const T* r = l_pos + t * 7;
+        q0 = Quat<T>{r[0], r[1], r[2], r[3]};
+        p0 = Vec3<T>{r[4], r[5], r[6]};
+        const T* s = l_vel + t * 6;
+        v0.ang = Vec3<T>{s[0], s[1], s[2]};
+        v0.lin = Vec3<T>{s[3], s[4], s[5]};
+        const T* m = l_c + t * 7;
+        I_diag = Vec3<T>{m[0], m[1], m[2]};
+#ifdef SIXDOF_TICK_ENTRY
+        mass = m[6];
+        if (inv_rows != nullptr) {
+            inv_I = Vec3<T>{inv_row[0], inv_row[1], inv_row[2]};
+            inv_m = inv_row[3];
+        } else {
+            inv_I = Vec3<T>{recip(m[0]), recip(m[1]), recip(m[2])};
+            inv_m = recip(mass);
+        }
+#else
+        inv_I = Vec3<T>{recip(m[0]), recip(m[1]), recip(m[2])};
+        mass = m[6];
+        inv_m = recip(mass);
+#endif
+        if constexpr (INTEGRATOR == kNone || PIPE::kPreReadsAccel) {
+            const T* a = g_accel + (size_t)t * 6;
+            A_out = Spatial<T>{{a[0], a[1], a[2]}, {a[3], a[4], a[5]}};
+        }
+        if constexpr (INTEGRATOR == kNone) {
+            const T* f = g_force + (size_t)t * 6;
+            F_out = Spatial<T>{{f[0], f[1], f[2]}, {f[3], f[4], f[5]}};
+        }
+    }
+    if (P.n_ticks == 0) return;
+    __syncthreads();
+
+    auto stage_pos = [&](const Quat<T>& q, const Vec3<T>& p) {
+        if (active) {
+            T* r = l_pos + t * 7;
+            r[0] = q.i; r[1] = q.j; r[2] = q.k; r[3] = q.w; r[4] = p.x; r[5] = p.y; r[6] = p.z;
+        }
+    };
+    auto stage6 = [&](T* l, const Spatial<T>& m) {
+        if (active) {
+            T* s = l + t * 6;
+            s[0] = m.ang.x; s[1] = m.ang.y; s[2] = m.ang.z; s[3] = m.lin.x; s[4] = m.lin.y; s[5] = m.lin.z;
+        }
+    };
+    auto flush7 = [&](const T* l, T* o, auto pol) {
+        if (full) slab_out<ROWS * 7 * sizeof(T), decltype(pol)::value>(reinterpret_cast<const char*>(l), reinterpret_cast<char*>(o), t);
+        else slab_out_tail(l, o, rows * 7, t);
+    };
+    auto flush6 = [&](const T* l, T* o, auto pol) {
+        if (full) slab_out<ROWS * 6 * sizeof(T), decltype(pol)::value>(reinterpret_cast<const char*>(l), reinterpret_cast<char*>(o), t);
+        else slab_out_tail(l, o, rows * 6, t);
+    };
+    constexpr std::integral_constant<int, POL> kLive{};
+    constexpr std::integral_constant<int, 1> kRing{};
+
+    const bool record = P.hist_pos != nullptr && P.hist_ring != 0;
+    const bool early_ok = !PIPE::kHasModel && !record && !(P.streaming & 256u);
+    const bool state_only = !PIPE::kHasModel && P.state_only != 0;
+    const T dt_g = T(P.dt_g), dt = T(P.dt);
+    Body<T> b;
+    b.mass = mass;
+    b.I = I_diag;
+    Wrench<T> F = zero_wrench<T>();
+    bool flushed = false;
+#ifdef SIXDOF_TICK_OUT_OF_LINE
+    auto one_tick = [&](auto early_tag, auto check_tag, uint32_t tick) __attribute__((noinline)) {
+#else
+    auto one_tick = [&](auto early_tag, auto check_tag, uint32_t tick) {
+#endif
+        constexpr bool early = decltype(early_tag)::value;
+        const bool check = decltype(check_tag)::value || (PIPE::kHasModel && P.accel_in_check && tick == 0);
+        if constexpr (PIPE::kHasModel) {
+            PIPE::pre(P, P.tick0 + tick + 1, regs, q0, p0, v0, I_diag, mass, A_out);
+            if constexpr (PIPE::kWritesInertia) {
+                inv_I = Vec3<T>{recip(I_diag.x), recip(I_diag.y), recip(I_diag.z)};
+                inv_m = recip(mass);
+                b.mass = mass;
+                b.I = I_diag;
+            }
+        }
+        if constexpr (INTEGRATOR == kRk4) {
+            const T h1 = dt_g * T(0.5), h3 = dt_g;
+            Spatial<T> A, sv, sa;
+            b.q = normalized(q0);
+            b.p = p0;
+            b.v = v0;
+            if (check && active) {
+                const T* a = g_accel + (size_t)t * 6;
+                b.v.ang = b.v.ang + T(0) * Vec3<T>{a[0], a[1], a[2]};
+                b.v.lin = b.v.lin + T(0) * Vec3<T>{a[3], a[4], a[5]};
+            }
+            F = zero_wrench<T>();
+            PIPE::apply(P, aux, regs, b, F);
+            A = calc_accel<PIPE>(b.q, F, inv_I, inv_m, T(0));
+            sv = b.v;
+            sa = A;
+            b.q = integrate_world(q0, h1 * v0.ang);
+            b.p = axpy(h1, v0.lin, p0);
+            b.v = axpy(h1, A, v0);
+            sv = axpy(T(2), b.v, sv);
+            F = zero_wrench<T>();
+            PIPE::apply(P, aux, regs, b, F);
+            A = calc_accel<PIPE>(b.q, F, inv_I, inv_m, T(0));
+            sa = axpy(T(2), A, sa);
+            b.v = axpy(h1, A, v0);
+            sv = axpy(T(2), b.v, sv);
+            if (!PIPE::vel_independent(P)) {
+                F = zero_wrench<T>();
+                PIPE::apply(P, aux, regs, b, F);
+                A = calc_accel<PIPE>(b.q, F, inv_I, inv_m, T(0));
+            }
+            sa = axpy(T(2), A, sa);
+            T n3;
+            b.q = integrate_world(q0, h3 * v0.ang, &n3);
+            const T taint = accel_taint(n3);
+            b.p = axpy(h3, v0.lin, p0);
+            b.v = axpy(PIPE::vel_independent(P) ? h3 : h3 + taint, A, v0);
+            sv = sv + b.v;
+            const T g = dt * T(1.0 / 6.0);
+            const Quat<T> q_new = integrate_world(q0, g * sv.ang);
+            const Vec3<T> p_new = axpy(g + taint, sv.lin, p0);
+            if constexpr (early) {
+                stage_pos(q_new, p_new);
+                __syncthreads();
+                flush7(l_pos, g_pos, kLive);
+            }
+            F = zero_wrench<T>();
+            PIPE::apply(P, aux, regs, b, F);
+            if constexpr (early) {
+                if (!state_only) {
+                    stage6(l_force, world_wrench<PIPE>(b.q, F));
+                    __syncthreads();
+                    flush6(l_force, g_force, kLive);
+                }
+            }
+            A = calc_accel<PIPE>(b.q, F, inv_I, inv_m + taint, taint);
+            if constexpr (early) {
+                if (!state_only) {
+                    stage6(l_c, A);
+                    __syncthreads();
+                    flush6(l_c, g_accel, kLive);
+                }
+            }
+            sa = sa + A;
+            v0 = axpy(g, sa, v0);
+            q0 = q_new;
+            p0 = p_new;
+            A_out = A;
+            if constexpr (early) {
+                stage6(l_vel, v0);
+                __syncthreads();
+                flush6(l_vel, g_vel, kLive);
+                flushed = true;
+            }
+        } else if constexpr (INTEGRATOR == kNone) {
+        } else {
+            T n0;
+            b.q = normalized(q0, &n0);
+            const T taint = accel_taint(n0);
+            b.p = p0;
+            b.v = v0;
+            F = zero_wrench<T>();
+            PIPE::apply(P, aux, regs, b, F);
+            if constexpr (early) {
+                if (!state_only) {
+                    stage6(l_force, world_wrench<PIPE>(b.q, F));
+                    __syncthreads();
+                    flush6(l_force, g_force, kLive);
+                }
+            }
+            const Spatial<T> A = calc_accel<PIPE>(b.q, F, inv_I, inv_m + taint, taint);
+            if constexpr (early) {
+                if (!state_only) {
+                    stage6(l_c, A);
+                    __syncthreads();
+                    flush6(l_c, g_accel, kLive);
+                }
+            }
+            v0 = axpy(dt, A, v0);
+            if constexpr (early) {
+                stage6(l_vel, v0);
+                __syncthreads();
+                flush6(l_vel, g_vel, kLive);
+            }
+            q0 = integrate_world(q0, dt * v0.ang);
+            p0 = axpy(dt, v0.lin, p0);
+            A_out = A;
+            if constexpr (early) {
+                stage_pos(q0, p0);
+                __syncthreads();
+                flush7(l_pos, g_pos, kLive);
+                flushed = true;
+            }
+        }
+        if constexpr (PIPE::kHasModel) PIPE::post(P, P.tick0 + tick + 1, regs, q0, p0, v0, I_diag, mass, A_out);
+        if (record) {
+            if constexpr (INTEGRATOR != kNone) F_out = world_wrench<PIPE>(b.q, F);
+            const size_t slot = (size_t)((P.hist_slot0 + tick) % P.hist_ring);
+            if constexpr (!kDead) {
+                stage_pos(q0, p0);
+                stage6(l_vel, v0);
+                stage6(l_c, A_out);
+                stage6(l_force, F_out);
+                __syncthreads();
+                const size_t r7 = (slot * P.n + row0) * 7, r6 = (slot * P.n + row0) * 6;
+                flush7(l_pos, static_cast<T*>(P.hist_pos) + r7, kRing);
+                flush6(l_vel, static_cast<T*>(P.hist_vel) + r6, kRing);
+                flush6(l_c, static_cast<T*>(P.hist_accel) + r6, kRing);
+                flush6(l_force, static_cast<T*>(P.hist_force) + r6, kRing);
+            }
+            if constexpr (PIPE::kHasModel)
+                if (active) PIPE::record(P, slot, row0 + t, regs);
+            __syncthreads();
+        }
+    };
+    {
+        constexpr std::false_type no{};
+        constexpr std::true_type yes{};
+        uint32_t tick = 0;
+        if constexpr (PIPE::kHasModel) {
+            for (; tick < P.n_ticks; tick++) one_tick(no, no, tick);
+        } else {
+            if constexpr (INTEGRATOR == kRk4 && CHECK)
+                if (P.accel_in_check && P.n_ticks) one_tick(no, yes, tick++);
+            for (; tick + 1 < P.n_ticks; tick++) one_tick(no, no, tick);
+            if (tick < P.n_ticks) {
+                if (early_ok) one_tick(yes, no, tick);
+                else one_tick(no, no, tick);
+            }
+        }
+    }
+    if constexpr (PIPE::kHasModel) {
+        if (active) {
+            PIPE::template store<T, POL>(P, row0 + t, regs);
+            if constexpr (PIPE::kWritesInertia) {
+                T* gi = static_cast<T*>(const_cast<void*>(P.inertia)) + (size_t)(row0 + t) * 7;
+                gi[0] = I_diag.x; gi[1] = I_diag.y; gi[2] = I_diag.z; gi[6] = mass;
+            }
+        }
+    }
+    if (flushed || kDead) return;
+    stage_pos(q0, p0);
+    stage6(l_vel, v0);
+    if (!state_only) {
+        if constexpr (INTEGRATOR != kNone) F_out = world_wrench<PIPE>(b.q, F);
+        stage6(l_c, A_out);
+        stage6(l_force, F_out);
+    }
+    __syncthreads();
+    flush7(l_pos, g_pos, kLive);
+    flush6(l_vel, g_vel, kLive);
+    if (state_only) return;
+    flush6(l_c, g_accel, kLive);
+    flush6(l_force, g_force, kLive);
diff --git a/elodin_amd/csrc/step_kernel.hpp b/elodin_amd/csrc/step_kernel.hpp
--- a/elodin_amd/csrc/step_kernel.hpp
+++ b/elodin_amd/csrc/step_kernel.hpp
@@ -1,4 +1,5 @@
 #pragma once
+#include <initializer_list>
 #include <type_traits>
 
 #include "effectors.hpp"
@@ -124,323 +125,23 @@
 
 template <class T, int INTEGRATOR, class PIPE, int POL, bool CHECK = false, int ROWS = kWave>
 __global__ __launch_bounds__(kWave) void sixdof_step_kernel(const StepParams P) {
-    __shared__ __attribute__((aligned(16))) T lds[ROWS * 25];
-    T* const l_pos = lds;
-    T* const l_vel = lds + ROWS * 7;
-    T* const l_c = lds + ROWS * 13;
-    T* const l_force = lds + ROWS * 19;
-
-    const uint32_t row0 = blockIdx.x * ROWS;
-    const uint32_t rows = min((uint32_t)ROWS, P.n - row0);
-    const uint32_t t = threadIdx.x;
-    const bool full = rows == ROWS;
-
-    T* const g_pos = static_cast<T*>(P.pos) + (size_t)row0 * 7;
-    T* const g_vel = static_cast<T*>(P.vel) + (size_t)row0 * 6;
-    T* const g_accel = static_cast<T*>(P.accel) + (size_t)row0 * 6;
-    T* const g_force = static_cast<T*>(P.force) + (size_t)row0 * 6;
-    const T* const g_inertia = static_cast<const T*>(P.inertia) + (size_t)row0 * 7;
-
-    constexpr bool kEntryArgs = PIPE::kBuiltIn && (PIPE::kStatic || INTEGRATOR == kRk4);
-    constexpr bool kAuxRows3 = kEntryArgs && (PIPE::kStatic || sizeof(T) == 8);
-    if constexpr (kEntryArgs) read_entry_args<PIPE, CHECK, !kAuxRows3>(P);
-
-    constexpr bool kDead = INTEGRATOR == kNone && PIPE::kBodyDead;
-    if constexpr (!kDead) {
-        if (full) {
-            slab_dma_in<ROWS * 7 * sizeof(T), POL>(reinterpret_cast<const char*>(g_pos), reinterpret_cast<char*>(l_pos), t);
-            slab_dma_in<ROWS * 6 * sizeof(T), POL>(reinterpret_cast<const char*>(g_vel), reinterpret_cast<char*>(l_vel), t);
-            slab_dma_in<ROWS * 7 * sizeof(T), POL>(reinterpret_cast<const char*>(g_inertia), reinterpret_cast<char*>(l_c), t);
-        } else {
-            slab_in_tail(g_pos, l_pos, rows * 7, t);
-            slab_in_tail(g_vel, l_vel, rows * 6, t);
-            slab_in_tail(g_inertia, l_c, rows * 7, t);
-        }
-    }
-
-    const bool active = t < rows;
-    Vec3<T> aux[kMaxOps];
-#pragma unroll
-    for (int k = 0; k < kMaxOps; k++) aux[k] = Vec3<T>{T(0), T(0), T(0)};
-    auto load_aux = [&](auto kc) {
-        constexpr int k = decltype(kc)::value;
-        if constexpr (PIPE::template uses_aux<k>()) {
-            if (k < (int)P.n_ops && P.ops[k].aux != nullptr && active) {
-                if constexpr (!kAuxRows3) {
-                    const int w = P.ops[k].aux_width ? P.ops[k].aux_width : 3;
-                    const T* a = static_cast<const T*>(P.ops[k].aux) + (size_t)(row0 + t) * w;
-                    aux[k] = Vec3<T>{a[0], w > 1 ? a[1] : T(0), w > 2 ? a[2] : T(0)};
-                } else {
-                    const T* a = static_cast<const T*>(P.ops[k].aux) + (size_t)(row0 + t) * 3;
-                    aux[k] = Vec3<T>{a[0], a[1], a[2]};
-                }
-            }
-        }
-    };
-    load_aux(std::integral_constant<int, 0>{});
-    load_aux(std::integral_constant<int, 1>{});
-    load_aux(std::integral_constant<int, 2>{});
-    load_aux(std::integral_constant<int, 3>{});
-
-    typename PIPE::template Regs<T> regs;
-    if constexpr (PIPE::kHasModel) PIPE::template load<T, POL>(P, row0 + t, active, regs);
-
-    asm volatile("s_waitcnt vmcnt(0)" ::: "memory");
-    __syncthreads();
-
-    const Spatial<T> zero6 = {{T(0), T(0), T(0)}, {T(0), T(0), T(0)}};
-    Quat<T> q0 = {T(0), T(0), T(0), T(1)};
-    Vec3<T> p0 = {T(0), T(0), T(0)}, inv_I = {T(1), T(1), T(1)}, I_diag = {T(1), T(1), T(1)};
-    Spatial<T> v0 = zero6, A_out = zero6, F_out = zero6;
-    T mass = T(1), inv_m = T(1);
-    if (active && !kDead) {
-        const T* r = l_pos + t * 7;
-        q0 = Quat<T>{r[0], r[1], r[2], r[3]};
-        p0 = Vec3<T>{r[4], r[5], r[6]};
-        const T* s = l_vel + t * 6;
-        v0.ang = Vec3<T>{s[0], s[1], s[2]};
-        v0.lin = Vec3<T>{s[3], s[4], s[5]};
-        const T* m = l_c + t * 7;
-        I_diag = Vec3<T>{m[0], m[1], m[2]};
-        inv_I = Vec3<T>{recip(m[0]), recip(m[1]), recip(m[2])};
-        mass = m[6];
-        inv_m = recip(mass);
-        if constexpr (INTEGRATOR == kNone || PIPE::kPreReadsAccel) {
-            const T* a = g_accel + (size_t)t * 6;
-            A_out = Spatial<T>{{a[0], a[1], a[2]}, {a[3], a[4], a[5]}};
-        }
-        if constexpr (INTEGRATOR == kNone) {
-            const T* f = g_force + (size_t)t * 6;
-            F_out = Spatial<T>{{f[0], f[1], f[2]}, {f[3], f[4], f[5]}};
-        }
-    }
-    if (P.n_ticks == 0) return;
-    __syncthreads();
-
-    auto stage_pos = [&](const Quat<T>& q, const Vec3<T>& p) {
-        if (active) {
-            T* r = l_pos + t * 7;
-            r[0] = q.i; r[1] = q.j; r[2] = q.k; r[3] = q.w; r[4] = p.x; r[5] = p.y; r[6] = p.z;
-        }
-    };
-    auto stage6 = [&](T* l, const Spatial<T>& m) {
-        if (active) {
-            T* s = l + t * 6;
-            s[0] = m.ang.x; s[1] = m.ang.y; s[2] = m.ang.z; s[3] = m.lin.x; s[4] = m.lin.y; s[5] = m.lin.z;
-        }
-    };
-    auto flush7 = [&](const T* l, T* o, auto pol) {
-        if (full) slab_out<ROWS * 7 * sizeof(T), decltype(pol)::value>(reinterpret_cast<const char*>(l), reinterpret_cast<char*>(o), t);
-        else slab_out_tail(l, o, rows * 7, t);
-    };
-    auto flush6 = [&](const T* l, T* o, auto pol) {
-        if (full) slab_out<ROWS * 6 * sizeof(T), decltype(pol)::value>(reinterpret_cast<const char*>(l), reinterpret_cast<char*>(o), t);
-        else slab_out_tail(l, o, rows * 6, t);
-    };
-    constexpr std::integral_constant<int, POL> kLive{};
-    constexpr std::integral_constant<int, 1> kRing{};
-
-    const bool record = P.hist_pos != nullptr && P.hist_ring != 0;
-    const bool early_ok = !PIPE::kHasModel && !record && !(P.streaming & 256u);
-    const bool state_only = !PIPE::kHasModel && P.state_only != 0;
-    const T dt_g = T(P.dt_g), dt = T(P.dt);
-    Body<T> b;
-    b.mass = mass;
-    b.I = I_diag;
-    Wrench<T> F = zero_wrench<T>();
-    bool flushed = false;
-#ifdef SIXDOF_TICK_OUT_OF_LINE
-    auto one_tick = [&](auto early_tag, auto check_tag, uint32_t tick) __attribute__((noinline)) {
-#else
-    auto one_tick = [&](auto early_tag, auto check_tag, uint32_t tick) {
-#endif
-        constexpr bool early = decltype(early_tag)::value;
-        const bool check = decltype(check_tag)::value || (PIPE::kHasModel && P.accel_in_check && tick == 0);
-        if constexpr (PIPE::kHasModel) {
-            PIPE::pre(P, P.tick0 + tick + 1, regs, q0, p0, v0, I_diag, mass, A_out);
-            if constexpr (PIPE::kWritesInertia) {
-                inv_I = Vec3<T>{recip(I_diag.x), recip(I_diag.y), recip(I_diag.z)};
-                inv_m = recip(mass);
-                b.mass = mass;
-                b.I = I_diag;
-            }
-        }
-        if constexpr (INTEGRATOR == kRk4) {
-            const T h1 = dt_g * T(0.5), h3 = dt_g;
-            Spatial<T> A, sv, sa;
-            b.q = normalized(q0);
-            b.p = p0;
-            b.v = v0;
-            if (check && active) {
-                const T* a = g_accel + (size_t)t * 6;
-                b.v.ang = b.v.ang + T(0) * Vec3<T>{a[0], a[1], a[2]};
-                b.v.lin = b.v.lin + T(0) * Vec3<T>{a[3], a[4], a[5]};
-            }
-            F = zero_wrench<T>();
-            PIPE::apply(P, aux, regs, b, F);
-            A = calc_accel<PIPE>(b.q, F, inv_I, inv_m, T(0));
-            sv = b.v;
-            sa = A;
-            b.q = integrate_world(q0, h1 * v0.ang);
-            b.p = axpy(h1, v0.lin, p0);
-            b.v = axpy(h1, A, v0);
-            sv = axpy(T(2), b.v, sv);
-            F = zero_wrench<T>();
-            PIPE::apply(P, aux, regs, b, F);
-            A = calc_accel<PIPE>(b.q, F, inv_I, inv_m, T(0));
-            sa = axpy(T(2), A, sa);
-            b.v = axpy(h1, A, v0);
-            sv = axpy(T(2), b.v, sv);
-            if (!PIPE::vel_independent(P)) {
-                F = zero_wrench<T>();
-                PIPE::apply(P, aux, regs, b, F);
-                A = calc_accel<PIPE>(b.q, F, inv_I, inv_m, T(0));
-            }
-            sa = axpy(T(2), A, sa);
-            T n3;
-            b.q = integrate_world(q0, h3 * v0.ang, &n3);
-            const T taint = accel_taint(n3);
-            b.p = axpy(h3, v0.lin, p0);
-            b.v = axpy(PIPE::vel_independent(P) ? h3 : h3 + taint, A, v0);
-            sv = sv + b.v;
-            const T g = dt * T(1.0 / 6.0);
-            const Quat<T> q_new = integrate_world(q0, g * sv.ang);
-            const Vec3<T> p_new = axpy(g + taint, sv.lin, p0);
-            if constexpr (early) {
-                stage_pos(q_new, p_new);
-                __syncthreads();
-                flush7(l_pos, g_pos, kLive);
-            }
-            F = zero_wrench<T>();
-            PIPE::apply(P, aux, regs, b, F);
-            if constexpr (early) {
-                if (!state_only) {
-                    stage6(l_force, world_wrench<PIPE>(b.q, F));
-                    __syncthreads();
-                    flush6(l_force, g_force, kLive);
-                }
-            }
-            A = calc_accel<PIPE>(b.q, F, inv_I, inv_m + taint, taint);
-            if constexpr (early) {
-                if (!state_only) {
-                    stage6(l_c, A);
-                    __syncthreads();
-                    flush6(l_c, g_accel, kLive);
-                }
-            }
-            sa = sa + A;
-            v0 = axpy(g, sa, v0);
-            q0 = q_new;
-            p0 = p_new;
-            A_out = A;
-            if constexpr (early) {
-                stage6(l_vel, v0);
-                __syncthreads();
-                flush6(l_vel, g_vel, kLive);
-                flushed = true;
-            }
-        } else if constexpr (INTEGRATOR == kNone) {
-        } else {
-            T n0;
-            b.q = normalized(q0, &n0);
-            const T taint = accel_taint(n0);
-            b.p = p0;
-            b.v = v0;
-            F = zero_wrench<T>();
-            PIPE::apply(P, aux, regs, b, F);
-            if constexpr (early) {
-                if (!state_only) {
-                    stage6(l_force, world_wrench<PIPE>(b.q, F));
-                    __syncthreads();
-                    flush6(l_force, g_force, kLive);
-                }
-            }
-            const Spatial<T> A = calc_accel<PIPE>(b.q, F, inv_I, inv_m + taint, taint);
-            if constexpr (early) {
-                if (!state_only) {
-                    stage6(l_c, A);
-                    __syncthreads();
-                    flush6(l_c, g_accel, kLive);
-                }
-            }
-            v0 = axpy(dt, A, v0);
-            if constexpr (early) {
-                stage6(l_vel, v0);
-                __syncthreads();
-                flush6(l_vel, g_vel, kLive);
-            }
-            q0 = integrate_world(q0, dt * v0.ang);
-            p0 = axpy(dt, v0.lin, p0);
-            A_out = A;
-            if constexpr (early) {
-                stage_pos(q0, p0);
-                __syncthreads();
-                flush7(l_pos, g_pos, kLive);
-                flushed = true;
-            }
-        }
-        if constexpr (PIPE::kHasModel) PIPE::post(P, P.tick0 + tick + 1, regs, q0, p0, v0, I_diag, mass, A_out);
-        if (record) {
-            if constexpr (INTEGRATOR != kNone) F_out = world_wrench<PIPE>(b.q, F);
-            const size_t slot = (size_t)((P.hist_slot0 + tick) % P.hist_ring);
-            if constexpr (!kDead) {
-                stage_pos(q0, p0);
-                stage6(l_vel, v0);
-                stage6(l_c, A_out);
-                stage6(l_force, F_out);
-                __syncthreads();
-                const size_t r7 = (slot * P.n + row0) * 7, r6 = (slot * P.n + row0) * 6;
-                flush7(l_pos, static_cast<T*>(P.hist_pos) + r7, kRing);
-                flush6(l_vel, static_cast<T*>(P.hist_vel) + r6, kRing);
-                flush6(l_c, static_cast<T*>(P.hist_accel) + r6, kRing);
-                flush6(l_force, static_cast<T*>(P.hist_force) + r6, kRing);
-            }
-            if constexpr (PIPE::kHasModel)
-                if (active) PIPE::record(P, slot, row0 + t, regs);
-            __syncthreads();
-        }
-    };
-    {
-        constexpr std::false_type no{};
-        constexpr std::true_type yes{};
-        uint32_t tick = 0;
-        if constexpr (PIPE::kHasModel) {
-            for (; tick < P.n_ticks; tick++) one_tick(no, no, tick);
-        } else {
-            if constexpr (INTEGRATOR == kRk4 && CHECK)
-                if (P.accel_in_check && P.n_ticks) one_tick(no, yes, tick++);
-            for (; tick + 1 < P.n_ticks; tick++) one_tick(no, no, tick);
-            if (tick < P.n_ticks) {
-                if (early_ok) one_tick(yes, no, tick);
-                else one_tick(no, no, tick);
-            }
-        }
-    }
-    if constexpr (PIPE::kHasModel) {
-        if (active) {
-            PIPE::template store<T, POL>(P, row0 + t, regs);
-            if constexpr (PIPE::kWritesInertia) {
-                T* gi = static_cast<T*>(const_cast<void*>(P.inertia)) + (size_t)(row0 + t) * 7;
-                gi[0] = I_diag.x; gi[1] = I_diag.y; gi[2] = I_diag.z; gi[6] = mass;
-            }
-        }
-    }
-    if (flushed || kDead) return;
-    stage_pos(q0, p0);
-    stage6(l_vel, v0);
-    if (!state_only) {
-        if constexpr (INTEGRATOR != kNone) F_out = world_wrench<PIPE>(b.q, F);
-        stage6(l_c, A_out);
-        stage6(l_force, F_out);
-    }
-    __syncthreads();
-    flush7(l_pos, g_pos, kLive);
-    flush6(l_vel, g_vel, kLive);
-    if (state_only) return;
-    flush6(l_c, g_accel, kLive);
-    flush6(l_force, g_force, kLive);
+#include "step_body.hpp"
 }
 
+
+using PipeNone = PipeStatic<>;
+using PipeGravity = PipeStatic<SIXDOF_EFF_UNIFORM_GRAVITY>;
+using PipeGravityTorque = PipeStatic<SIXDOF_EFF_UNIFORM_GRAVITY, SIXDOF_EFF_BODY_TORQUE>;
+using PipeGravityDrag = PipeStatic<SIXDOF_EFF_UNIFORM_GRAVITY, SIXDOF_EFF_BALL_DRAG>;
+using PipeGravityThrustTorque = PipeStatic<SIXDOF_EFF_UNIFORM_GRAVITY, SIXDOF_EFF_BODY_FORCE, SIXDOF_EFF_BODY_TORQUE>;
+
+inline bool kinds_are(const StepParams& p, std::initializer_list<int> kinds) {
+    if (p.n_ops != kinds.size()) return false;
+    uint32_t k = 0;
+    for (int kind : kinds)
+        if (p.ops[k++].kind != kind) return false;
+    return true;
+}
 
 template <class T, class PIPE, int POL>
 inline StepKernel select_i(const StepParams& p, int integrator, dim3 grid) {
diff --git a/elodin_amd/csrc/tick_kernels.hip b/elodin_amd/csrc/tick_kernels.hip
--- /dev/null
+++ b/elodin_amd/csrc/tick_kernels.hip
@@ -0,0 +1,99 @@
+#include "step_kernel.hpp"
+
+namespace sixdof {
+
+template <class PIPE, int J, int K = 0>
+constexpr int tick_aux_op() {
+    if constexpr (K >= kMaxOps) return -1;
+    else if constexpr (PIPE::template uses_aux<K>()) {
+        if constexpr (J == 0) return K;
+        else return tick_aux_op<PIPE, J - 1, K + 1>();
+    } else return tick_aux_op<PIPE, J, K + 1>();
+}
+
+template <class T, class PIPE, int POL>
+__global__ __launch_bounds__(kWave) void sixdof_tick_kernel(void* pos, void* vel, const void* inertia, const void* inv_rows, const void* aux0,
+                                                            const void* aux1, uint32_t n, uint32_t state_only_arg, const TickTail R) {
+    static_assert(PIPE::kStatic && tick_aux_op<PIPE, kTickAux>() < 0, "a compile-time pipe with at most kTickAux aux columns");
+    StepParams P{};
+    P.pos = pos, P.vel = vel, P.accel = R.accel, P.force = R.force, P.inertia = inertia;
+    P.n = n, P.n_ticks = 1;
+    P.dt_g = R.dt_g, P.dt = R.dt;
+    P.n_ops = PIPE::kOps;
+    P.state_only = state_only_arg;
+    constexpr int a0 = tick_aux_op<PIPE, 0>(), a1 = tick_aux_op<PIPE, 1>();
+    if constexpr (a0 >= 0) P.ops[a0].aux = aux0;
+    if constexpr (a1 >= 0) P.ops[a1].aux = aux1;
+#pragma unroll
+    for (int k = 0; k < PIPE::kOps; k++)
+#pragma unroll
+        for (int j = 0; j < 6; j++) P.ops[k].p[j] = R.p[k][j];
+    constexpr int INTEGRATOR = kRk4, ROWS = kWave;
+    constexpr bool CHECK = false;
+#define SIXDOF_TICK_ENTRY
+#include "step_body.hpp"
+#undef SIXDOF_TICK_ENTRY
+}
+
+namespace {
+
+template <class T, class PIPE, int POL>
+StepKernel tick_of(dim3 grid) {
+    StepKernel k{reinterpret_cast<const void*>(&sixdof_tick_kernel<T, PIPE, POL>), grid, true};
+    k.tick_aux[0] = tick_aux_op<PIPE, 0>(), k.tick_aux[1] = tick_aux_op<PIPE, 1>();
+    return k;
+}
+template <class T, class PIPE>
+StepKernel tick_t(uint32_t pol, dim3 grid) {
+    switch (pol) {
+    case kPolNt: return tick_of<T, PIPE, kPolNt>(grid);
+    case kPolNtStores: return tick_of<T, PIPE, kPolNtStores>(grid);
+    case kPolPlain: return tick_of<T, PIPE, kPolPlain>(grid);
+    default: break;
+    }
+#ifdef SIXDOF_AB_BUILD
+    return {};
+#else
+    return tick_of<T, PIPE, kPolPlain>(grid);
+#endif
+}
+template <class PIPE>
+StepKernel tick_p(uint32_t pol, int dtype, dim3 grid) {
+    return dtype == SIXDOF_F64 ? tick_t<double, PIPE>(pol, grid) : tick_t<float, PIPE>(pol, grid);
+}
+
+}
+
+template <class T>
+__global__ __launch_bounds__(kBlock) void fill_inverse_kernel(const T* __restrict__ inertia, T* __restrict__ inv, uint32_t n) {
+    const uint32_t i = blockIdx.x * kBlock + threadIdx.x;
+    if (i >= n) return;
+    const T* m = inertia + (size_t)i * 7;
+    T* o = inv + (size_t)i * 4;
+    o[0] = recip(m[0]), o[1] = recip(m[1]), o[2] = recip(m[2]), o[3] = recip(m[6]);
+}
+
+hipError_t launch_fill_inverse(const void* inertia, void* inv, uint32_t n, int dtype, hipStream_t stream) {
+    if (n == 0) return hipSuccess;
+    const dim3 grid((n + kBlock - 1) / kBlock);
+    if (dtype == SIXDOF_F64) fill_inverse_kernel<double><<<grid, kBlock, 0, stream>>>(static_cast<const double*>(inertia), static_cast<double*>(inv), n);
+    else fill_inverse_kernel<float><<<grid, kBlock, 0, stream>>>(static_cast<const float*>(inertia), static_cast<float*>(inv), n);
+    return hipGetLastError();
+}
+
+StepKernel select_tick(const StepParams& p, int integrator, int dtype) {
+    const bool record = p.hist_pos != nullptr && p.hist_ring != 0;
+    if (p.n_ticks != 1 || p.accel_in_check || record || integrator != kRk4 || (p.streaming & (256u | 512u | kStreamingKeepStepKernel)))
+        return {};
+    const dim3 grid((p.n + kWave - 1) / kWave);
+    const uint32_t pol = p.streaming & 255u;
+    if (kinds_are(p, {})) return tick_p<PipeNone>(pol, dtype, grid);
+    if (kinds_are(p, {SIXDOF_EFF_UNIFORM_GRAVITY})) return tick_p<PipeGravity>(pol, dtype, grid);
+    if (kinds_are(p, {SIXDOF_EFF_UNIFORM_GRAVITY, SIXDOF_EFF_BODY_TORQUE})) return tick_p<PipeGravityTorque>(pol, dtype, grid);
+    if (kinds_are(p, {SIXDOF_EFF_UNIFORM_GRAVITY, SIXDOF_EFF_BALL_DRAG})) return tick_p<PipeGravityDrag>(pol, dtype, grid);
+    if (kinds_are(p, {SIXDOF_EFF_UNIFORM_GRAVITY, SIXDOF_EFF_BODY_FORCE, SIXDOF_EFF_BODY_TORQUE}))
+        return tick_p<PipeGravityThrustTorque>(pol, dtype, grid);
+    return {};
+}
+
+}
diff --git a/profiles/summarize.py b/profiles/summarize.py
--- a/profiles/summarize.py
+++ b/profiles/summarize.py
@@ -44,7 +44,7 @@
 pmc = defaultdict(lambda: defaultdict(list))
 for which in ("fetch", "write"):
     for r in rows(f"{out}/pmc_{which}_*/**/*counter_collection.csv"):
-        if "sixdof_step_kernel" not in r["Kernel_Name"]:
+        if "sixdof_step_kernel" not in r["Kernel_Name"] and "sixdof_tick_kernel" not in r["Kernel_Name"]:
             continue
         grid = int(r.get("Grid_Size") or 0)
         pmc[grid][r["Counter_Name"]].append(float(r["Counter_Value"]))
```

Measured after the change: 17.21 billion, median of 6. 1.07x the previous value.
